# lukors/kanter_core

Hardware: AMD Instinct MI355X
Metric: node-Mpix/s on 4096x4096 f32x4, 32-node graph (higher is better)
Workload: dtype f32

## Files before the change

### bindings/rust/kanter_core_amd_sys.rs

```rust
#![allow(non_camel_case_types, dead_code)]
use std::os::raw::{c_char, c_void};

#[repr(C)] pub struct KcPlane { _private: [u8; 0] }
#[repr(C)] pub struct KcImage { _private: [u8; 0] }
#[repr(C)] pub struct KcNodeGraph { _private: [u8; 0] }
#[repr(C)] pub struct KcLiveGraph { _private: [u8; 0] }
#[repr(C)] pub struct KcTexPro { _private: [u8; 0] }
#[repr(C)] pub struct KcPartition { _private: [u8; 0] }
#[repr(C)] pub struct KcU8Pipe { _private: [u8; 0] }

#[repr(C)] #[derive(Clone, Copy, Debug, PartialEq, Eq)]
pub struct KcPlacement { pub node_id: u32, pub rank: i32, pub component: i32, pub kind: i32 }

#[repr(C)] #[derive(Clone, Copy, Debug, PartialEq, Eq)]
pub struct KcBandRows { pub node_id: u32, pub y0: i32, pub y1: i32, pub width: u32, pub height: u32 }

#[repr(C)] #[derive(Clone, Copy, Debug, PartialEq, Eq)]
pub struct KcBandRange { pub y0: i32, pub y1: i32 }

#[repr(C)] #[derive(Clone, Copy, Debug, PartialEq, Eq)]
pub struct KcTransfer { pub node_id: u32, pub slot_id: u32, pub src_rank: i32, pub dst_rank: i32, pub level: i32 }

#[repr(C)] #[derive(Clone, Copy, Debug)]
pub struct KcDeviceImage {
// ... 75 lines not shown
    pub node_type: i32,
    pub mix_type: i32,
    pub value: f32,
    pub embed_id: u32,
    pub text: *const c_char,
    pub graph: *const KcNodeGraph,
    pub resize_policy: i32,
    pub policy_slot: u32,
    pub policy_size: KcSize,
    pub resize_filter: i32,
}

pub const KC_OK: i32 = 0;
pub const KC_ERR_CANCELED: i32 = 2;
pub const KC_ERR_NO_DEVICE: i32 = 101;

#[link(name = "kanter_core_amd")]
extern "C" {
    pub fn kc_init(device_ordinal: i32) -> i32;
    pub fn kc_shutdown() -> i32;
    pub fn kc_is_initialized() -> i32;
    pub fn kc_set_stream(hip_stream: *mut c_void) -> i32;
    pub fn kc_get_stream() -> *mut c_void;
    pub fn kc_sync() -> i32;
    pub fn kc_last_error() -> *const c_char;
    pub fn kc_status_string(status: i32) -> *const c_char;
    pub fn kc_set_fusion(enabled: i32) -> i32;
    pub fn kc_get_fusion() -> i32;
    pub fn kc_set_resize_mode(mode: i32) -> i32;
    pub fn kc_get_resize_mode() -> i32;
    pub fn kc_set_cache_policy(mode: i32) -> i32;
    pub fn kc_get_cache_policy() -> i32;
    pub fn kc_set_option(name: *const c_char, value: i32) -> i32;
    pub fn kc_get_option(name: *const c_char, value: *mut i32) -> i32;
    pub fn kc_resize_upsample_plan(in_n: u32, out_n: u32, filter: i32, eligible: *mut i32, info: *mut i32, rows: *mut f32, cap: usize) -> i32;
    pub fn kc_resize_down2_plan(in_n: u32, out_n: u32, filter: i32, info: *mut i32, left_count: *mut u32, w: *mut f32, wcap: usize, vrec: *mut u32, vcap: usize, hw: *mut f32, hcap: usize) -> i32;
    pub fn kc_stats(bytes_in_use: *mut u64, bytes_cached: *mut u64, kernel_launches: *mut u64) -> i32;
    pub fn kc_stats_algorithmic_bytes(bytes: *mut u64) -> i32;
    pub fn kc_stats_counter(name: *const c_char, value: *mut u64) -> i32;
    pub fn kc_pool_trim() -> i32;
    pub fn kc_set_specialize(mode: i32, after: i32) -> i32;
    pub fn kc_get_specialize() -> i32;
    pub fn kc_specialize_wait() -> i32;
    pub fn kc_specialize_stats(kernels_compiled: *mut u64, compiles_failed: *mut u64, specialized_launches: *mut u64, compiles_pending: *mut u64) -> i32;
    pub fn kc_specialize_compile_check(words: *const u32, n_ops: u32, n_in: u32, start_src: i32, flat: i32, source: *mut c_char, cap: usize) -> i32;
    pub fn kc_specialize_compile_check_mask(words: *const u32, n_ops: u32, n_in: u32, start_src: i32, flat: i32, nt_mask: u32, source: *mut c_char, cap: usize) -> i32;
    pub fn kc_set_chain_quads(quads: i32) -> i32;
    pub fn kc_get_chain_quads() -> i32;
    pub fn kc_specialize_compile_check_upsample(words: *const u32, n_ops: u32, n_in: u32, start_src: i32, taps: u32, wide: i32, source: *mut c_char, cap: usize) -> i32;
    pub fn kc_kernel_cache_set_dir(dir: *const c_char) -> i32;
    pub fn kc_kernel_cache_stats(files_accepted: *mut u64, files_refused: *mut u64, files_written: *mut u64, kernels_loaded: *mut u64) -> i32;
    pub fn kc_kernel_cache_precompile(words: *const u32, n_ops: u32, n_in: u32, start_src: i32, flat: i32, nt_mask: u32, up_taps: u32, up_wide: i32, dir: *const c_char) -> i32;
    pub fn kc_specialize_reset() -> i32;
    pub fn kc_plane_alloc(width: u32, height: u32, out: *mut *mut KcPlane) -> i32;
    pub fn kc_plane_const(width: u32, height: u32, value: f32, out: *mut *mut KcPlane) -> i32;
    pub fn kc_plane_wrap(device_ptr: *mut c_void, width: u32, height: u32, pitch_bytes: usize, out: *mut *mut KcPlane) -> i32;
    pub fn kc_plane_retain(p: *mut KcPlane) -> i32;
    pub fn kc_plane_release(p: *mut KcPlane) -> i32;
    pub fn kc_plane_size(p: *const KcPlane, width: *mut u32, height: *mut u32) -> i32;
    pub fn kc_plane_is_const(p: *const KcPlane, is_const: *mut i32, value: *mut f32) -> i32;
    pub fn kc_plane_materialize(p: *mut KcPlane) -> i32;
    pub fn kc_plane_device_ptr(p: *mut KcPlane, device_ptr: *mut *mut c_void, pitch_bytes: *mut usize) -> i32;
    pub fn kc_plane_upload_f32(p: *mut KcPlane, host: *const f32, host_pitch_bytes: usize) -> i32;
    pub fn kc_plane_download_f32(p: *mut KcPlane, host: *mut f32, host_pitch_bytes: usize) -> i32;
    pub fn kc_image_gray(p: *mut KcPlane, out: *mut *mut KcImage) -> i32;
    pub fn kc_image_rgba(planes: *const *mut KcPlane, out: *mut *mut KcImage) -> i32;
    pub fn kc_image_retain(img: *mut KcImage) -> i32;
    pub fn kc_image_release(img: *mut KcImage) -> i32;
    pub fn kc_image_is_rgba(img: *const KcImage, is_rgba: *mut i32) -> i32;
    pub fn kc_image_size(img: *const KcImage, size: *mut KcSize) -> i32;
    pub fn kc_image_plane(img: *const KcImage, channel: i32, out: *mut *mut KcPlane) -> i32;
    pub fn kc_image_from_value(size: KcSize, value: f32, rgba: i32, out: *mut *mut KcImage) -> i32;
    pub fn kc_image_as_type(img: *const KcImage, rgba: i32, out: *mut *mut KcImage) -> i32;
    pub fn kc_image_materialize(img: *mut KcImage) -> i32;
    pub fn kc_image_from_u8(host: *const u8, width: u32, height: u32, channels: i32, out: *mut *mut KcImage) -> i32;
    pub fn kc_image_to_u8(img: *mut KcImage, srgb: i32, host_rgba8: *mut u8) -> i32;
    pub fn kc_u8_pipe_create(width: u32, height: u32, channels: i32, depth: i32, out: *mut *mut KcU8Pipe) -> i32;
    pub fn kc_u8_pipe_free(pipe: *mut KcU8Pipe) -> i32;
    pub fn kc_u8_pipe_buffers(pipe: *mut KcU8Pipe, slot: i32, host_in: *mut *mut u8, host_out: *mut *const u8) -> i32;
    pub fn kc_u8_pipe_upload(pipe: *mut KcU8Pipe, slot: i32, out: *mut *mut KcImage) -> i32;
    pub fn kc_u8_pipe_download(pipe: *mut KcU8Pipe, slot: i32, img: *mut KcImage, srgb: i32) -> i32;
    pub fn kc_u8_pipe_wait_download(pipe: *mut KcU8Pipe, slot: i32) -> i32;
    pub fn kc_image_from_f32(host_planes: *const *const f32, n_planes: i32, width: u32, height: u32, out: *mut *mut KcImage) -> i32;
    pub fn kc_image_to_f32(img: *mut KcImage, host_planes: *const *mut f32, n_planes: i32) -> i32;
    pub fn kc_device_image_validate(d: *const KcDeviceImage, extent_bytes: *mut usize) -> i32;
    pub fn kc_image_from_device(src: *const KcDeviceImage, flags: u32, hip_stream: *mut c_void, out: *mut *mut KcImage) -> i32;
    pub fn kc_image_to_device(img: *mut KcImage, dst: *const KcDeviceImage, flags: u32, hip_stream: *mut c_void) -> i32;
    pub fn kc_image_channel_stats(img: *mut KcImage, flags: u32, out: *mut KcChannelStats) -> i32;
    pub fn kc_bc_image_validate(d: *const KcBcImage, extent_bytes: *mut usize) -> i32;
    pub fn kc_image_to_bc(img: *mut KcImage, format: i32, flags: u32, host: *mut u8, host_bytes: usize) -> i32;
    pub fn kc_image_to_bc_device(img: *mut KcImage, dst: *const KcBcImage, flags: u32, hip_stream: *mut c_void) -> i32;
    pub fn kc_mip_level_count(width: u32, height: u32, levels: *mut u32) -> i32;
    pub fn kc_preview_level(width: u32, height: u32, max_extent: u32, level: *mut u32, level_width: *mut u32, level_height: *mut u32) -> i32;
    pub fn kc_image_build_mips(img: *mut KcImage, flags: u32, levels: *mut *mut KcImage, cap: u32, count: *mut u32) -> i32;
    pub fn kc_bc_mip_layout(width: u32, height: u32, format: i32, levels: *mut u32, offsets: *mut usize, cap: u32, total_bytes: *mut usize) -> i32;
    pub fn kc_image_to_bc_mips(img: *mut KcImage, format: i32, flags: u32, host: *mut u8, host_bytes: usize) -> i32;
    pub fn kc_image_to_bc_mips_device(img: *mut KcImage, format: i32, flags: u32, device_ptr: *mut c_void, bytes: usize, hip_stream: *mut c_void) -> i32;
    pub fn kc_dds_header(width: u32, height: u32, format: i32, flags: u32, levels: u32, out: *mut u8, bytes: *mut usize) -> i32;
    pub fn kc_image_write_dds(img: *mut KcImage, path: *const c_char, format: i32, flags: u32, with_mips: i32) -> i32;
    pub fn kc_image_from_bc(host: *const u8, host_bytes: usize, width: u32, height: u32, format: i32, flags: u32, out: *mut *mut KcImage, undecoded_blocks: *mut u64) -> i32;
    pub fn kc_image_from_bc_device(src: *const KcBcImage, flags: u32, hip_stream: *mut c_void, out: *mut *mut KcImage, undecoded_blocks: *mut u64) -> i32;
    pub fn kc_image_bc_compare(img: *mut KcImage, blocks: *const KcBcImage, flags: u32, out: *mut KcBcError) -> i32;
    pub fn kc_image_bc_error(img: *mut KcImage, format: i32, flags: u32, out: *mut KcBcError) -> i32;
    pub fn kc_dds_parse(data: *const u8, bytes: usize, info: *mut KcDdsInfo) -> i32;
    pub fn kc_image_read_dds(path: *const c_char, level: u32, flags: u32, out: *mut *mut KcImage, info: *mut KcDdsInfo) -> i32;
    pub fn kc_image_read_png(path: *const c_char, out: *mut *mut KcImage) -> i32;
// ... 93 lines not shown
```

### include/kanter_core_amd.h

```cpp
#ifndef KANTER_CORE_AMD_H
#define KANTER_CORE_AMD_H

#include <stddef.h>
#include <stdint.h>

#ifdef __cplusplus
extern "C" {
#endif

#define KC_API __attribute__((visibility("default")))

typedef enum kc_status {
    KC_OK = 0,
    KC_ERR_GENERIC = 1,
    KC_ERR_CANCELED = 2,
    KC_ERR_IMAGE = 3,
    KC_ERR_INVALID_BUFFER_COUNT = 4,
    KC_ERR_INVALID_NODE_ID = 5,
    KC_ERR_INVALID_NODE_TYPE = 6,
    KC_ERR_INVALID_SLOT_ID = 7,
    KC_ERR_INVALID_SLOT_TYPE = 8,
    KC_ERR_INVALID_EDGE = 9,
    KC_ERR_NO_SLOT_DATA = 10,
    KC_ERR_SLOT_OCCUPIED = 11,
// ... 40 lines not shown
    int32_t mix_type;
    float value;
    uint32_t embed_id;
    const char *text;
    const kc_node_graph *graph;
    int32_t resize_policy;
    uint32_t policy_slot;
    kc_size policy_size;
    int32_t resize_filter;
} kc_node_desc;

KC_API int kc_init(int device_ordinal);
KC_API int kc_shutdown(void);
KC_API int kc_is_initialized(void);
KC_API int kc_set_stream(void *hip_stream);
KC_API void *kc_get_stream(void);
KC_API int kc_sync(void);
KC_API const char *kc_last_error(void);
KC_API const char *kc_status_string(int status);
KC_API int kc_set_fusion(int enabled);
KC_API int kc_get_fusion(void);
KC_API int kc_set_resize_mode(int mode);
KC_API int kc_get_resize_mode(void);
KC_API int kc_set_cache_policy(int mode);
KC_API int kc_get_cache_policy(void);
KC_API int kc_set_option(const char *name, int value);
KC_API int kc_get_option(const char *name, int *value);
KC_API int kc_resize_upsample_plan(uint32_t in_n, uint32_t out_n, int filter, int *eligible, int32_t info[5], float *rows,
                                   size_t cap);
KC_API int kc_resize_down2_plan(uint32_t in_n, uint32_t out_n, int filter, int32_t info[5], uint32_t *left_count, float *w, size_t wcap,
                                uint32_t *vrec, size_t vcap, float *hw, size_t hcap);
KC_API int kc_stats(uint64_t *bytes_in_use, uint64_t *bytes_cached, uint64_t *kernel_launches);
KC_API int kc_stats_algorithmic_bytes(uint64_t *bytes);
KC_API int kc_stats_counter(const char *name, uint64_t *value);
KC_API int kc_pool_trim(void);
KC_API int kc_set_specialize(int mode, int after);
KC_API int kc_get_specialize(void);
KC_API int kc_specialize_wait(void);
KC_API int kc_specialize_stats(uint64_t *kernels_compiled, uint64_t *compiles_failed, uint64_t *specialized_launches,
                               uint64_t *compiles_pending);
KC_API int kc_specialize_compile_check(const uint32_t *words, uint32_t n_ops, uint32_t n_in, int start_src, int flat,
                                       char *source, size_t cap);
KC_API int kc_specialize_compile_check_mask(const uint32_t *words, uint32_t n_ops, uint32_t n_in, int start_src, int flat,
                                            uint32_t nt_mask, char *source, size_t cap);
KC_API int kc_set_chain_quads(int quads);
KC_API int kc_get_chain_quads(void);
KC_API int kc_specialize_compile_check_upsample(const uint32_t *words, uint32_t n_ops, uint32_t n_in, int start_src, uint32_t taps,
                                                int wide, char *source, size_t cap);
KC_API int kc_kernel_cache_set_dir(const char *dir);
KC_API int kc_kernel_cache_stats(uint64_t *files_accepted, uint64_t *files_refused, uint64_t *files_written, uint64_t *kernels_loaded);
KC_API int kc_kernel_cache_precompile(const uint32_t *words, uint32_t n_ops, uint32_t n_in, int start_src, int flat, uint32_t nt_mask,
                                      uint32_t up_taps, int up_wide, const char *dir);
KC_API int kc_specialize_reset(void);

KC_API int kc_plane_alloc(uint32_t width, uint32_t height, kc_plane **out);
KC_API int kc_plane_const(uint32_t width, uint32_t height, float value, kc_plane **out);
KC_API int kc_plane_wrap(void *device_ptr, uint32_t width, uint32_t height, size_t pitch_bytes, kc_plane **out);
KC_API int kc_plane_retain(kc_plane *p);
KC_API int kc_plane_release(kc_plane *p);
KC_API int kc_plane_size(const kc_plane *p, uint32_t *width, uint32_t *height);
KC_API int kc_plane_is_const(const kc_plane *p, int *is_const, float *value);
KC_API int kc_plane_materialize(kc_plane *p);
KC_API int kc_plane_device_ptr(kc_plane *p, void **device_ptr, size_t *pitch_bytes);
KC_API int kc_plane_upload_f32(kc_plane *p, const float *host, size_t host_pitch_bytes);
KC_API int kc_plane_download_f32(kc_plane *p, float *host, size_t host_pitch_bytes);

KC_API int kc_image_gray(kc_plane *p, kc_image **out);
KC_API int kc_image_rgba(kc_plane *const planes[4], kc_image **out);
KC_API int kc_image_retain(kc_image *img);
KC_API int kc_image_release(kc_image *img);
KC_API int kc_image_is_rgba(const kc_image *img, int *is_rgba);
KC_API int kc_image_size(const kc_image *img, kc_size *size);
KC_API int kc_image_plane(const kc_image *img, int channel, kc_plane **out);
KC_API int kc_image_from_value(kc_size size, float value, int rgba, kc_image **out);
KC_API int kc_image_as_type(const kc_image *img, int rgba, kc_image **out);
KC_API int kc_image_materialize(kc_image *img);
KC_API int kc_image_from_u8(const uint8_t *host, uint32_t width, uint32_t height, int channels, kc_image **out);
KC_API int kc_image_to_u8(kc_image *img, int srgb, uint8_t *host_rgba8);
KC_API int kc_u8_pipe_create(uint32_t width, uint32_t height, int channels, int depth, kc_u8_pipe **out);
KC_API int kc_u8_pipe_free(kc_u8_pipe *pipe);
KC_API int kc_u8_pipe_buffers(kc_u8_pipe *pipe, int slot, uint8_t **host_in, const uint8_t **host_out);
KC_API int kc_u8_pipe_upload(kc_u8_pipe *pipe, int slot, kc_image **out);
KC_API int kc_u8_pipe_download(kc_u8_pipe *pipe, int slot, kc_image *img, int srgb);
KC_API int kc_u8_pipe_wait_download(kc_u8_pipe *pipe, int slot);
KC_API int kc_image_from_f32(const float *const host_planes[], int n_planes, uint32_t width, uint32_t height, kc_image **out);
KC_API int kc_image_to_f32(kc_image *img, float *const host_planes[], int n_planes);
typedef enum kc_dtype { KC_DTYPE_U8 = 0, KC_DTYPE_U16 = 1, KC_DTYPE_F16 = 2, KC_DTYPE_BF16 = 3, KC_DTYPE_F32 = 4 } kc_dtype;
typedef enum kc_layout { KC_LAYOUT_INTERLEAVED = 0 , KC_LAYOUT_PLANAR = 1  } kc_layout;
typedef struct kc_device_image {
    void *ptr;
    uint32_t width, height;
    int32_t channels;
    int32_t dtype, layout;
    size_t row_pitch_bytes;
    size_t channel_pitch_bytes;
} kc_device_image;
#define KC_DEVICE_SRGB 1u
#define KC_DEVICE_GRAY 2u
KC_API int kc_device_image_validate(const kc_device_image *d, size_t *extent_bytes);
KC_API int kc_image_from_device(const kc_device_image *src, uint32_t flags, void *hip_stream, kc_image **out);
KC_API int kc_image_to_device(kc_image *img, const kc_device_image *dst, uint32_t flags, void *hip_stream);
#define KC_STATS_HISTOGRAM 1u
#define KC_STATS_SRGB 2u
typedef struct kc_channel_stats {
    uint32_t channels;
    uint32_t flags;
// ... 185 lines not shown
```

### kanter_core_amd/__init__.py

```python
from .api import (Edge, EmbeddedSlotDataId, LiveGraph, MixType, Node, NodeGraph, NodeId, NodeState, NodeType,
                  ResizeFilter, ResizePolicy, Side, Size, SlotData, SlotId, SlotImage, TexProError,
                  TextureProcessor, calculate_size, combine_rgba_process, get_stream, height_to_normal_process,
                  init, is_initialized, mix_process, resize_image, separate_rgba_process, set_fusion, set_stream,
                  shutdown, stats, sync, value_process, set_specialize, get_specialize, specialize_wait,
                  specialize_stats, specialize_compile_check, Partition, PartitionPolicy, NodeKind, set_resize_mode,
                  get_resize_mode, resize_upsample_plan, resize_down2_plan, stats_counter, specialize_compile_check_upsample, specialize_compile_check_mask, set_chain_quads, get_chain_quads, set_cache_policy, get_cache_policy, set_option, get_option, comm_unique_id, comm_init,
                  comm_destroy, comm_info, comm_stats, comm_transport, comm_gather_bands, PlanKind, pool_trim, kernel_cache_set_dir, kernel_cache_stats,
                  kernel_cache_precompile, specialize_reset, U8Pipe, device_image_desc, DEVICE_SRGB, DEVICE_GRAY,
                  ChannelStats, STATS_HISTOGRAM, STATS_SRGB, BC_SRGB, BC6H, BC7, BC_BLOCK_BYTES,
                  MIP_PER_LEVEL, mip_level_count, bc_mip_layout, dds_header, BC_GRAY, BC_ALL_MODES, BcError, DdsInfo, dds_parse, preview_level)

__all__ = [n for n in dir() if not n.startswith("_")]
```

### kanter_core_amd/_lib.py

```python
import ctypes as C
import os

_HERE = os.path.dirname(os.path.abspath(__file__))
LIB_PATH = os.path.join(_HERE, "libkanter_core_amd.so")

c_u8p = C.POINTER(C.c_uint8)
c_u32p = C.POINTER(C.c_uint32)
c_fp = C.POINTER(C.c_float)
c_vp = C.c_void_p


class kc_size(C.Structure):
    _fields_ = [("width", C.c_uint32), ("height", C.c_uint32)]


class kc_edge(C.Structure):
    _fields_ = [("output_id", C.c_uint32), ("input_id", C.c_uint32), ("output_slot", C.c_uint32),
                ("input_slot", C.c_uint32)]


class kc_node_desc(C.Structure):
    _fields_ = [("node_id", C.c_uint32), ("node_type", C.c_int32), ("mix_type", C.c_int32), ("value", C.c_float),
                ("embed_id", C.c_uint32), ("text", C.c_char_p), ("graph", c_vp), ("resize_policy", C.c_int32),
                ("policy_slot", C.c_uint32), ("policy_size", kc_size), ("resize_filter", C.c_int32)]
# ... 39 lines not shown
    _fields_ = [("width", C.c_uint32), ("height", C.c_uint32), ("format", C.c_int32), ("flags", C.c_uint32), ("levels", C.c_uint32),
                ("data_offset", C.c_size_t), ("data_bytes", C.c_size_t)]


SIGNATURES = {
    "kc_init": (C.c_int, [C.c_int]),
    "kc_shutdown": (C.c_int, []),
    "kc_is_initialized": (C.c_int, []),
    "kc_set_stream": (C.c_int, [c_vp]),
    "kc_get_stream": (c_vp, []),
    "kc_sync": (C.c_int, []),
    "kc_last_error": (C.c_char_p, []),
    "kc_status_string": (C.c_char_p, [C.c_int]),
    "kc_set_fusion": (C.c_int, [C.c_int]),
    "kc_set_resize_mode": (C.c_int, [C.c_int]),
    "kc_get_resize_mode": (C.c_int, []),
    "kc_set_cache_policy": (C.c_int, [C.c_int]),
    "kc_comm_unique_id": (C.c_int, [C.c_void_p]),
    "kc_comm_init": (C.c_int, [C.c_int, C.c_int, C.c_void_p]),
    "kc_comm_destroy": (C.c_int, []),
    "kc_comm_info": (C.c_int, [C.POINTER(C.c_int), C.POINTER(C.c_int)]),
    "kc_comm_stats": (C.c_int, [C.POINTER(C.c_uint64), C.POINTER(C.c_uint64), C.POINTER(C.c_uint64)]),
    "kc_live_graph_exchange": (C.c_int, [C.c_void_p, C.c_void_p, C.c_uint32]),
    "kc_comm_transport": (C.c_int, [C.c_char_p, C.c_size_t]),
    "kc_u8_pipe_create": (C.c_int, [C.c_uint32, C.c_uint32, C.c_int, C.c_int, C.POINTER(C.c_void_p)]),
    "kc_u8_pipe_free": (C.c_int, [C.c_void_p]),
    "kc_u8_pipe_buffers": (C.c_int, [C.c_void_p, C.c_int, C.POINTER(C.c_void_p), C.POINTER(C.c_void_p)]),
    "kc_u8_pipe_upload": (C.c_int, [C.c_void_p, C.c_int, C.POINTER(C.c_void_p)]),
    "kc_u8_pipe_download": (C.c_int, [C.c_void_p, C.c_int, C.c_void_p, C.c_int]),
    "kc_u8_pipe_wait_download": (C.c_int, [C.c_void_p, C.c_int]),
    "kc_kernel_cache_set_dir": (C.c_int, [C.c_char_p]),
    "kc_kernel_cache_stats": (C.c_int, [C.POINTER(C.c_uint64)] * 4),
    "kc_kernel_cache_precompile": (C.c_int, [C.POINTER(C.c_uint32), C.c_uint32, C.c_uint32, C.c_int, C.c_int, C.c_uint32, C.c_uint32, C.c_int, C.c_char_p]),
    "kc_specialize_reset": (C.c_int, []),
    "kc_comm_gather_bands": (C.c_int, [C.c_void_p, C.c_int32, C.c_uint32, C.c_int, C.POINTER(C.c_void_p)]),
    "kc_live_graph_evaluate_partitioned": (C.c_int, [C.c_void_p, C.c_void_p, C.c_uint32, C.POINTER(C.c_void_p)]),
    "kc_set_option": (C.c_int, [C.c_char_p, C.c_int]),
    "kc_get_option": (C.c_int, [C.c_char_p, C.POINTER(C.c_int)]),
    "kc_get_cache_policy": (C.c_int, []),
    "kc_stats_counter": (C.c_int, [C.c_char_p, C.POINTER(C.c_uint64)]),
    "kc_resize_down2_plan": (C.c_int, [C.c_uint32, C.c_uint32, C.c_int, C.POINTER(C.c_int32), C.POINTER(C.c_uint32), C.POINTER(C.c_float),
                                       C.c_size_t, C.POINTER(C.c_uint32), C.c_size_t, C.POINTER(C.c_float), C.c_size_t]),
    "kc_resize_upsample_plan": (C.c_int, [C.c_uint32, C.c_uint32, C.c_int, C.POINTER(C.c_int), C.POINTER(C.c_int32),
                                          C.POINTER(C.c_float), C.c_size_t]),
    "kc_get_fusion": (C.c_int, []),
    "kc_stats": (C.c_int, [C.POINTER(C.c_uint64)] * 3),
    "kc_set_specialize": (C.c_int, [C.c_int, C.c_int]),
    "kc_get_specialize": (C.c_int, []),
    "kc_specialize_wait": (C.c_int, []),
    "kc_specialize_stats": (C.c_int, [C.POINTER(C.c_uint64)] * 4),
    "kc_specialize_compile_check": (C.c_int, [c_u32p, C.c_uint32, C.c_uint32, C.c_int, C.c_int, C.c_char_p, C.c_size_t]),
    "kc_specialize_compile_check_mask": (C.c_int, [c_u32p, C.c_uint32, C.c_uint32, C.c_int, C.c_int, C.c_uint32, C.c_char_p, C.c_size_t]),
    "kc_set_chain_quads": (C.c_int, [C.c_int]),
    "kc_get_chain_quads": (C.c_int, []),
    "kc_specialize_compile_check_upsample": (C.c_int, [c_u32p, C.c_uint32, C.c_uint32, C.c_int, C.c_uint32, C.c_int, C.c_char_p,
                                                       C.c_size_t]),
    "kc_stats_algorithmic_bytes": (C.c_int, [C.POINTER(C.c_uint64)]),
    "kc_pool_trim": (C.c_int, []),
    "kc_live_graph_partition": (C.c_int, [c_vp, C.c_uint32, C.c_int, C.c_int, C.POINTER(c_vp)]),
    "kc_partition_free": (C.c_int, [c_vp]),
    "kc_partition_info": (C.c_int, [c_vp, C.POINTER(C.c_int), C.POINTER(C.c_int), C.POINTER(C.c_int)]),
    "kc_partition_nodes": (C.c_int, [c_vp, C.POINTER(kc_placement), C.c_uint32, c_u32p]),
    "kc_partition_transfers": (C.c_int, [c_vp, C.POINTER(kc_transfer), C.c_uint32, c_u32p]),
    "kc_partition_kind": (C.c_int, [c_vp, C.POINTER(C.c_int), C.POINTER(C.c_double), C.POINTER(C.c_double), C.POINTER(C.c_double)]),
    "kc_partition_bands": (C.c_int, [c_vp, C.POINTER(kc_band_range), C.c_uint32, c_u32p, c_u32p, c_u32p]),
    "kc_partition_set_gather": (C.c_int, [c_vp, C.c_int]),
    "kc_live_graph_import_slot_data": (C.c_int, [c_vp, C.c_uint32, C.c_uint32, c_vp]),
    "kc_live_graph_evaluate_band": (C.c_int, [c_vp, C.c_uint32, C.c_uint32, C.c_int32, C.c_int32, C.POINTER(c_vp)]),
    "kc_live_graph_band_source_rows": (C.c_int, [c_vp, C.c_uint32, C.c_int32, C.c_int32, C.POINTER(kc_band_rows), C.c_uint32, c_u32p]),
    "kc_live_graph_embed_slot_data_band": (C.c_int, [c_vp, c_vp, C.c_uint32, C.c_uint32, C.c_int32, C.c_uint32]),
    "kc_plane_alloc": (C.c_int, [C.c_uint32, C.c_uint32, C.POINTER(c_vp)]),
    "kc_plane_const": (C.c_int, [C.c_uint32, C.c_uint32, C.c_float, C.POINTER(c_vp)]),
    "kc_plane_wrap": (C.c_int, [c_vp, C.c_uint32, C.c_uint32, C.c_size_t, C.POINTER(c_vp)]),
    "kc_plane_retain": (C.c_int, [c_vp]),
    "kc_plane_release": (C.c_int, [c_vp]),
    "kc_plane_size": (C.c_int, [c_vp, c_u32p, c_u32p]),
    "kc_plane_is_const": (C.c_int, [c_vp, C.POINTER(C.c_int), c_fp]),
    "kc_plane_materialize": (C.c_int, [c_vp]),
    "kc_plane_device_ptr": (C.c_int, [c_vp, C.POINTER(c_vp), C.POINTER(C.c_size_t)]),
    "kc_plane_upload_f32": (C.c_int, [c_vp, c_vp, C.c_size_t]),
    "kc_plane_download_f32": (C.c_int, [c_vp, c_vp, C.c_size_t]),
    "kc_image_gray": (C.c_int, [c_vp, C.POINTER(c_vp)]),
    "kc_image_rgba": (C.c_int, [C.POINTER(c_vp), C.POINTER(c_vp)]),
    "kc_image_retain": (C.c_int, [c_vp]),
    "kc_image_release": (C.c_int, [c_vp]),
    "kc_image_is_rgba": (C.c_int, [c_vp, C.POINTER(C.c_int)]),
    "kc_image_size": (C.c_int, [c_vp, C.POINTER(kc_size)]),
    "kc_image_plane": (C.c_int, [c_vp, C.c_int, C.POINTER(c_vp)]),
    "kc_image_from_value": (C.c_int, [kc_size, C.c_float, C.c_int, C.POINTER(c_vp)]),
    "kc_image_as_type": (C.c_int, [c_vp, C.c_int, C.POINTER(c_vp)]),
    "kc_image_materialize": (C.c_int, [c_vp]),
    "kc_image_from_u8": (C.c_int, [c_vp, C.c_uint32, C.c_uint32, C.c_int, C.POINTER(c_vp)]),
    "kc_image_to_u8": (C.c_int, [c_vp, C.c_int, c_vp]),
    "kc_device_image_validate": (C.c_int, [C.POINTER(kc_device_image), C.POINTER(C.c_size_t)]),
    "kc_image_from_device": (C.c_int, [C.POINTER(kc_device_image), C.c_uint32, c_vp, C.POINTER(c_vp)]),
    "kc_image_to_device": (C.c_int, [c_vp, C.POINTER(kc_device_image), C.c_uint32, c_vp]),
    "kc_image_channel_stats": (C.c_int, [c_vp, C.c_uint32, C.POINTER(kc_channel_stats)]),
    "kc_bc_image_validate": (C.c_int, [C.POINTER(kc_bc_image), C.POINTER(C.c_size_t)]),
    "kc_image_to_bc": (C.c_int, [c_vp, C.c_int, C.c_uint32, c_vp, C.c_size_t]),
    "kc_image_to_bc_device": (C.c_int, [c_vp, C.POINTER(kc_bc_image), C.c_uint32, c_vp]),
    "kc_mip_level_count": (C.c_int, [C.c_uint32, C.c_uint32, C.POINTER(C.c_uint32)]),
    "kc_preview_level": (C.c_int, [C.c_uint32, C.c_uint32, C.c_uint32, c_u32p, c_u32p, c_u32p]),
    "kc_image_build_mips": (C.c_int, [c_vp, C.c_uint32, C.POINTER(c_vp), C.c_uint32, C.POINTER(C.c_uint32)]),
    "kc_bc_mip_layout": (C.c_int, [C.c_uint32, C.c_uint32, C.c_int, C.POINTER(C.c_uint32), C.POINTER(C.c_size_t), C.c_uint32,
                                   C.POINTER(C.c_size_t)]),
    "kc_image_to_bc_mips": (C.c_int, [c_vp, C.c_int, C.c_uint32, c_vp, C.c_size_t]),
# ... 126 lines not shown
```

### kanter_core_amd/api.py

```python
import collections
import ctypes as C
import os

import numpy as np

from . import _lib
from ._lib import kc_edge, kc_node_desc, kc_size

_ERROR_NAMES = {
    1: "Generic", 2: "Canceled", 3: "Image", 4: "InvalidBufferCount", 5: "InvalidNodeId", 6: "InvalidNodeType",
    7: "InvalidSlotId", 8: "InvalidSlotType", 9: "InvalidEdge", 10: "NoSlotData", 11: "SlotOccupied",
    12: "SlotNotOccupied", 13: "UnableToLock", 14: "NodeProcessing", 15: "PoisonError", 16: "TryLockError",
    17: "NodeDirty", 18: "Io", 19: "InvalidName", 100: "Hip", 101: "NoDevice", 102: "InvalidArgument",
    103: "OutOfMemory", 104: "Unsupported",
}


class TexProError(Exception):

    def __init__(self, code, detail=""):
        self.code = code
        self.kind = _ERROR_NAMES.get(code, "Unknown")
        L = _lib.load()
        msg = L.kc_status_string(code).decode()
# ... 139 lines not shown
    lc = np.zeros(2 * out_n, np.uint32)
    w = np.zeros((out_n, stride), np.float32)
    vrec = np.zeros((groups, max(nc, 1), 72), np.uint32)
    hw = np.zeros((out_n, max(hstride, 1)), np.float32)
    _check(L.kc_resize_down2_plan(int(in_n), int(out_n), int(f), info, lc.ctypes.data_as(C.POINTER(C.c_uint32)),
                                  w.ctypes.data_as(C.POINTER(C.c_float)), w.size,
                                  vrec.ctypes.data_as(C.POINTER(C.c_uint32)), vrec.size if nc else 0,
                                  hw.ctypes.data_as(C.POINTER(C.c_float)), hw.size if hstride else 0))
    return dict(stride=stride, nc=nc, hstride=hstride, tile_w=tile_w, min_count=min_count, left=lc[:out_n].copy(),
                count=lc[out_n:].copy(), w=w, vrec=vrec if nc else None, hw=hw if hstride else None)


def set_specialize(mode, after=0):
    _check(_lib.load().kc_set_specialize(int(mode), int(after)))


def get_specialize():
    return _lib.load().kc_get_specialize()


def specialize_wait():
    _check(_lib.load().kc_specialize_wait())


def specialize_stats():
    v = [C.c_uint64() for _ in range(4)]
    _check(_lib.load().kc_specialize_stats(*[C.byref(x) for x in v]))
    return dict(zip(("kernels_compiled", "compiles_failed", "specialized_launches", "compiles_pending"), [x.value for x in v]))


def specialize_compile_check(words, n_in, start_src=0, flat=True):
    arr = (C.c_uint32 * len(words))(*words)
    buf = C.create_string_buffer(1 << 16)
    _check(_lib.load().kc_specialize_compile_check(arr, len(words), int(n_in), int(start_src), int(bool(flat)), buf, len(buf)))
    return buf.value.decode()


def specialize_compile_check_mask(words, n_in, nt_mask, start_src=0, flat=True):
    arr = (C.c_uint32 * len(words))(*words)
    buf = C.create_string_buffer(1 << 17)
    _check(_lib.load().kc_specialize_compile_check_mask(arr, len(words), int(n_in), int(start_src), int(bool(flat)), int(nt_mask),
                                                        buf, len(buf)))
    return buf.value.decode()


def set_chain_quads(quads):
    _check(_lib.load().kc_set_chain_quads(int(quads)))


def get_chain_quads():
    return _lib.load().kc_get_chain_quads()


def specialize_compile_check_upsample(words, n_in, start_src=0, taps=3, wide=True):
    arr = (C.c_uint32 * len(words))(*words)
    buf = C.create_string_buffer(1 << 17)
    _check(_lib.load().kc_specialize_compile_check_upsample(arr, len(words), int(n_in), int(start_src), int(taps), int(bool(wide)),
                                                            buf, len(buf)))
    return buf.value.decode()


def stats():
    a, b, c = C.c_uint64(), C.c_uint64(), C.c_uint64()
    _check(_lib.load().kc_stats(C.byref(a), C.byref(b), C.byref(c)))
    d = C.c_uint64()
    _check(_lib.load().kc_stats_algorithmic_bytes(C.byref(d)))
    return {"bytes_in_use": a.value, "bytes_cached": b.value, "kernel_launches": c.value, "algorithmic_bytes": d.value}


def kernel_cache_set_dir(path):
    _check(_lib.load().kc_kernel_cache_set_dir(None if path is None else str(path).encode()))


def kernel_cache_stats():
    v = [C.c_uint64() for _ in range(4)]
    _check(_lib.load().kc_kernel_cache_stats(*[C.byref(x) for x in v]))
    return dict(zip(("files_accepted", "files_refused", "files_written", "kernels_loaded"), (x.value for x in v)))


def kernel_cache_precompile(words, n_in, start_src, flat, nt_mask, directory, up_taps=0, up_wide=False):
    arr = (C.c_uint32 * len(words))(*words)
    _check(_lib.load().kc_kernel_cache_precompile(arr, len(words), int(n_in), int(start_src), int(bool(flat)), int(nt_mask),
                                                  int(up_taps), int(bool(up_wide)), str(directory).encode()))


def specialize_reset():
    _check(_lib.load().kc_specialize_reset())


def pool_trim():
    _check(_lib.load().kc_pool_trim())


def stats_counter(name):
    v = C.c_uint64()
    _check(_lib.load().kc_stats_counter(name.encode(), C.byref(v)))
    return v.value


class NodeId(int):
    """NodeId(u32), src/node_graph.rs:592-607"""


class SlotId(int):
    """SlotId(u32), src/node_graph.rs:609-624"""


class EmbeddedSlotDataId(int):
    """src/node/embed.rs:13-14"""


class Size:

    def __init__(self, width, height):
        self.width, self.height = int(width), int(height)

    def pixel_count(self):
        return (self.width * self.height) & 0xFFFFFFFF

    def __eq__(self, o):
        if isinstance(o, tuple):
            return (self.width, self.height) == o
        return isinstance(o, Size) and (self.width, self.height) == (o.width, o.height)

    def __hash__(self):
        return hash((self.width, self.height))

    def __iter__(self):
        return iter((self.width, self.height))

    def __repr__(self):
        return "%dx%d" % (self.width, self.height)

    def _c(self):
# ... 1143 lines not shown
```

### kanter_core_amd/build.py

```python
import os
import subprocess
import sys
from concurrent.futures import ThreadPoolExecutor

HERE = os.path.dirname(os.path.abspath(__file__))
CSRC = os.path.join(HERE, "csrc")
OBJ = os.path.join(HERE, "csrc", "build")
LIB = os.path.join(HERE, "libkanter_core_amd.so")
SOURCES = ["chain.hip", "upsample.hip", "resize_tile.hip", "resize_down.hip", "h2n.hip", "u8.hip", "chain1.hip", "down2.hip", "runtime.cpp",
           "ops.cpp", "resize.cpp", "graph.cpp", "json.cpp", "png.cpp", "specialize.cpp", "partition.cpp", "bands.cpp", "comm.cpp", "replay.cpp",
           "u8pipe.cpp", "devimage.hip", "devimage.cpp", "stats.hip", "stats.cpp", "bc.hip", "bc7.hip", "bc6h.hip", "bc.cpp", "mip.hip", "mip.cpp", "bc_decode.hip",
           "bc_decode.cpp", "bc_modes.hip",
           "c_api.cpp"]
HEADERS = ["kc_internal.hpp", "kc_runtime.hpp", "chain_program.h", os.path.join("..", "..", "include", "kanter_core_amd.h"), "pow_positive.inc",
           "srgb_thresholds.inc", "streaming.h", "bc_blocks.h", "bc_modes.h", "upsample.h", "upsample_chain.inc", "chain_apply.inc", "chain_interp.inc", "resample.inc"]
JIT_TEXTS = [("kJitChainProgramH", "chain_program.h"), ("kJitPowPositiveInc", "pow_positive.inc"), ("kJitUpsampleH", "upsample.h"),
             ("kJitUpsampleChainInc", "upsample_chain.inc")]

FLAGS = ["--offload-arch=gfx950", "-O3", "-std=c++17", "-fPIC", "-fvisibility=hidden", "-fno-fast-math",
         "-ffp-contract=off", "-fhip-fp32-correctly-rounded-divide-sqrt", "-Wall", "-Wno-unused-result"]
DEVICE_FLAGS = ["-mllvm", "-structurizecfg-skip-uniform-regions=1"]
if os.environ.get("KC_HOST_PROFILE"):
    FLAGS = FLAGS + ["-DKC_HOST_PROFILE"]
if os.environ.get("KC_HOST_SAMPLE"):
    FLAGS = FLAGS + ["-DKC_HOST_SAMPLE", "-fno-omit-frame-pointer"]


def _hipcc():
    for cand in (os.environ.get("HIPCC"), "/opt/rocm/bin/hipcc", "hipcc"):
        if cand and (os.path.isabs(cand) and os.path.exists(cand) or not os.path.isabs(cand)):
            return cand
    return "hipcc"


def _stale(target, deps):
    if not os.path.exists(target):
        return True
    t = os.path.getmtime(target)
    return any(os.path.getmtime(d) > t for d in deps)


def object_name(src):
    stem = os.path.splitext(src)[0]
    if src.endswith(".hip") and stem + ".cpp" in SOURCES:
        stem += "_kernels"
    return stem + ".o"


def _write_jit_texts():
    out = os.path.join(OBJ, "jit_texts.cpp")
    parts = ["// generated by kanter_core_amd/build.py from csrc/chain_program.h and csrc/pow_positive.inc -- do not edit\n",
             "namespace kc {\n"]
    for name, fn in JIT_TEXTS:
        with open(os.path.join(CSRC, fn)) as f:
            text = f.read()
        assert ')KCJIT"' not in text
        parts.append('extern const char %s[];\nconst char %s[] = R"KCJIT(\n%s)KCJIT";\n' % (name, name, text))
    parts.append("}  // namespace kc\n")
    new = "".join(parts)
    old = open(out).read() if os.path.exists(out) else None
    if new != old:
        with open(out, "w") as f:
            f.write(new)
    return out


def build(force=False, verbose=False):
    os.makedirs(OBJ, exist_ok=True)
    hipcc = _hipcc()
    hdrs = [os.path.join(CSRC, h) for h in HEADERS]
# ... 6 lines not shown
        jobs.append([hipcc] + FLAGS + ["-c", jit, "-o", jit_o])
    for src in SOURCES:
        s = os.path.join(CSRC, src)
        o = os.path.join(OBJ, object_name(src))
        objs.append(o)
        if force or _stale(o, [s] + hdrs):
            cmd = [hipcc] + FLAGS + (DEVICE_FLAGS + ["-x", "hip"] if src.endswith(".hip") else []) + ["-c", s, "-o", o]
            jobs.append(cmd)

    def run(cmd):
        if verbose:
            print(" ".join(cmd), flush=True)
        r = subprocess.run(cmd, stdout=subprocess.PIPE, stderr=subprocess.STDOUT, text=True)
        if r.returncode != 0:
            raise RuntimeError("hipcc failed:\n%s\n%s" % (" ".join(cmd), r.stdout))
        return r.stdout

    with ThreadPoolExecutor(max_workers=4) as ex:
        for out in ex.map(run, jobs):
            if verbose and out.strip():
                print(out)
    if force or jobs or _stale(LIB, objs):
        run([hipcc, "--offload-arch=gfx950", "-shared", "-fPIC", "-o", LIB] + objs + ["-lz", "-ldl"])
    populate_kernel_cache(verbose=verbose)
    return LIB


MANIFEST = os.path.join(HERE, "baseline_programs.jsonl")
KERNEL_CACHE = os.path.join(HERE, "kernel_cache")


def populate_kernel_cache(force=False, verbose=False):
    import ctypes as C
    import hashlib
    import json
    if not os.path.exists(MANIFEST) or not os.path.exists(LIB):
        return 0
    with open(MANIFEST) as f:
        text = f.read()
    entries = [json.loads(line) for line in text.splitlines() if line.strip()]
    st = os.stat(LIB)
    stamp = hashlib.sha256(("%s|%d|%d" % (text, st.st_mtime_ns, st.st_size)).encode()).hexdigest()
    stamp_file = os.path.join(KERNEL_CACHE, ".stamp")
    if not force and os.path.exists(stamp_file) and open(stamp_file).read() == stamp:
        return len(entries)
    os.makedirs(KERNEL_CACHE, exist_ok=True)
    for old in os.listdir(KERNEL_CACHE):
        if old.endswith(".kcco"):
            os.remove(os.path.join(KERNEL_CACHE, old))
    L = C.CDLL(LIB)
    L.kc_kernel_cache_precompile.argtypes = [C.POINTER(C.c_uint32), C.c_uint32, C.c_uint32, C.c_int, C.c_int, C.c_uint32, C.c_uint32,
                                             C.c_int, C.c_char_p]
    L.kc_kernel_cache_precompile.restype = C.c_int
    L.kc_last_error.restype = C.c_char_p

    def one(e):
        words = (C.c_uint32 * len(e["words"]))(*e["words"])
        rc = L.kc_kernel_cache_precompile(words, len(e["words"]), e["n_in"], e["start_src"], e["flat"], e["nt_mask"], e["up_taps"],
                                          e["up_wide"], KERNEL_CACHE.encode())
        if rc != 0:
            raise RuntimeError("pre-compiling %s failed (%d): %s" % (e.get("name"), rc, (L.kc_last_error() or b"").decode(errors="replace")))
        if verbose:
            print("pre-compiled", e.get("name"), flush=True)

    with ThreadPoolExecutor(max_workers=4) as ex:
        list(ex.map(one, entries))
    with open(stamp_file, "w") as f:
        f.write(stamp)
    return len(entries)


if __name__ == "__main__":
    print(build(force="--force" in sys.argv, verbose=True))
```

### kanter_core_amd/csrc/c_api.cpp

```cpp
#include <algorithm>
#include <cctype>
#include <climits>
#include <cstdio>
#include <cstdlib>
#include <cstring>
#include <fstream>
#include <sstream>

#include "kc_runtime.hpp"

namespace kc {
const std::string &last_error();
}
using namespace kc;

#define KC_ARG(cond)                                         \
    do {                                                     \
        if (!(cond)) {                                       \
            set_error("invalid argument: " #cond);           \
            return KC_ERR_INVALID_ARG;                       \
        }                                                    \
    } while (0)

typedef std::lock_guard<std::recursive_mutex> Lock;
// ... 359 lines not shown
    P.nt_mask = nt_mask;
    for (uint32_t i = 0; i < n_ops; ++i) {
        const uint32_t from = (words[i] >> 8) & 0xffu, level = words[i] >> 16;
        KC_ARG((words[i] & 0xffu) <= CH_SAVE_LOAD && (from <= n_in || (from == (uint32_t)KC_CHAIN_SRC_SAVED && (words[i] & 0xffu) != CH_SAVE_LOAD)));
        KC_ARG(level < (uint32_t)KC_CHAIN_MAX_SAVED && (level == 0 || from == (uint32_t)KC_CHAIN_SRC_SAVED || (words[i] & 0xffu) == CH_SAVE_LOAD));
        ((i & 1u) ? P.step[0][i / 2].b : P.step[0][i / 2].a).word = words[i];
    }
    if (source && cap) {
        const std::string src = specialize_source(P);
        std::snprintf(source, cap, "%s", src.c_str());
    }
    std::string log;
    int s = specialize_compile_only(P, &log);
    if (s != KC_OK) set_error("specialised chain kernel did not compile: " + log);
    return s;
}
KC_CATCH

int kc_set_chain_quads(int quads)
try {
    const int s = specialize_set_chain_quads(quads);
    if (s != KC_OK) set_error("kc_set_chain_quads accepts 0, 1, 2 or 4");
    return s;
}
KC_CATCH

int kc_get_chain_quads(void)
try {
    return specialize_get_chain_quads();
}
catch (...) {
    return 0;
}

int kc_kernel_cache_set_dir(const char *dir)
try {
    Lock lk(ctx().mu);
    return kernel_cache_set_dir(dir);
}
KC_CATCH

int kc_kernel_cache_stats(uint64_t *hits, uint64_t *rejected, uint64_t *written, uint64_t *kernels_loaded)
try {
    kernel_cache_stats(hits, rejected, written, kernels_loaded);
    return KC_OK;
}
KC_CATCH

int kc_kernel_cache_precompile(const uint32_t *words, uint32_t n_ops, uint32_t n_in, int start_src, int flat, uint32_t nt_mask,
                               uint32_t up_taps, int up_wide, const char *dir)
try {
    KC_ARG(words && dir);
    std::string log;
    const int s = kernel_cache_precompile(words, n_ops, n_in, start_src, flat != 0, nt_mask, up_taps, up_wide != 0, dir, &log);
    if (s != KC_OK) set_error("kernel cache: " + log);
    return s;
}
KC_CATCH

int kc_specialize_reset(void)
try {
    Lock lk(ctx().mu);
    if (ctx().stream) (void)hipStreamSynchronize(ctx().stream);
    const int mode = specialize_get_mode();
    specialize_shutdown();
    (void)mode;
    return KC_OK;
}
KC_CATCH

int kc_specialize_compile_check_upsample(const uint32_t *words, uint32_t n_ops, uint32_t n_in, int start_src, uint32_t taps, int wide,
                                         char *source, size_t cap)
try {
    KC_ARG(words && n_ops >= 1 && n_ops <= (uint32_t)KC_CHAIN_MAX_OPS && n_in >= 1 && n_in <= (uint32_t)KC_CHAIN_INTERP_IN);
    KC_ARG(start_src >= -1 && start_src < (int)n_in && (taps == 1 || taps == 3));
    ChainProgram P;
    std::memset(&P, 0, sizeof P);
    P.n_ops = n_ops;
    P.n_in = n_in;
    P.start_src = start_src;
    for (uint32_t i = 0; i < n_ops; ++i) {
        const uint32_t from = words[i] >> 8, code = words[i] & 0xffu;
        KC_ARG(code <= CH_MUL_INV && from <= n_in && code != CH_DIV_L && code != CH_DIV_R && code != CH_POW_L && code != CH_POW_R);
        ((i & 1u) ? P.step[0][i / 2].b : P.step[0][i / 2].a).word = words[i];
    }
    UpsampleArgs U{};
    U.H.taps = U.V.taps = taps;
    U.tile_w = wide ? 1024u : 256u;
    if (source && cap) {
        const std::string src = specialize_source(P, &U);
        std::snprintf(source, cap, "%s", src.c_str());
    }
    std::string log;
    int s = specialize_compile_only(P, &log, &U);
    if (s != KC_OK) set_error("specialised up-sampling kernel did not compile: " + log);
    return s;
}
KC_CATCH

int kc_stats(uint64_t *in_use, uint64_t *cached, uint64_t *launches)
try {
    Context &c = ctx();
    Lock lk(c.mu);
    if (in_use) *in_use = c.bytes_in_use;
    if (cached) *cached = c.bytes_cached;
    if (launches) *launches = c.launches;
    return KC_OK;
}
KC_CATCH

int kc_stats_counter(const char *name, uint64_t *value)
// ... 60 lines not shown
    *out = p;
    return KC_OK;
}
KC_CATCH

int kc_plane_retain(kc_plane *p)
try {
    Lock api_lock(ctx().mu);
    KC_ARG(p);
    plane_retain(p);
    return KC_OK;
}
KC_CATCH

int kc_plane_release(kc_plane *p)
try {
    if (!p) return KC_OK;
    Lock lk(ctx().mu);
    plane_release(p);
    return KC_OK;
}
KC_CATCH

int kc_plane_size(const kc_plane *p, uint32_t *w, uint32_t *h)
try {
    KC_ARG(p);
    if (w) *w = p->w;
    if (h) *h = p->h;
    return KC_OK;
}
KC_CATCH

int kc_plane_is_const(const kc_plane *p, int *is_const, float *v)
try {
    KC_ARG(p);
    if (is_const) *is_const = p->kind == kc_plane::CONST;
    if (v) *v = p->cval;
    return KC_OK;
}
KC_CATCH

int kc_plane_materialize(kc_plane *p)
try {
    Lock api_lock(ctx().mu);
    KC_ARG(p);
    return plane_materialize(p);
}
KC_CATCH

int kc_plane_device_ptr(kc_plane *p, void **dptr, size_t *pitch)
try {
    KC_ARG(p);
    KC_TRY(plane_materialize(p));
    if (dptr) *dptr = p->dptr;
    if (pitch) *pitch = p->pitch;
    return KC_OK;
}
KC_CATCH

int kc_plane_upload_f32(kc_plane *p, const float *host, size_t host_pitch)
try {
    KC_TRY(need_init());
    KC_ARG(p && host && p->kind == kc_plane::MEM);
    if (host_pitch == 0) host_pitch = (size_t)p->w * 4;
    Lock lk(ctx().mu);
    KC_HIP(hipMemcpy2DAsync(p->dptr, p->pitch, host, host_pitch, (size_t)p->w * 4, p->h, hipMemcpyHostToDevice, ctx().stream));
    KC_HIP(hipStreamSynchronize(ctx().stream));
    return KC_OK;
}
KC_CATCH

int kc_plane_download_f32(kc_plane *p, float *host, size_t host_pitch)
try {
    KC_ARG(p && host);
    if (host_pitch == 0) host_pitch = (size_t)p->w * 4;
    Lock lk(ctx().mu);
    if (p->kind == kc_plane::CONST) {
        for (uint32_t y = 0; y < p->h; ++y) {
            float *row = (float *)((char *)host + y * host_pitch);
            for (uint32_t x = 0; x < p->w; ++x) row[x] = p->cval;
        }
        return KC_OK;
    }
    KC_TRY(need_init());
    KC_TRY(plane_force(p));
    KC_HIP(hipMemcpy2DAsync(host, host_pitch, p->dptr, p->pitch, (size_t)p->w * 4, p->h, hipMemcpyDeviceToHost, ctx().stream));
    KC_HIP(hipStreamSynchronize(ctx().stream));
    return KC_OK;
}
KC_CATCH

int kc_image_gray(kc_plane *p, kc_image **out)
try {
    Lock api_lock(ctx().mu);
    KC_ARG(p && out);
    *out = image_new(1, &p);
    return KC_OK;
}
KC_CATCH

int kc_image_rgba(kc_plane *const planes[4], kc_image **out)
try {
    Lock api_lock(ctx().mu);
    KC_ARG(planes && out && planes[0] && planes[1] && planes[2] && planes[3]);
    for (int i = 1; i < 4; ++i) KC_ARG(planes[i]->w == planes[0]->w && planes[i]->h == planes[0]->h);
    *out = image_new(4, planes);
    return KC_OK;
}
KC_CATCH

int kc_image_retain(kc_image *img)
try {
    Lock api_lock(ctx().mu);
    KC_ARG(img);
    image_retain(img);
    return KC_OK;
}
KC_CATCH
// ... 1195 lines not shown
```

### kanter_core_amd/csrc/chain_program.h

```cpp
enum { KC_CHAIN_MAX_OPS = 80, KC_CHAIN_MAX_IN = 16, KC_CHAIN_INTERP_IN = 4, KC_CHAIN_MAX_BATCH = 4 };
#define KC_CHAIN_NT_BIT(k) ((k) < 8 ? 1u << (k) : 1u << ((k) + 8))

enum ChainCode : unsigned char {
    CH_ADD = 0,
    CH_SUB_L = 1,
    CH_SUB_R = 2,
    CH_MUL = 3,
    CH_DIV_L = 4,
    CH_DIV_R = 5,
    CH_POW_L = 6,
    CH_POW_R = 7,
    CH_ADD_R = 8,
    CH_MUL_R = 9,
    CH_ADD_INV = 10,
    CH_SUBL_INV = 11,
    CH_SUBR_INV = 12,
    CH_MUL_INV = 13,
    CH_SAVE_LOAD = 14
};
enum { KC_CHAIN_SRC_SAVED = 255, KC_CHAIN_MAX_SAVED = 3 };

struct ChainStepRec {
    unsigned int word;
    float c;
};
struct alignas(16) ChainStepPair {
    ChainStepRec a, b;
};

struct ChainProgram {
    unsigned int n_ops;
    unsigned int n_in;
    unsigned int row_units;
    unsigned int rows;
    int start_src;
    unsigned int nt_mask;
    const float *in[KC_CHAIN_MAX_BATCH][KC_CHAIN_MAX_IN];
    unsigned int in_pitch[KC_CHAIN_MAX_BATCH][KC_CHAIN_MAX_IN];
    float *out[KC_CHAIN_MAX_BATCH];
    unsigned int out_pitch[KC_CHAIN_MAX_BATCH];
    float start_c[KC_CHAIN_MAX_BATCH];
    const float *samp_src[KC_CHAIN_MAX_BATCH];
    unsigned int samp_pitch[KC_CHAIN_MAX_BATCH];
    ChainStepPair step[KC_CHAIN_MAX_BATCH][KC_CHAIN_MAX_OPS / 2 + 1];
};
```

### kanter_core_amd/csrc/kc_internal.hpp

```cpp
#pragma once

#include <hip/hip_runtime.h>

#include <atomic>
#include <cstdint>
#include <map>
#include <memory>
#include <mutex>
#include <string>
#include <vector>

#include "../../include/kanter_core_amd.h"

namespace kc {

#include "chain_program.h"
#include "upsample.h"

struct Options {
    int chain1, replay, join, wide, fusion, down2, down2_by_rows, poly2, poly2_min_ratio, resize_mode, resize_tile_w, resize_tile_h;
    int poly_rows, poly2_xcd, down2_xcd, h2n_tiled, cache_policy, cache_budget_mb, nt_force, chain_unroll, max_blocks, tune_cap;
    int upload_ring, link_gbps, hbm_gbps;
};
Options option_defaults();
// ... 118 lines not shown
                                    uint32_t dh, TapsDev h, hipStream_t s);
hipError_t launch_resize_down(const ResizePlan &r, const ResizePlanes &p, TapsDev v, TapsDev h, hipStream_t s);
hipError_t launch_resize_poly(const ResizePlan &r, const ResizePlanes &p, TapsDev v, TapsDev h, hipStream_t s);
hipError_t launch_resize_poly2(const ResizePlan &r, const ResizePlanes &p, TapsDev v, TapsDev h, hipStream_t s);
hipError_t launch_resize_down2(const ResizePlan &r, const ResizePlanes &p, const Down2Args &a, hipStream_t s);
#ifdef KC_UP_RU
constexpr uint32_t KC_UPSAMPLE_ROWS = KC_UP_RU;
#else
constexpr uint32_t KC_UPSAMPLE_ROWS = 4;
#endif
inline uint32_t upsample_tile_rows(const UpsampleArgs &u) { return KC_UPSAMPLE_ROWS * (1024u / u.tile_w); }
inline size_t upsample_lds_bytes(const UpsampleArgs &u)
{
    return ((size_t)upsample_tile_rows(u) * u.ncp + (size_t)(std::max(u.H.ratio >> 2, 1u) + u.H.qb_lo + u.H.qb_hi) * 4u * u.H.taps) * sizeof(float);
}
inline bool upsample_args_ok(const UpsampleArgs &u, int batch)
{
    if (batch < 1 || batch > 4) return false;
    if (u.tile_w % 4 != 0 || u.tile_w == 0 || u.tile_w > 1024 || 256u % (u.tile_w / 4) != 0) return false;
    const uint32_t tile_h = upsample_tile_rows(u);
    if (u.chunk == 0 || tile_h % u.chunk != 0 || u.V.ratio % u.chunk != 0) return false;
    if (u.H.ratio % 4 != 0 && !(u.H.ratio == 2 && u.H.n_out % 4 == 0)) return false;
    if (u.H.taps != u.V.taps || u.ncp % 4 != 0 || !u.H.qcls || !u.V.cls) return false;
    if (u.H.n_out > 65535 || u.V.n_out > 65535) return false;
    if (u.ncp / 4 > 257 || (std::max(u.H.ratio >> 2, 1u) + u.H.qb_lo + u.H.qb_hi) * u.H.taps > 256) return false;
    return upsample_lds_bytes(u) <= 64 * 1024;
}
inline dim3 upsample_grid(const UpsampleArgs &u, int batch)
{
    const uint32_t tile_h = upsample_tile_rows(u);
    return dim3((u.H.n_out + u.tile_w - 1) / u.tile_w, (u.V.n_out + tile_h - 1) / tile_h, batch);
}
struct UpsamplePlanes {
    const float *samp_src[4];
    unsigned int samp_pitch[4];
    float *out[4];
    unsigned int out_pitch[4];
    const float *in[4][1];
    unsigned int in_pitch[4][1];
    unsigned int nt_mask;
};
hipError_t launch_upsample_chain(const ChainProgram &p, int batch, const UpsampleArgs &u, hipStream_t s);
hipError_t launch_upsample(const UpsamplePlanes &p, int batch, const UpsampleArgs &u, hipStream_t s);
struct H2nVariant {
    bool launched = false, band = false, nt = false;
    uint32_t tq = 0;
};
hipError_t launch_height_to_normal(const float *hgt, uint32_t hpitch, uint32_t w, uint32_t h, uint32_t full_h, int band,
                                   float *nx, float *ny, float *nz, uint32_t opitch, uint32_t nt_mask, hipStream_t s, H2nVariant *var);
hipError_t launch_to_u8(Operand r, Operand g, Operand b, Operand a, int gray, int srgb, uint32_t w, uint32_t h,
                        uint8_t *dst, uint32_t nt_mask, hipStream_t s, bool *launched_nt);
hipError_t launch_from_u8(const uint8_t *src, int channels, uint32_t w, uint32_t h, float *const planes[4],
                          uint32_t pitch, uint32_t nt_mask, hipStream_t s, bool *launched_nt);
struct DevImageArgs {
    const char *ptr;
    uint64_t row_pitch, channel_pitch;
    uint32_t w, h;
    int channels, layout;
    int vec;
};
hipError_t launch_image_import(int dtype, const DevImageArgs &a, float *const planes[4], uint32_t ppitch, uint32_t nt_mask, hipStream_t s,
                               bool *launched_nt);
hipError_t launch_image_export(int dtype, int srgb, const Operand op[4], int gray, const DevImageArgs &a, uint32_t nt_mask, hipStream_t s,
                               bool *launched_nt);
struct StatsArgs {
    const float *ptr[4];
    uint32_t pitch[4];
    uint32_t w, h, n, srgb;
    uint32_t *partials;
    uint32_t rec_words;
    unsigned long long *result;
};
hipError_t launch_channel_stats(const StatsArgs &a, bool hist, bool srgb, bool nt, uint32_t groups, hipStream_t s);
uint32_t channel_stats_groups(uint32_t w, uint32_t h, bool hist, bool srgb, uint32_t cus);
hipError_t launch_bc_encode(int fmt, int srgb, const Operand op[4], int gray, char *dst, uint64_t row_pitch, uint32_t w, uint32_t h,
                            uint32_t nt_mask, hipStream_t s);
hipError_t launch_bc7_encode(int srgb, const Operand op[4], int gray, char *dst, uint64_t row_pitch, uint32_t w, uint32_t h, uint32_t nt_mask,
                             hipStream_t s);
struct BcDecodeArgs {
    const char *src;
    uint64_t row_pitch;
    float *dst[4];
    uint32_t dst_pitch;
    uint32_t w, h, bx, by;
    unsigned long long *partials, *result;
};
hipError_t launch_bc_decode(int fmt, const BcDecodeArgs &a, bool count, uint32_t nt_mask, uint32_t groups, hipStream_t s);
uint32_t bc_decode_groups(uint32_t w, uint32_t h, bool count);
constexpr uint32_t KC_BC_REC_WORDS = 17;
hipError_t launch_bc_compare(int fmt, int srgb, const Operand op[4], int gray, const char *blocks, uint64_t row_pitch, uint32_t w, uint32_t h,
                             uint32_t nt_mask, uint32_t groups, unsigned long long *partials, unsigned long long *result, hipStream_t s);
uint32_t bc_compare_groups(uint32_t w, uint32_t h);
hipError_t launch_bc_combine(const unsigned long long *partials, uint32_t groups, uint32_t rec_words, uint32_t max_cols,
                             unsigned long long *result, hipStream_t s);
hipError_t launch_bc6h_encode(const Operand op[4], int gray, char *dst, uint64_t row_pitch, uint32_t w, uint32_t h, uint32_t nt_mask,
                              hipStream_t s);
hipError_t launch_bc6h_decode(const BcDecodeArgs &a, bool count, uint32_t nt_mask, uint32_t groups, hipStream_t s);
hipError_t launch_bc6h_compare(const Operand op[4], int gray, const char *blocks, uint64_t row_pitch, uint32_t w, uint32_t h, uint32_t nt_mask,
                               uint32_t groups, unsigned long long *partials, unsigned long long *result, hipStream_t s);
hipError_t launch_bc_modes_decode(int fmt, const BcDecodeArgs &a, uint32_t nt_mask, uint32_t groups, hipStream_t s);
hipError_t launch_bc_modes_compare(int fmt, int srgb, const Operand op[4], int gray, const char *blocks, uint64_t row_pitch, uint32_t w,
                                   uint32_t h, uint32_t nt_mask, uint32_t groups, unsigned long long *partials, unsigned long long *result,
                                   hipStream_t s);
struct MipPyramidArgs {
    const float *src[4];
    uint32_t src_pitch[4];
// ... 16 lines not shown
```

### kanter_core_amd/csrc/kc_runtime.hpp

```cpp
#pragma once

#include <cstring>
#include <deque>
#include <set>
#include <tuple>
#include <type_traits>
#include <unordered_map>
#include <unordered_set>

#include "kc_internal.hpp"

namespace kc {
struct Chain;
struct ChainLink;
}

namespace kc {
#if defined(__SANITIZE_ADDRESS__) || defined(__SANITIZE_THREAD__)
#define KC_NO_OBJECT_POOL 1
#elif defined(__has_feature)
#if __has_feature(address_sanitizer) || __has_feature(thread_sanitizer)
#define KC_NO_OBJECT_POOL 1
#endif
#endif
// ... 13 lines not shown
                head = b->next;
                ::operator delete(b);
            }
            n = 0;
        }
    };
    static FreeList &list()
    {
        static FreeList fl;
        return fl;
    }
    static void *operator new(size_t bytes)
    {
        FreeList &fl = list();
        if (bytes == sizeof(T) && fl.head) {
            typename FreeList::Block *b = fl.head;
            fl.head = b->next;
            --fl.n;
            return b;
        }
        return ::operator new(bytes < sizeof(typename FreeList::Block) ? sizeof(typename FreeList::Block) : bytes);
    }
    static void operator delete(void *q, size_t bytes)
    {
        FreeList &fl = list();
        if (bytes == sizeof(T) && fl.n < FreeList::kMaxFree && !fl.closed) {
            typename FreeList::Block *b = static_cast<typename FreeList::Block *>(q);
            b->next = fl.head;
            fl.head = b;
            ++fl.n;
            return;
        }
        ::operator delete(q);
    }
#endif
};
}

struct kc_plane : kc::Pooled<kc_plane> {
    enum Kind { MEM = 0, CONST = 1, LAZY = 2, RESIZE = 3 };
    int refs = 1;
    uint32_t w = 0, h = 0;
    Kind kind = MEM;
    float *dptr = nullptr;
    size_t pitch = 0;
    size_t bytes = 0;
    bool owned = false;
    float cval = 0.0f;
    kc::ChainLink *link = nullptr;
    kc::Chain *chain = nullptr;
    kc_plane *view_of = nullptr;
    kc_plane *rz_src = nullptr;
    int rz_filter = 0;
};

struct kc_image : kc::Pooled<kc_image> {
    int refs = 1;
    int n = 0;
    kc_plane *planes[4] = { nullptr, nullptr, nullptr, nullptr };
    bool is_rgba() const { return n == 4; }
    uint32_t w() const { return planes[0]->w; }
    uint32_t h() const { return planes[0]->h; }
};

namespace kc {

struct ChainStep {
    uint8_t code;
    kc_plane *operand;
    uint8_t level = 0;
};
kc_plane *saved_value_marker();

struct Chain : Pooled<Chain> {
    kc_plane *start = nullptr;
    std::vector<ChainStep> steps;
    std::vector<kc_plane *> joined;
    ~Chain();
};

struct ChainLink : Pooled<ChainLink> {
    kc_plane *prev = nullptr;
    kc_plane *start = nullptr;
    ChainStep step{};
    uint32_t length = 1;
    bool fused = false;
    uint8_t saved = 0;
    int n_in = 0;
    struct InKey {
        const void *p = nullptr;
        size_t q = 0;
        bool operator==(const InKey &o) const { return p == o.p && q == o.q; }
    };
    InKey ins[KC_CHAIN_MAX_IN + 1];
    ~ChainLink();
};

struct TapsHost {
    std::vector<uint32_t> left, count;
    std::vector<float> w;
    uint32_t stride = 1;
    uint32_t min_count = 1;
    uint32_t reg_a = 0, reg_b = 0, reg_ages = 0, reg_ratio = 0;
    bool up_ok = false;
    UpAxis up{};
    std::vector<float> up_rows, up_qrows;
    std::vector<uint32_t> d2_vrec, d2_strips;
    std::vector<float> d2_hw;
    bool d2_want = false;
    uint32_t d2_nc = 0, d2_hstride = 0, d2_tile_w = 0;
    uint32_t p2_tile_w = 0;
    const uint32_t *d2_vrec_dev = nullptr, *d2_strips_dev = nullptr;
    const float *d2_hw_dev = nullptr;
};

struct TapsEntry {
    uint64_t last_use = 0;
    TapsHost host;
    void *dev_block = nullptr;
    size_t dev_bytes = 0;
    TapsDev dev{};
};

struct ReplayLaunch {
    ChainProgram prog;
    int batch = 0, mode = 0;
    uint32_t in_refs[KC_CHAIN_MAX_IN] = {};
    uint32_t w = 0, h = 0;
    kc_plane *planes[KC_CHAIN_MAX_BATCH] = { nullptr, nullptr, nullptr, nullptr };
    int in_from[KC_CHAIN_MAX_BATCH][KC_CHAIN_MAX_IN];
    int in_ch[KC_CHAIN_MAX_BATCH][KC_CHAIN_MAX_IN];
};
struct ReplayCapture {
    bool ok = true;
    std::vector<ReplayLaunch> launches;
};

struct Context {
    std::recursive_mutex mu;
    ReplayCapture *capture = nullptr;
    uint64_t band_taps_clock = 0;
    bool inited = false;
    int device = -1;
    hipStream_t own_stream = nullptr;
    hipStream_t stream = nullptr;
    Options opt = option_defaults();
    bool plain_chains = false;
    std::multimap<size_t, void *> free_blocks;
    uint64_t bytes_in_use = 0, bytes_cached = 0, launches = 0;
    std::map<std::string, uint64_t> counters;
    uint64_t alg_bytes = 0;
    std::map<std::tuple<uint32_t, uint32_t, int>, TapsEntry> taps;
    std::map<std::tuple<uint32_t, uint32_t, int, int32_t, int32_t, int32_t>, TapsEntry> band_taps;
    int memo_depth = 0;
    std::map<std::tuple<kc_plane *, uint32_t, uint32_t, int>, kc_plane *> resize_memo;
    struct UploadSlot {
        void *host = nullptr;
        size_t bytes = 0;
        hipEvent_t copied = nullptr;
    };
    static constexpr int kUploadSlots = 4;
    static constexpr size_t kUploadSlotMax = (size_t)4 << 20;
    UploadSlot upload_ring[kUploadSlots];
    int upload_next = 0;
    struct StatsBuffers {
        void *partials = nullptr;
        size_t partials_bytes = 0;
        unsigned long long *result = nullptr, *host = nullptr;
        hipEvent_t done = nullptr;
        uint32_t cus = 0;
    };
    StatsBuffers stats;
};

struct ResizeMemoScope {
    ResizeMemoScope();
    ~ResizeMemoScope();
};

Context &ctx();
void set_error(const std::string &msg);
const std::string &last_error();
int hip_fail(hipError_t e, const char *what);
int need_init();

#ifdef KC_HOST_PROFILE
struct ProfScope {
    const char *name;
    unsigned long long t0;
    explicit ProfScope(const char *n) : name(n), t0(__builtin_ia32_rdtsc()) {}
    ~ProfScope();
};
void prof_report();
#define KC_PROF(name) kc::ProfScope _kc_prof_scope(name)
#else
#define KC_PROF(name) (void)0
#endif

#ifdef KC_HOST_SAMPLE
void sampler_start();
void sampler_report();
#endif

// ... 87 lines not shown
    return (uint32_t)(uint8_t)a | (uint32_t)(uint8_t)b << 8 | (uint32_t)(uint8_t)c << 16 | (uint32_t)(uint8_t)d << 24;
}
const BcFormat *bc_format(int format);
const BcFormat *bc_format_of_dds(uint32_t dxgi, uint32_t cc, uint32_t *flags);
size_t bc_block_bytes(int format);
size_t bc_level_bytes(uint32_t w, uint32_t h, const BcFormat &f);
int bc_block_count(uint32_t w, uint32_t h, const char *who, uint64_t *bx, uint64_t *by);
int bc_check_flags(int format, uint32_t flags, uint32_t allowed, const char *who);
uint32_t bc_source_operands(const kc_image *img, uint32_t mask, Operand (&o)[4]);
int bc_encode(kc_image *img, int format, bool srgb, char *dst, size_t row_pitch, hipStream_t s);
hipError_t bc_launch_encode(int format, bool srgb, const Operand op[4], int gray, char *dst, uint64_t row_pitch, uint32_t w, uint32_t h,
                            uint32_t nt_mask, hipStream_t s);
hipError_t bc_launch_decode(int format, bool all_modes, const BcDecodeArgs &a, bool count, uint32_t nt_mask, uint32_t groups, hipStream_t s);
hipError_t bc_launch_compare(int format, bool srgb, bool all_modes, const Operand op[4], int gray, const char *blocks, uint64_t row_pitch, uint32_t w, uint32_t h,
                             uint32_t nt_mask, uint32_t groups, unsigned long long *partials, unsigned long long *result, hipStream_t s);
int image_from_bc(const uint8_t *host, size_t host_bytes, uint32_t w, uint32_t h, int format, uint32_t flags, kc_image **out,
                  uint64_t *undecoded_blocks);
int image_from_bc_device(const kc_bc_image *src, uint32_t flags, void *hip_stream, kc_image **out, uint64_t *undecoded_blocks);
int image_bc_compare(kc_image *img, const kc_bc_image *blocks, uint32_t flags, kc_bc_error *out);
int image_bc_error(kc_image *img, int format, uint32_t flags, kc_bc_error *out);
int dds_parse(const uint8_t *data, size_t bytes, kc_dds_info *info);
int image_read_dds(const char *path, uint32_t level, uint32_t flags, kc_image **out, kc_dds_info *info);
int mip_level_count(uint32_t w, uint32_t h, uint32_t *levels);
int preview_level(uint32_t w, uint32_t h, uint32_t max_extent, uint32_t *level, uint32_t *pw, uint32_t *ph);
float mip_const_fold(float c);
int image_build_mips(kc_image *img, uint32_t flags, kc_image **levels, uint32_t cap, uint32_t *count);
int bc_mip_layout(uint32_t w, uint32_t h, int format, uint32_t *levels, size_t *offsets, uint32_t cap, size_t *total_bytes);
int image_to_bc_mips(kc_image *img, int format, uint32_t flags, uint8_t *host, size_t host_bytes);
int image_to_bc_mips_device(kc_image *img, int format, uint32_t flags, void *device_ptr, size_t bytes, void *hip_stream);
int dds_header(uint32_t w, uint32_t h, int format, uint32_t flags, uint32_t levels, uint8_t *out, size_t *bytes);
int image_write_dds(kc_image *img, const char *path, int format, uint32_t flags, int with_mips);
int image_channel_stats(kc_image *img, uint32_t flags, kc_channel_stats *out);
int stats_buffers(size_t partials_bytes);
void channel_stats_release();
int calculate_size(int policy, const kc_size *sizes, int n, int slot_index, kc_size specific, kc_size *out);
int mix_process(kc_image *left, kc_image *right, int mix_type, kc_image **out);
int separate_process(kc_image *in, kc_image *out[4]);
int combine_process(kc_image *const in[4], kc_image **out);
int value_process(float v, kc_image **out);
int height_to_normal_process(kc_image *in, kc_image **out);
int height_to_normal_band(kc_image *in_with_halo, uint32_t full_h, kc_image **out);

int build_taps_host(uint32_t in_n, uint32_t out_n, int filter, TapsHost &t);
int resize_image(kc_image *src, kc_size size, int filter, kc_image **out);
int resize_force(kc_plane *p);
int resize_planes_band(kc_plane *const *srcs, int n, int32_t src_y0, uint32_t src_h_full, kc_size dst_full, int32_t a, int32_t b,
                       int filter, kc_plane **outs);
int resize_force_many(kc_plane *const *planes, int n);
int chain_resize_launch(const ChainProgram &P, int batch, int mode, kc_plane *const *sampled, bool *launched);

hipError_t launch_chain_specialized(const ChainProgram &P, int batch, hipStream_t s, bool *launched, uint32_t *nt_mask, uint32_t *quads = nullptr);
uint32_t cache_policy_mask(uint64_t in_bytes, uint64_t out_bytes, uint32_t n_resident, const Options &o = options());
uint32_t chain_cache_policy(const uint32_t *refs, uint32_t n, uint64_t stream_bytes, uint64_t out_bytes);
hipError_t chain_dispatch(ChainProgram &P, int batch, int mode, uint32_t w, uint32_t h, size_t out_pitch_bytes);
hipError_t launch_upsample_chain_specialized(const ChainProgram &P, int batch, const UpsampleArgs &U, hipStream_t s, bool *launched);
int specialize_set_mode(int mode, int after);
int specialize_get_mode();
int specialize_set_chain_quads(int quads);
int specialize_get_chain_quads();
void specialize_wait();
void specialize_stats(uint64_t *compiled, uint64_t *failed, uint64_t *launches, uint64_t *pending);
std::string specialize_last_log();
void specialize_shutdown();
std::string specialize_source(const ChainProgram &P, const UpsampleArgs *U = nullptr);
int specialize_compile_only(const ChainProgram &P, std::string *log, const UpsampleArgs *U = nullptr);
int kernel_cache_set_dir(const char *dir);
void kernel_cache_stats(uint64_t *hits, uint64_t *rejected, uint64_t *written, uint64_t *kernels_loaded);
bool kernel_cache_populated();
int kernel_cache_precompile(const uint32_t *words, uint32_t n_ops, uint32_t n_in, int32_t start_src, bool flat, uint32_t nt_mask,
                            uint32_t up_taps, bool up_wide, const char *dir, std::string *log);

int u8_pipe_create(uint32_t w, uint32_t h, int channels, int depth, kc_u8_pipe **out);
int u8_pipe_free(kc_u8_pipe *p);
int u8_pipe_buffers(kc_u8_pipe *p, int slot, uint8_t **host_in, const uint8_t **host_out);
int u8_pipe_upload(kc_u8_pipe *p, int slot, kc_image **out);
int u8_pipe_download(kc_u8_pipe *p, int slot, kc_image *img, bool srgb);
int u8_pipe_wait_download(kc_u8_pipe *p, int slot);

int png_read(const std::string &path, std::vector<uint8_t> &px, uint32_t &w, uint32_t &h, int &channels);
int png_write_rgba8(const std::string &path, const uint8_t *px, uint32_t w, uint32_t h);

struct NodeGraph;

struct Node {
    uint32_t node_id = 0;
    int type = KC_NODE_VALUE;
    int mix_type = KC_MIX_ADD;
    float value = 0.0f;
    uint32_t embed_id = 0;
    std::string text;
    std::shared_ptr<NodeGraph> graph;
    int policy = KC_POLICY_MOST_PIXELS;
    uint32_t policy_slot = 0;
    kc_size policy_size{ 0, 0 };
    int filter = KC_FILTER_TRIANGLE;

    bool is_input() const { return type == KC_NODE_INPUT_GRAY || type == KC_NODE_INPUT_RGBA; }
    bool is_output() const { return type == KC_NODE_OUTPUT_GRAY || type == KC_NODE_OUTPUT_RGBA; }
    bool is_source() const { return type == KC_NODE_EMBED || type == KC_NODE_IMAGE || is_input(); }
};

enum SlotType { SLOT_GRAY = 0, SLOT_RGBA = 1, SLOT_GRAY_OR_RGBA = 2 };
struct Slot {
    std::string name;
    uint32_t slot_id;
    int slot_type;
};

struct GraphIndex {
    uint64_t version = ~0ull;
    size_t n_nodes = 0, n_edges = 0;
    std::unordered_map<uint32_t, uint32_t> node_pos;
    std::unordered_map<uint32_t, std::vector<kc_edge>> in_edges;
    std::unordered_map<uint32_t, std::vector<kc_edge>> out_edges;
};

struct NodeGraph {
    std::vector<Node> nodes;
    std::vector<kc_edge> edges;
    uint32_t node_id_counter = 0;
    uint64_t version = 0;
    mutable GraphIndex idx;
// ... 213 lines not shown
```

### kanter_core_amd/csrc/replay.cpp

```cpp
#include "kc_runtime.hpp"

using namespace kc;

struct kc_live_graph::ReplayEntry {
    uint32_t root = 0;
    uint64_t ghash = 0;
    std::vector<std::pair<uint32_t, int>> pre_state;
    struct Held {
        uint32_t node, slot;
        kc_image *img;
    };
    std::vector<Held> pre_slots;
    std::vector<EmbeddedSlotData> embedded;
    std::vector<std::pair<uint32_t, int>> post_state;
    std::vector<uint32_t> dropped;
    std::vector<uint32_t> changed_ids;
    std::vector<ReplayLaunch> launches;
    uint32_t w = 0, h = 0;
    uint32_t root_slot = 0;
    int n_planes = 0;
    int out_l[4] = { -1, -1, -1, -1 };
    int out_b[4] = { -1, -1, -1, -1 };
    float cval[4] = { 0, 0, 0, 0 };

// ... 28 lines not shown
    h = mix64(h, g.edges.size());
    for (auto &e : g.edges) {
        h = mix64(h, ((uint64_t)e.output_id << 32) | e.input_id);
        h = mix64(h, ((uint64_t)e.output_slot << 32) | e.input_slot);
    }
    return h;
}

static bool recordable_type(int t)
{
    return t == KC_NODE_MIX || t == KC_NODE_VALUE || t == KC_NODE_COMBINE_RGBA || t == KC_NODE_SEPARATE_RGBA ||
           t == KC_NODE_OUTPUT_GRAY || t == KC_NODE_OUTPUT_RGBA || t == KC_NODE_EMBED;
}

static size_t slot_count_except(const kc_live_graph &lg, uint32_t node)
{
    size_t n = 0;
    for (auto &kv : lg.slot_datas)
        if (kv.first != node) n += kv.second.size();
    return n;
}

int replay_try(kc_live_graph &lg, uint32_t id, bool *hit)
{
    *hit = false;
    const kc_live_graph::ReplayEntry *e = lg.replay;
    if (!e || e->root != id || lg.use_cache || lg.auto_update || !options().fusion || !options().replay) return KC_OK;
    if (e->pre_state.size() != lg.node_state.size()) return KC_OK;
    for (auto &ps : e->pre_state) {
        auto it = lg.node_state.find(ps.first);
        if (it == lg.node_state.end() || it->second != ps.second) return KC_OK;
    }
    if (slot_count_except(lg, id) != e->pre_slots.size()) return KC_OK;
    for (auto &h : e->pre_slots) {
        const SlotData *sd = lg.find_slot(h.node, h.slot);
        if (!sd || sd->image != h.img) return KC_OK;
    }
    if (lg.embedded.size() != e->embedded.size()) return KC_OK;
    for (size_t i = 0; i < e->embedded.size(); ++i) {
        const EmbeddedSlotData &a = lg.embedded[i], &b = e->embedded[i];
        if (a.image != b.image || a.slot_data_id != b.slot_data_id || a.slot_id != b.slot_id || a.full_h != b.full_h || a.band_y0 != b.band_y0)
            return KC_OK;
    }
    if (graph_content_hash(lg.g) != e->ghash) return KC_OK;

    Context &c = ctx();
    std::vector<kc_plane *> outs(e->launches.size() * KC_CHAIN_MAX_BATCH, nullptr);
    auto drop_outs = [&] {
        for (auto *o : outs) plane_release(o);
    };
    for (size_t li = 0; li < e->launches.size(); ++li) {
        const ReplayLaunch &L = e->launches[li];
        ChainProgram P = L.prog;
        for (int b = 0; b < L.batch; ++b) {
            kc_plane *&o = outs[li * KC_CHAIN_MAX_BATCH + b];
            int s = plane_new_mem(L.w, L.h, &o);
            if (s != KC_OK) {
                drop_outs();
                return s;
            }
            P.out[b] = o->dptr;
            P.out_pitch[b] = (uint32_t)(o->pitch / 16);
            for (uint32_t k = 0; k < P.n_in; ++k)
                if (L.in_from[b][k] >= 0) {
                    const kc_plane *src = outs[(size_t)L.in_from[b][k] * KC_CHAIN_MAX_BATCH + L.in_ch[b][k]];
                    P.in[b][k] = src->dptr;
                    P.in_pitch[b][k] = (uint32_t)(src->pitch / 16);
                }
        }
        const uint64_t px4 = 4ull * L.w * L.h;
        P.nt_mask = chain_cache_policy(L.in_refs, P.n_in, px4 * L.batch, px4 * L.batch);
        hipError_t he = chain_dispatch(P, L.batch, L.mode, L.w, L.h, outs[li * KC_CHAIN_MAX_BATCH]->pitch);
        if (he == hipErrorNotReady) {
            drop_outs();
            return KC_OK;
        }
        if (he != hipSuccess) {
            drop_outs();
            return hip_fail(he, "launch_chain (replay)");
        }
        c.launches++;
        c.alg_bytes += (uint64_t)L.batch * px4 * (P.n_in + 1);
    }
    c.counters["replayed_evaluations"]++;

    kc_plane *planes[4] = { nullptr, nullptr, nullptr, nullptr };
    std::vector<kc_plane *> consts;
    for (int p = 0; p < e->n_planes; ++p) {
        if (e->out_l[p] >= 0) planes[p] = outs[(size_t)e->out_l[p] * KC_CHAIN_MAX_BATCH + e->out_b[p]];
        else {
            planes[p] = plane_new_const(e->w, e->h, e->cval[p]);
            consts.push_back(planes[p]);
        }
    }
    kc_image *img = image_new(e->n_planes, planes);
    for (auto *q : consts) plane_release(q);
    drop_outs();

    for (uint32_t d : e->dropped) lg.remove_nodes_data(d);
    lg.slot_datas[id].push_back(SlotData{ id, e->root_slot, img });
    for (auto &ps : e->post_state) lg.node_state[ps.first] = ps.second;
    for (uint32_t ch : e->changed_ids) lg.changed.insert(ch);
    *hit = true;
    return KC_OK;
}

struct ReplayRecorder {
    kc_live_graph::ReplayEntry *entry = nullptr;
    ReplayCapture cap;
    uint64_t launches0 = 0;
    std::unordered_set<uint32_t> changed0;
    std::set<const void *> resident0;
};

static void note_resident(std::set<const void *> &set, const kc_image *img)
{
    for (int p = 0; p < img->n; ++p)
        if (img->planes[p]->kind == kc_plane::MEM) set.insert(img->planes[p]->dptr);
}

ReplayRecorder *replay_begin(kc_live_graph &lg, uint32_t id)
{
    Context &c = ctx();
    if (lg.use_cache || lg.auto_update || !c.opt.fusion || !c.opt.replay || c.capture || lg.depth > 0) return nullptr;
    if (lg.g.nodes.size() > 4096) return nullptr;
    auto *r = new ReplayRecorder();
    auto *e = new kc_live_graph::ReplayEntry();
    r->entry = e;
    e->root = id;
    e->ghash = graph_content_hash(lg.g);
    e->pre_state.assign(lg.node_state.begin(), lg.node_state.end());
    for (auto &kv : lg.slot_datas)
        for (auto &sd : kv.second) {
            if (sd.node_id == id) continue;
            image_retain(sd.image);
            e->pre_slots.push_back({ sd.node_id, sd.slot_id, sd.image });
            note_resident(r->resident0, sd.image);
        }
    for (auto &em : lg.embedded) {
        if (em.full_h != 0) {
            delete e;
            delete r;
            return nullptr;
        }
        image_retain(em.image);
        e->embedded.push_back(em);
        note_resident(r->resident0, em.image);
    }
    r->launches0 = c.launches;
    r->changed0 = lg.changed;
    c.capture = &r->cap;
    return r;
}

void replay_end(kc_live_graph &lg, uint32_t id, ReplayRecorder *r, int s)
{
    if (!r) return;
    Context &c = ctx();
    c.capture = nullptr;
    std::unique_ptr<ReplayRecorder> own(r);
    std::unique_ptr<kc_live_graph::ReplayEntry> e(r->entry);
    lg.replay_clear();
    if (s != KC_OK || !r->cap.ok || r->cap.launches.empty() || c.launches - r->launches0 != r->cap.launches.size()) return;
    std::unordered_map<uint32_t, int> pre(e->pre_state.begin(), e->pre_state.end());
    if (pre.size() != lg.node_state.size()) return;
    {
        std::unordered_set<uint32_t> had;
        for (auto &h : e->pre_slots) had.insert(h.node);
        for (auto &n : lg.g.nodes)
            if (!had.count(n.node_id) && !recordable_type(n.type)) return;
    }
    for (auto &kv : lg.node_state) {
        auto it = pre.find(kv.first);
        if (it == pre.end()) return;
        if (it->second != kv.second) {
            const Node *n = lg.g.find(kv.first);
            if (!n || !recordable_type(n->type)) return;
            e->post_state.push_back({ kv.first, kv.second });
        }
    }
    std::unordered_map<uint64_t, kc_image *> before;
    for (auto &h : e->pre_slots) before[((uint64_t)h.node << 32) | h.slot] = h.img;
    std::unordered_set<uint32_t> has_after;
    const SlotData *root_sd = nullptr;
    size_t root_slots = 0;
    for (auto &kv : lg.slot_datas)
        for (auto &sd : kv.second) {
            has_after.insert(sd.node_id);
            if (sd.node_id == id) {
                root_sd = &sd;
                ++root_slots;
                continue;
            }
            auto it = before.find(((uint64_t)sd.node_id << 32) | sd.slot_id);
            if (it == before.end() || it->second != sd.image) return;
        }
    if (!root_sd || root_slots != 1) return;
    std::unordered_set<uint32_t> dropped;
    for (auto &h : e->pre_slots)
        if (!has_after.count(h.node)) dropped.insert(h.node);
    dropped.insert(id);
    for (auto &h : e->pre_slots)
        if (!dropped.count(h.node) && !lg.find_slot(h.node, h.slot)) return;
    e->dropped.assign(dropped.begin(), dropped.end());
    const kc_image *img = root_sd->image;
    ReplayCapture &cap = r->cap;
    e->w = img->w();
    e->h = img->h();
    e->root_slot = root_sd->slot_id;
    e->n_planes = img->n;
    for (int p = 0; p < img->n; ++p) {
        const kc_plane *pl = img->planes[p];
        e->out_l[p] = e->out_b[p] = -1;
        if (pl->kind == kc_plane::CONST) {
            e->cval[p] = pl->cval;
            continue;
        }
        for (size_t li = 0; li < cap.launches.size(); ++li)
            for (int b = 0; b < cap.launches[li].batch; ++b)
                if (cap.launches[li].planes[b] == pl && cap.launches[li].w == img->w() && cap.launches[li].h == img->h()) {
                    e->out_l[p] = (int)li;
                    e->out_b[p] = b;
                }
        if (e->out_l[p] < 0) return;
    }
    for (size_t li = 0; li < cap.launches.size(); ++li) {
        ReplayLaunch &L = cap.launches[li];
        for (int b = 0; b < L.batch; ++b)
            for (uint32_t k = 0; k < L.prog.n_in; ++k) {
                L.in_from[b][k] = L.in_ch[b][k] = -1;
                for (size_t lj = li; lj-- > 0 && L.in_from[b][k] < 0;)
                    for (int bj = 0; bj < cap.launches[lj].batch; ++bj)
                        if (cap.launches[lj].prog.out[bj] == L.prog.in[b][k]) {
                            if (cap.launches[lj].w != L.w || cap.launches[lj].h != L.h) return;
                            L.in_from[b][k] = (int)lj;
                            L.in_ch[b][k] = bj;
                        }
                if (L.in_from[b][k] < 0 && !r->resident0.count(L.prog.in[b][k])) return;
            }
    }
    for (uint32_t ch : lg.changed)
        if (!r->changed0.count(ch)) e->changed_ids.push_back(ch);
    e->launches = std::move(cap.launches);
    lg.replay = e.release();
}

}

void kc_live_graph::replay_clear()
{
    delete replay;
    replay = nullptr;
}
```

### kanter_core_amd/csrc/runtime.cpp

```cpp
#include <cmath>
#include <cstdlib>
#include <cstdio>
#include <cstring>

#include <algorithm>

#ifdef KC_HOST_SAMPLE
#include <dlfcn.h>
#include <new>
#include <signal.h>
#include <sys/time.h>
#include <ucontext.h>
#endif

#include "kc_runtime.hpp"

namespace kc {

static const int KC_RETRY_CHAIN = -1000;

static thread_local std::string g_last_error;

Context &ctx()
{
// ... 161 lines not shown
    c.bytes_cached = 0;
    return KC_OK;
}

static size_t pitch_for(uint32_t w)
{
    size_t row = (size_t)w * sizeof(float);
    return (row + 255) / 256 * 256;
}

int plane_new_mem(uint32_t w, uint32_t h, kc_plane **out)
{
    KC_TRY(need_init());
    if (w == 0 || h == 0) {
        set_error("plane with zero extent");
        return KC_ERR_INVALID_ARG;
    }
    kc_plane *p = new kc_plane();
    p->w = w;
    p->h = h;
    p->kind = kc_plane::MEM;
    p->pitch = pitch_for(w);
    p->bytes = p->pitch * h;
    p->owned = true;
    void *d = nullptr;
    int s = pool_alloc(p->bytes, &d);
    if (s != KC_OK) {
        delete p;
        return s;
    }
    p->dptr = (float *)d;
    *out = p;
    return KC_OK;
}

kc_plane *plane_new_const(uint32_t w, uint32_t h, float v)
{
    kc_plane *p = new kc_plane();
    p->w = w;
    p->h = h;
    p->kind = kc_plane::CONST;
    p->cval = v;
    return p;
}

void plane_release(kc_plane *p)
{
    if (!p) return;
    if (--p->refs == 0) {
        if (p->chain) delete p->chain;
        if (p->link) delete p->link;
        if (p->rz_src) plane_release(p->rz_src);
        if (p->view_of) plane_release(p->view_of);
        if (p->owned && p->dptr) pool_free(p->dptr, p->bytes);
        delete p;
    }
}

Chain::~Chain()
{
    plane_release(start);
    for (auto &s : steps) plane_release(s.operand);
    for (auto *j : joined) plane_release(j);
}

kc_plane *saved_value_marker()
{
    static kc_plane *m = [] {
        kc_plane *p = new kc_plane();
        p->kind = kc_plane::CONST;
        p->refs = 1 << 30;
        return p;
    }();
    return m;
}

ChainLink::~ChainLink()
{
    plane_release(start);
    plane_release(step.operand);
    kc_plane *q = prev;
    prev = nullptr;
    while (q) {
        if (--q->refs != 0) break;
        kc_plane *next = nullptr;
        if (q->link) {
            next = q->link->prev;
            q->link->prev = nullptr;
        }
        q->refs = 1;
        plane_release(q);
        q = next;
    }
}

static int chain_in_limit()
{
    const Context &c = ctx();
    return (c.opt.wide && c.opt.fusion && !c.plain_chains && specialize_get_mode() != 0) ? KC_CHAIN_MAX_IN : KC_CHAIN_INTERP_IN;
}

static void link_add_input(ChainLink &L, const kc_plane *q)
{
    ChainLink::InKey k;
    if (q->kind == kc_plane::MEM)
        k = { q->dptr, q->pitch };
// ... 49 lines not shown
            uint8_t code = L->step.code;
            switch (code) {
            case CH_SUB_L: code = CH_SUB_R; break;
            case CH_SUB_R: code = CH_SUB_L; break;
            case CH_DIV_L: code = CH_DIV_R; break;
            case CH_DIV_R: code = CH_DIV_L; break;
            case CH_POW_L: code = CH_POW_R; break;
            case CH_POW_R: code = CH_POW_L; break;
            default: break;
            }
            c->steps.push_back({ code, saved_value_marker(), 0 });
            for (size_t i = sub.steps.size(); i-- > 0;) {
                ChainStep st = sub.steps[i];
                if (st.code == CH_SAVE_LOAD || st.operand == saved_value_marker()) st.level++;
                c->steps.push_back(st);
            }
            c->steps.push_back({ (uint8_t)CH_SAVE_LOAD, sub.start, 0 });
            c->joined.push_back(opnd);
            plane_retain(opnd);
        } else {
            c->steps.push_back(L->step);
        }
        if (L->prev && L->prev->kind == kc_plane::LAZY) {
            q = L->prev;
            continue;
        }
        c->start = L->prev ? L->prev : L->start;
        break;
    }
    std::reverse(c->steps.begin(), c->steps.end());
    plane_retain(c->start);
    for (auto &s : c->steps) plane_retain(s.operand);
    p->chain = c;
}

Operand plane_operand(const kc_plane *p)
{
    Operand o;
    if (p->kind == kc_plane::CONST) {
        o.ptr = nullptr;
        o.pitch = 0;
        o.c = p->cval;
    } else {
        o.ptr = p->dptr;
        o.pitch = (uint32_t)(p->pitch / sizeof(float));
        o.c = 0.0f;
    }
    return o;
}

struct BuiltChain {
    ChainProgram prog;
    uint32_t in_refs[KC_CHAIN_MAX_IN] = {};
    int mode = 0;
    kc_plane *sampled[KC_CHAIN_MAX_BATCH] = { nullptr, nullptr, nullptr, nullptr };
    bool joins = false;
};

static int input_index(std::vector<const kc_plane *> &ins, const kc_plane *p)
{
    for (size_t i = 0; i < ins.size(); ++i)
        if (ins[i] == p || (p->kind == kc_plane::MEM && ins[i]->kind == kc_plane::MEM && ins[i]->dptr == p->dptr &&
                            ins[i]->pitch == p->pitch))
            return (int)i;
    ins.push_back(p);
    return (int)ins.size() - 1;
}

static bool chain_fill(BuiltChain &bc, int b, const kc_plane *p)
{
    KC_PROF("chain_fill");
    const Chain &ch = *p->chain;
    ChainProgram &P = bc.prog;
    std::vector<const kc_plane *> ins;
    kc_plane *samp = nullptr;
    if (ch.start->kind == kc_plane::MEM) input_index(ins, ch.start);
    for (auto &st : ch.steps)
        if (st.operand->kind == kc_plane::MEM) input_index(ins, st.operand);
    auto slot = [&](kc_plane *q, float *c) -> int {
        if (q == saved_value_marker()) return KC_CHAIN_SRC_SAVED - 1;
        if (q->kind == kc_plane::MEM) return input_index(ins, q);
        if (q->kind == kc_plane::RESIZE) {
            samp = q;
            return -2;
        }
        *c = q->cval;
        return -1;
    };
    const int km = (int)ins.size();
    if (km > KC_CHAIN_MAX_IN) return false;
    float c0 = 0.0f;
    int start_src = slot(ch.start, &c0);
    if (start_src == -2) start_src = km;
    if (b == 0) {
        std::memset(&P, 0, sizeof(P));
        P.start_src = start_src;
    } else if (P.start_src != start_src) {
        return false;
    }
    P.start_c[b] = c0;
    size_t r = 0;
    for (size_t i = 0; i < ch.steps.size(); ++i, ++r) {
        const ChainStep &st = ch.steps[i];
        float c = 0.0f;
        int src = slot(st.operand, &c);
        if (src == -2) src = km;
        uint8_t code = st.code;
        if (code == CH_ADD_R) code = CH_ADD;
        if (code == CH_MUL_R) code = CH_MUL;
        if (code == CH_SAVE_LOAD) bc.joins = true;
        if (src >= 0 && code <= CH_MUL && i + 1 < ch.steps.size() && ch.steps[i + 1].code == CH_SUB_R &&
            ch.steps[i + 1].operand->kind == kc_plane::CONST && ch.steps[i + 1].operand != saved_value_marker()) {
            static const uint8_t inv[4] = { CH_ADD_INV, CH_SUBL_INV, CH_SUBR_INV, CH_MUL_INV };
            code = inv[code];
            c = ch.steps[i + 1].operand->cval;
            ++i;
        }
        uint32_t word = chain_op_word(code, src);
        if (st.code == CH_SAVE_LOAD || st.operand == saved_value_marker()) word |= (uint32_t)st.level << 16;
        auto rec = [&](int ch_) -> ChainStepRec & { return (r & 1) ? P.step[ch_][r / 2].b : P.step[ch_][r / 2].a; };
        if (b == 0) {
            rec(0).word = word;
            if (code == CH_DIV_L || code == CH_DIV_R) bc.mode = bc.mode < 1 ? 1 : bc.mode;
            if (code == CH_POW_L || code == CH_POW_R) bc.mode = 2;
        } else if (r >= P.n_ops || rec(0).word != word) {
            return false;
        }
        rec(b).word = word;
        rec(b).c = c;
    }
    if (b == 0)
        P.n_ops = (uint32_t)r;
    else if (P.n_ops != r)
        return false;
    const uint32_t n_in = (uint32_t)km + (samp ? 1u : 0u);
    if (b == 0)
        P.n_in = n_in;
    else if (P.n_in != n_in || (samp != nullptr) != (bc.sampled[0] != nullptr))
        return false;
    if (samp && b > 0) {
        const kc_plane *s0 = bc.sampled[0];
        if (samp->rz_filter != s0->rz_filter || samp->rz_src->w != s0->rz_src->w || samp->rz_src->h != s0->rz_src->h)
            return false;
    }
    bc.sampled[b] = samp;
    for (int k = 0; k < km; ++k) {
        P.in[b][k] = ins[k]->dptr;
        P.in_pitch[b][k] = (uint32_t)(ins[k]->pitch / 16);
        if (b == 0) bc.in_refs[k] = (uint32_t)ins[k]->refs;
    }
    if (samp) {
        P.samp_src[b] = samp->rz_src->dptr;
        P.samp_pitch[b] = (uint32_t)(samp->rz_src->pitch / 4);
    }
    return true;
}

static int chain_prepare(kc_plane *p)
{
    Chain &ch = *p->chain;
    kc_plane *first = nullptr;
    auto visit = [&](kc_plane *q) -> int {
        if (q->kind != kc_plane::RESIZE) return KC_OK;
        if (!first) {
            first = q;
            return KC_OK;
        }
        return q == first ? KC_OK : resize_force(q);
    };
    KC_TRY(visit(ch.start));
    for (auto &st : ch.steps) KC_TRY(visit(st.operand));
    return KC_OK;
}

uint32_t chain_cache_policy(const uint32_t *refs, uint32_t n, uint64_t stream_bytes, uint64_t out_bytes)
{
    const Options &o = options();
    if (!o.cache_policy) return 0;
    uint32_t all = 0;
    for (uint32_t k = 0; k < n; ++k) all |= KC_CHAIN_NT_BIT(k);
    if (o.nt_force >= 0) return (uint32_t)o.nt_force & (all | 0x100u);
    const uint64_t budget = (uint64_t)o.cache_budget_mb << 20;
    if (n * stream_bytes + out_bytes <= budget) return 0;
    uint32_t mask = all;
    uint64_t used = 0;
    for (;;) {
        int best = -1;
        for (uint32_t k = 0; k < n; ++k)
            if ((mask & KC_CHAIN_NT_BIT(k)) && refs[k] >= 2 && (best < 0 || refs[k] > refs[best])) best = (int)k;
        if (best < 0 || used + stream_bytes > budget) break;
        used += stream_bytes;
        mask &= ~KC_CHAIN_NT_BIT(best);
    }
    if (used + out_bytes > budget) mask |= 0x100u;
    return mask;
}

uint32_t cache_policy_mask(uint64_t in_bytes, uint64_t out_bytes, uint32_t n_resident, const Options &o)
{
    if (!o.cache_policy) return 0;
    if (o.nt_force >= 0) return (uint32_t)o.nt_force & (((1u << n_resident) - 1u) | 0x100u);
    const uint64_t budget = (uint64_t)o.cache_budget_mb << 20;
    if (in_bytes + out_bytes <= budget) return 0;
    uint32_t mask = (1u << n_resident) - 1u;
    if (out_bytes > budget) mask |= 0x100u;
    return mask;
}

namespace {
struct ChainCounterNames {
    std::string interp[5][9][3][2];
    std::string k0[3];
    std::string chain1[8];
    std::string spec[0x200], spec_q2[0x200], spec_q4[0x200];
    ChainCounterNames()
    {
        char buf[64];
        for (int k = 1; k <= 4; ++k)
            for (int u : { 1, 2, 4, 6, 8 })
                for (int m = 0; m < 3; ++m)
                    for (int nt = 0; nt < 2; ++nt) {
                        std::snprintf(buf, sizeof buf, "chain_interp_k%d_u%d_m%d%s", k, u, m, nt ? "_nt" : "");
                        interp[k][u][m][nt] = buf;
                    }
        for (int m = 0; m < 3; ++m) k0[m] = "chain_k0_m" + std::to_string(m);
        for (int b = 0; b < 8; ++b) chain1[b] = "chain1_nt" + std::to_string(b);
        for (int b = 0; b < 0x200; ++b) {
            std::snprintf(buf, sizeof buf, "specialized_nt_%03x", b);
            spec[b] = buf;
            spec_q2[b] = spec[b] + "_q2";
            spec_q4[b] = spec[b] + "_q4";
        }
    }
};
const ChainCounterNames &chain_counter_names()
{
    static const ChainCounterNames n;
    return n;
}
}

hipError_t chain_dispatch(ChainProgram &P, int batch, int mode, uint32_t w, uint32_t h, size_t out_pitch_bytes)
{
    Context &c = ctx();
    const uint32_t row_units = (w + 3) / 4;
    bool launched = false;
    bool dense = (size_t)row_units * 16 == out_pitch_bytes;
    for (int b = 0; b < batch && dense; ++b)
        for (uint32_t k = 0; k < P.n_in; ++k)
            if (P.in_pitch[b][k] != row_units) dense = false;
    if (dense) {
        P.rows = 1;
        P.row_units = row_units * h;
    } else {
        P.rows = h;
        P.row_units = row_units;
    }
    if (!launched && P.n_ops == 1 && c.opt.chain1) {
        Chain1Args a{};
        const uint32_t w0 = P.step[0][0].a.word, from = w0 >> 8;
        for (int b = 0; b < batch; ++b) {
            if (P.start_src >= 0) {
                a.start[b] = P.in[b][P.start_src];
                a.start_pitch[b] = P.in_pitch[b][P.start_src];
            }
            a.start_c[b] = P.start_c[b];
            if (from) {
                a.operand[b] = P.in[b][from - 1];
                a.operand_pitch[b] = P.in_pitch[b][from - 1];
            }
            a.operand_c[b] = a.c[b] = P.step[b][0].a.c;
            a.out[b] = P.out[b];
            a.out_pitch[b] = P.out_pitch[b];
        }
        a.rows = P.rows;
        a.row_units = P.row_units;
        const unsigned nt = (P.start_src >= 0 && (P.nt_mask >> P.start_src & 1u) ? 1u : 0u) | (from && (P.nt_mask >> (from - 1) & 1u) ? 2u : 0u) |
                            (P.nt_mask & 0x100u ? 4u : 0u);
        unsigned launched_nt = ~0u;
        hipError_t e = launch_chain1(a, batch, (int)(w0 & 0xffu), nt, c.stream, &launched_nt);
        if (e != hipSuccess) return e;
        c.counters["chain1_launches"]++;
        if (launched_nt < 8) c.counters[chain_counter_names().chain1[launched_nt]]++;
        launched = true;
    }
    if (!launched) {
        uint32_t spec_nt = 0, spec_quads = 1;
        hipError_t e = launch_chain_specialized(P, batch, c.stream, &launched, &spec_nt, &spec_quads);
        if (e == hipSuccess && launched) {
            const ChainCounterNames &names = chain_counter_names();
            c.counters[(spec_quads == 2 ? names.spec_q2 : spec_quads == 4 ? names.spec_q4 : names.spec)[spec_nt & 0x1ffu]]++;
        }
        if (e == hipSuccess && !launched) {
            if (P.n_in > (uint32_t)KC_CHAIN_INTERP_IN) return hipErrorNotReady;
            for (uint32_t i = 0; i < P.n_ops; ++i)
                if ((((i & 1u) ? P.step[0][i / 2].b.word : P.step[0][i / 2].a.word) & 0xffu) == CH_SAVE_LOAD) return hipErrorNotReady;
            ChainVariant v;
            e = launch_chain(P, batch, mode, c.opt.max_blocks, c.opt.chain_unroll, c.stream, &v);
            if (e == hipSuccess && v.k == 0) c.counters[chain_counter_names().k0[v.mode]]++;
            else if (e == hipSuccess && v.k > 0) c.counters[chain_counter_names().interp[v.k][v.u][v.mode][v.nt ? 1 : 0]]++;
        }
        if (e != hipSuccess) return e;
    }
    return hipSuccess;
}

static int chain_flatten_to_fit(kc_plane *p, int limit);
static_assert(sizeof(ChainProgram) <= 4096, "a launch passes at most 4 KB of kernel arguments");

static int chain_launch(BuiltChain &bc, kc_plane *const *planes, int batch)
{
    KC_PROF("chain_launch");
    Context &c = ctx();
    ChainProgram &P = bc.prog;
    const kc_plane *p0 = planes[0];
    std::vector<kc_plane *> outs(batch, nullptr);
    for (int b = 0; b < batch; ++b) {
        int s = plane_new_mem(p0->w, p0->h, &outs[b]);
        if (s != KC_OK) {
            for (auto *o : outs) plane_release(o);
            return s;
        }
        P.out[b] = outs[b]->dptr;
        P.out_pitch[b] = (uint32_t)(outs[b]->pitch / 16);
    }
    {
        const uint64_t px4 = 4ull * p0->w * p0->h;
        const uint32_t resident = P.n_in - (bc.sampled[0] ? 1u : 0u);
        P.nt_mask = chain_cache_policy(bc.in_refs, resident, px4 * batch, px4 * batch);
    }
    bool launched = false;
    if (bc.sampled[0]) {
        int s = chain_resize_launch(P, batch, bc.mode, bc.sampled, &launched);
        if (s != KC_OK || !launched) {
            for (auto *o : outs) plane_release(o);
            if (s != KC_OK) return s;
            KC_TRY(resize_force_many(bc.sampled, batch));
            return KC_RETRY_CHAIN;
        }
    }
    if (!launched) {
        hipError_t e = chain_dispatch(P, batch, bc.mode, p0->w, p0->h, outs[0]->pitch);
        if (e == hipErrorNotReady && (bc.joins || P.n_in > (uint32_t)KC_CHAIN_INTERP_IN)) {
            for (auto *o : outs) plane_release(o);
            std::vector<kc_plane *> subs;
            for (size_t j = 0; j < planes[0]->chain->joined.size(); ++j)
                for (int b = 0; b < batch; ++b)
                    if (j < planes[b]->chain->joined.size()) subs.push_back(planes[b]->chain->joined[j]);
            if (!subs.empty()) KC_TRY(planes_force(subs.data(), (int)subs.size()));
            for (int b = 0; b < batch; ++b) {
                if (planes[b]->kind != kc_plane::LAZY) continue;
                delete planes[b]->chain;
                planes[b]->chain = nullptr;
                KC_TRY(chain_flatten_to_fit(planes[b], KC_CHAIN_INTERP_IN));
            }
            c.counters["join_fallbacks"]++;
            if (c.capture) c.capture->ok = false;
            return KC_RETRY_CHAIN;
        }
        if (e != hipSuccess) {
            for (auto *o : outs) plane_release(o);
            return hip_fail(e, "launch_chain");
        }
        if (bc.joins) c.counters["join_launches"]++;
        if (P.n_in > (uint32_t)KC_CHAIN_INTERP_IN) c.counters["wide_launches"]++;
    }
    c.launches++;
    {
        uint64_t px = (uint64_t)p0->w * p0->h, bytes = 0;
        for (int b = 0; b < batch; ++b) {
            const uint32_t resident = P.n_in - (bc.sampled[b] ? 1u : 0u);
            bytes += 4 * px * (resident + 1);
            if (bc.sampled[b]) bytes += 4 * (uint64_t)bc.sampled[b]->rz_src->w * bc.sampled[b]->rz_src->h;
        }
        c.alg_bytes += bytes;
    }
    if (c.capture) {
        ReplayCapture &cap = *c.capture;
        if (bc.sampled[0] || cap.launches.size() >= 32) cap.ok = false;
        else {
            cap.launches.emplace_back();
            ReplayLaunch &L = cap.launches.back();
            L.prog = P;
            L.batch = batch;
            L.mode = bc.mode;
            std::memcpy(L.in_refs, bc.in_refs, sizeof L.in_refs);
            L.w = p0->w;
            L.h = p0->h;
            for (int b = 0; b < batch; ++b) L.planes[b] = planes[b];
        }
    }
    for (int b = 0; b < batch; ++b) {
        kc_plane *p = planes[b];
        Chain *old = p->chain;
        ChainLink *old_link = p->link;
        p->chain = nullptr;
        p->link = nullptr;
        p->kind = kc_plane::MEM;
        p->dptr = outs[b]->dptr;
        p->pitch = outs[b]->pitch;
        p->bytes = outs[b]->bytes;
        p->owned = true;
        outs[b]->owned = false;
        outs[b]->dptr = nullptr;
        plane_release(outs[b]);
        delete old;
        delete old_link;
    }
    return KC_OK;
}

static int chain_flatten_to_fit(kc_plane *p, int limit)
{
    chain_flatten(p);
    while (chain_distinct_inputs(*p->chain) > limit || chain_record_count(*p->chain) > (size_t)KC_CHAIN_MAX_OPS) {
        if (!p->chain->joined.empty()) {
            std::vector<kc_plane *> subs(p->chain->joined);
            for (auto *q : subs) plane_retain(q);
            const int fs = planes_force(subs.data(), (int)subs.size());
            for (auto *q : subs) plane_release(q);
            KC_TRY(fs);
            if (p->kind != kc_plane::LAZY) return KC_OK;
            delete p->chain;
            p->chain = nullptr;
            chain_flatten(p);
            continue;
        }
        kc_plane *prev = p->link->prev;
        if (!prev || prev->kind != kc_plane::LAZY) {
            set_error("chain with more inputs than a program holds cannot be split");
            return KC_ERR_UNSUPPORTED;
        }
        {
            std::vector<kc_plane *> path;
            for (kc_plane *q = prev; q && q->kind == kc_plane::LAZY; q = q->link->prev) path.push_back(q);
            std::reverse(path.begin(), path.end());
            std::vector<ChainLink::InKey> keys;
            auto add = [&](const kc_plane *q) {
                ChainLink::InKey k;
                if (q->kind == kc_plane::MEM) k = { q->dptr, q->pitch };
                else if (q->kind == kc_plane::RESIZE) k = { q, ~(size_t)0 };
                else return;
// ... 328 lines not shown
```

### kanter_core_amd/csrc/specialize.cpp

```cpp
#include <dlfcn.h>
#include <sys/stat.h>
#include <unistd.h>

#include <condition_variable>
#include <cstdio>
#include <cstdlib>
#include <cstring>
#include <thread>

#include "kc_runtime.hpp"

namespace kc {

extern const char kJitChainProgramH[];
extern const char kJitPowPositiveInc[];
extern const char kJitUpsampleH[];
extern const char kJitUpsampleChainInc[];

namespace {

typedef struct _hiprtcProgram *hiprtcProgram;
struct Rtc {
    void *lib = nullptr;
    int (*create)(hiprtcProgram *, const char *, const char *, int, const char **, const char **) = nullptr;
    int (*compile)(hiprtcProgram, int, const char **) = nullptr;
    int (*log_size)(hiprtcProgram, size_t *) = nullptr;
    int (*log)(hiprtcProgram, char *) = nullptr;
    int (*code_size)(hiprtcProgram, size_t *) = nullptr;
    int (*code)(hiprtcProgram, char *) = nullptr;
    int (*destroy)(hiprtcProgram *) = nullptr;
    int (*version)(int *, int *) = nullptr;
    bool ok = false;
    bool tried = false;
};

void specialize_stop_at_exit();

Rtc &rtc()
{
    static Rtc r;
    static std::once_flag once;
    std::call_once(once, [] {
        r.tried = true;
        for (const char *name : { "libhiprtc.so", "libhiprtc.so.7", "/opt/rocm/lib/libhiprtc.so" }) {
            r.lib = dlopen(name, RTLD_NOW | RTLD_LOCAL);
            if (r.lib) break;
        }
        if (!r.lib) return;
#define KC_RTC_SYM(field, sym) *(void **)(&r.field) = dlsym(r.lib, sym)
        KC_RTC_SYM(create, "hiprtcCreateProgram");
        KC_RTC_SYM(compile, "hiprtcCompileProgram");
        KC_RTC_SYM(log_size, "hiprtcGetProgramLogSize");
        KC_RTC_SYM(log, "hiprtcGetProgramLog");
        KC_RTC_SYM(code_size, "hiprtcGetCodeSize");
        KC_RTC_SYM(code, "hiprtcGetCode");
        KC_RTC_SYM(destroy, "hiprtcDestroyProgram");
        KC_RTC_SYM(version, "hiprtcVersion");
#undef KC_RTC_SYM
        r.ok = r.create && r.compile && r.log_size && r.log && r.code_size && r.code && r.destroy;
        if (r.ok) std::atexit(specialize_stop_at_exit);
    });
    return r;
}

struct Signature {
    uint32_t n_in = 0, n_ops = 0;
    int32_t start_src = 0;
    bool flat = false;
    uint32_t up_taps = 0;
    bool up_wide = false;
    uint32_t nt_mask = 0;
    uint32_t quads = 1;
    uint32_t word[KC_CHAIN_MAX_OPS] = {};

    std::string key() const
    {
        std::string k((const char *)&n_in, sizeof n_in);
        k.append((const char *)&n_ops, sizeof n_ops);
        k.append((const char *)&start_src, sizeof start_src);
        k.push_back(flat ? 'f' : 'p');
        k.push_back((char)('0' + up_taps));
        k.push_back(up_wide ? 'w' : 'n');
        k.append((const char *)&nt_mask, sizeof nt_mask);
        k.append((const char *)word, sizeof(uint32_t) * n_ops);
        if (quads > 1) {
            k.push_back('q');
            k.push_back((char)('0' + quads));
        }
        return k;
    }
};

constexpr uint32_t kQuadsWarm = 2, kQuadsMaxOps = 16;
std::atomic<int> g_chain_quads{ 0 };

uint32_t chain_quads_for(const Signature &s, uint64_t total_units)
{
    if (s.up_taps || !s.flat || s.n_in < 1 || s.n_ops > kQuadsMaxOps || total_units > 0xF0000000ull) return 1;
    bool plain = false;
    for (uint32_t k = 0; k < s.n_in; ++k) plain |= !(s.nt_mask & KC_CHAIN_NT_BIT(k));
    if (!plain || !s.nt_mask) return 1;
    for (uint32_t i = 0; i < s.n_ops; ++i) {
        const uint32_t code = s.word[i] & 0xffu;
        if (code == CH_DIV_L || code == CH_DIV_R || code == CH_POW_L || code == CH_POW_R) return 1;
    }
    const int forced = g_chain_quads.load(std::memory_order_relaxed);
    return forced ? (uint32_t)forced : kQuadsWarm;
}

Signature signature_of(const ChainProgram &P, const UpsampleArgs *U = nullptr)
{
    Signature s;
    s.n_in = P.n_in;
    s.n_ops = P.n_ops;
    s.start_src = P.start_src;
    s.flat = U ? false : P.rows == 1;
    {
        uint32_t valid = 0x100u;
        for (uint32_t k = 0; k < (U ? P.n_in - 1u : P.n_in); ++k) valid |= KC_CHAIN_NT_BIT(k);
        s.nt_mask = P.nt_mask & valid;
    }
    if (U) {
        s.up_taps = U->H.taps;
        s.up_wide = U->tile_w == 1024;
    }
    for (uint32_t i = 0; i < P.n_ops; ++i) s.word[i] = (i & 1u) ? P.step[0][i / 2].b.word : P.step[0][i / 2].a.word;
    s.quads = chain_quads_for(s, (uint64_t)P.rows * P.row_units);
    return s;
}

static int spec_wg()
{
    static int wg = [] {
        int v = 256;
        if (const char *e = std::getenv("KC_SPEC_WG")) {
            const int x = std::atoi(e);
            if (x == 64 || x == 128 || x == 256 || x == 512 || x == 1024) v = x;
        }
        return v;
    }();
    return wg;
}

std::string kernel_name(const Signature &s)
{
    uint32_t h = 2166136261u;
    for (unsigned char c : s.key()) h = (h ^ c) * 16777619u;
    char buf[32];
    std::snprintf(buf, sizeof buf, s.up_taps ? "kc_upchain_%08x" : "kc_chain_%08x", h);
    return buf;
}

static const char kPackedF4[] = R"KCF4(typedef float raw4 __attribute__((ext_vector_type(4)));
typedef float f2 __attribute__((ext_vector_type(2)));
typedef unsigned long long __attribute__((may_alias)) rec64;
static __device__ __forceinline__ f2 pk_sub(f2 a, f2 b)
{
    f2 d;
    asm("v_pk_add_f32 %0, %1, %2 neg_lo:[0,1] neg_hi:[0,1]" : "=v"(d) : "v"(a), "v"(b));
    return d;
}
struct kconst {
    rec64 rec;  // { word, c }
    __device__ __forceinline__ operator float() const { return __builtin_bit_cast(float, (unsigned int)(rec >> 32)); }
    __device__ __forceinline__ f2 minus(f2 b) const
    {
        f2 d;
        asm("v_pk_add_f32 %0, %1, %2 op_sel_hi:[0,1] neg_lo:[0,1] neg_hi:[0,1]" : "=v"(d) : "s"(rec >> 32), "v"(b));
        return d;
    }
};
struct f4 {
    f2 lo, hi;
    f4() = default;
    __device__ __forceinline__ f4(float x, float y, float z, float w) : lo{ x, y }, hi{ z, w } {}
    __device__ __forceinline__ f4(f2 l, f2 h) : lo(l), hi(h) {}
    __device__ __forceinline__ f4(raw4 v) : lo(v.xy), hi(v.zw) {}
    __device__ __forceinline__ raw4 raw() const { return raw4{ lo.x, lo.y, hi.x, hi.y }; }
};
// ... 33 lines not shown
    case CH_MUL: return std::string("acc * ") + x;
    case CH_DIV_L: return std::string("acc / ") + x;
    case CH_DIV_R: return std::string(x) + " / acc";
    case CH_POW_L: return std::string("pow4(acc, ") + x + ", pow_tab)";
    case CH_POW_R: return std::string("pow4(") + x + ", acc, pow_tab)";
    case CH_ADD_INV: return std::string(c) + " - (acc + " + x + ")";
    case CH_SUBL_INV: return std::string(c) + " - (acc - " + x + ")";
    case CH_SUBR_INV: return std::string(c) + " - (" + x + " - acc)";
    case CH_MUL_INV: return std::string(c) + " - (acc * " + x + ")";
    default: return std::string();
    }
}

static std::string generate_up(const Signature &s)
{
    std::string src;
    src.reserve(32768);
    src += "namespace kc {\n";
    src += kJitChainProgramH;
    src += kJitUpsampleH;
    src += "typedef float f4 __attribute__((ext_vector_type(4)));\n";
    src += kJitUpsampleChainInc;
    char buf[320];
    std::snprintf(buf, sizeof buf,
                  "struct UpProg {\n    const ChainProgram &P;\n"
                  "    __device__ __forceinline__ void operator()(const f4 (&in)[%u][%u], f4 (&out)[%u]) const\n    {\n"
                  "        const unsigned int b = blockIdx.z;\n        const ChainStepPair *pp = P.step[b];\n"
                  "#pragma unroll\n        for (int u = 0; u < %u; ++u) {\n",
                  s.n_in, KC_UPSAMPLE_ROWS, KC_UPSAMPLE_ROWS, KC_UPSAMPLE_ROWS);
    src += buf;
    if (s.start_src < 0)
        src += "            f4 acc = f4{ P.start_c[b], P.start_c[b], P.start_c[b], P.start_c[b] };\n";
    else {
        std::snprintf(buf, sizeof buf, "            f4 acc = in[%d][u];\n", s.start_src);
        src += buf;
    }
    for (uint32_t i = 0; i < s.n_ops; ++i) {
        const uint32_t code = s.word[i] & 0xffu;
        if (code == CH_DIV_L || code == CH_DIV_R || code == CH_POW_L || code == CH_POW_R || code == CH_SAVE_LOAD) return std::string();
        const std::string e = step_expr(s, i, "in[", "][u]");
        if (e.empty()) return std::string();
        src += "            acc = " + e + ";\n";
    }
    src += "            out[u] = acc;\n        }\n    }\n};\n}  // namespace kc\nusing namespace kc;\n";
    std::snprintf(buf, sizeof buf,
                  "extern \"C\" __global__ __launch_bounds__(256) void %s(const ChainProgram P, const UpsampleArgs U)\n{\n"
                  "    extern __shared__ __attribute__((aligned(16))) float lds[];\n"
                  "    upsample_chain_tile<%u, %u, %u, %s, 0x%xu>(P, U, lds, UpProg{ P });\n}\n",
                  kernel_name(s).c_str(), s.n_in, s.up_taps, KC_UPSAMPLE_ROWS, s.up_wide ? "true" : "false", s.nt_mask);
    src += buf;
    return src;
}

static std::string generate_quads(const Signature &s, int SPEC_WG)
{
    std::string src;
    char buf[320];
    std::snprintf(buf, sizeof buf,
                  "    const unsigned int n = P.rows * P.row_units;\n"
                  "    const unsigned int idx = blockIdx.x * %uu + threadIdx.x;\n    if (idx >= n) return;\n",
                  s.quads * (uint32_t)SPEC_WG);
    src += buf;
    for (uint32_t u = 0; u < s.quads; ++u) {
        if (u == 0)
            src += "    const unsigned int at0 = idx;\n";
        else {
            std::snprintf(buf, sizeof buf, "    const unsigned int at%u = idx + %uu < n ? idx + %uu : n - 1u;\n", u, u * SPEC_WG, u * SPEC_WG);
            src += buf;
        }
        for (uint32_t k = 0; k < s.n_in; ++k) {
            if (s.nt_mask & KC_CHAIN_NT_BIT(k))
                std::snprintf(buf, sizeof buf, "    const f4 in%u_%u = __builtin_nontemporal_load(&reinterpret_cast<const raw4 *>(P.in[b][%u])[at%u]);\n", k, u, k, u);
            else
                std::snprintf(buf, sizeof buf, "    const f4 in%u_%u = reinterpret_cast<const raw4 *>(P.in[b][%u])[at%u];\n", k, u, k, u);
            src += buf;
        }
    }
    src += "    const StepTableView pp{ P.step[b] };\n";
    for (uint32_t u = 0; u < s.quads; ++u) {
        char suffix[8];
        std::snprintf(suffix, sizeof suffix, "_%u", u);
        std::snprintf(buf, sizeof buf, "    f4 out%u;\n    {\n", u);
        src += buf;
        if (s.start_src < 0)
            src += "        f4 acc = f4{ P.start_c[b], P.start_c[b], P.start_c[b], P.start_c[b] };\n";
        else {
            std::snprintf(buf, sizeof buf, "        f4 acc = in%d%s;\n", s.start_src, suffix);
            src += buf;
        }
        src += "        f4 saved0 = acc, saved1 = acc, saved2 = acc;\n";
        for (uint32_t i = 0; i < s.n_ops; ++i) {
            const std::string e = step_expr(s, i, "in", suffix);
            if (e.empty()) return std::string();
            src += "        acc = " + e + ";\n";
        }
        std::snprintf(buf, sizeof buf, "        out%u = acc;\n    }\n", u);
        src += buf;
    }
    for (uint32_t u = 0; u < s.quads; ++u) {
        std::snprintf(buf, sizeof buf, "    if (idx + %uu < n) ", u * SPEC_WG);
        src += u ? buf : "    ";
        std::snprintf(buf, sizeof buf,
                      s.nt_mask & 0x100u ? "__builtin_nontemporal_store(out%u.raw(), &reinterpret_cast<raw4 *>(P.out[b])[idx + %uu]);\n"
                                         : "reinterpret_cast<raw4 *>(P.out[b])[idx + %uu] = out%u.raw();\n",
                      s.nt_mask & 0x100u ? u : u * SPEC_WG, s.nt_mask & 0x100u ? u * SPEC_WG : u);
        src += buf;
    }
    src += "}\n";
    return src;
}

std::string generate(const Signature &s)
{
    if (s.up_taps) return generate_up(s);
    const int SPEC_WG = spec_wg();
    bool pow = false;
    for (uint32_t i = 0; i < s.n_ops; ++i) pow |= (s.word[i] & 0xffu) == CH_POW_L || (s.word[i] & 0xffu) == CH_POW_R;
    std::string src;
    src.reserve(16384);
    src += "namespace kc {\n";
    src += kJitChainProgramH;
    src += kPackedF4;
    if (pow) {
        src += kJitPowPositiveInc;
        src += "static __device__ __noinline__ float pow_general(float a, float b) { return (float)pow((double)a, (double)b); }\n"
               "static __device__ __forceinline__ float kc_powf(float a, float b, const PowCtx &pw)\n"
               "{\n"
               "    if (a > 0.0f && a < __builtin_inff() && __builtin_fabsf(b) < __builtin_inff()) return pow_positive(a, b, pw);\n"
               "    return pow_general(a, b);\n"
               "}\n"
               "static __device__ __forceinline__ f4 pow4(f4 a, f4 b, const PowCtx &t) { return f4{ kc_powf(a.lo.x, b.lo.x, t), kc_powf(a.lo.y, b.lo.y, t), kc_powf(a.hi.x, b.hi.x, t), kc_powf(a.hi.y, b.hi.y, t) }; }\n";
    }
    src += "}  // namespace kc\nusing namespace kc;\n";
    char buf[256];
    std::snprintf(buf, sizeof buf, "extern \"C\" __global__ __launch_bounds__(%d) void %s(const ChainProgram P)\n{\n", SPEC_WG,
                  kernel_name(s).c_str());
    src += buf;
    if (pow) src += "    __shared__ double pow_lds[KC_POW_TABLE_DOUBLES];\n    const PowCtx pow_tab = pow_setup(pow_lds);\n";
    src += "    const unsigned int b = blockIdx.y;\n";
    if (s.quads > 1) {
        const std::string body = generate_quads(s, SPEC_WG);
        return body.empty() ? body : src + body;
    }
    std::snprintf(buf, sizeof buf, "    const unsigned int idx = blockIdx.x * %du + threadIdx.x;\n", SPEC_WG);
    src += buf;
    src += "    if (idx >= P.rows * P.row_units) return;\n";
    if (s.flat)
        src += "    const unsigned int row = 0u, col = idx;\n";
    else
        src += "    const unsigned int row = idx / P.row_units, col = idx - row * P.row_units;\n";
    for (uint32_t k = 0; k < s.n_in; ++k) {
        if (s.nt_mask & KC_CHAIN_NT_BIT(k))
            std::snprintf(buf, sizeof buf, "    const f4 in%u = __builtin_nontemporal_load(&reinterpret_cast<const raw4 *>(P.in[b][%u])[row * P.in_pitch[b][%u] + col]);\n", k, k, k);
        else
            std::snprintf(buf, sizeof buf, "    const f4 in%u = reinterpret_cast<const raw4 *>(P.in[b][%u])[row * P.in_pitch[b][%u] + col];\n", k, k, k);
        src += buf;
    }
    src += "    const StepTableView pp{ P.step[b] };\n";
    if (s.start_src < 0)
        src += "    f4 acc = f4{ P.start_c[b], P.start_c[b], P.start_c[b], P.start_c[b] };\n";
    else {
        std::snprintf(buf, sizeof buf, "    f4 acc = in%d;\n", s.start_src);
        src += buf;
    }
    src += "    f4 saved0 = acc, saved1 = acc, saved2 = acc;\n";
    for (uint32_t i = 0; i < s.n_ops; ++i) {
        const std::string e = step_expr(s, i, "in", "");
        if (e.empty()) return std::string();
        src += "    acc = " + e + ";\n";
    }
    if (s.nt_mask & 0x100u)
        src += "    __builtin_nontemporal_store(acc.raw(), &reinterpret_cast<raw4 *>(P.out[b])[row * P.out_pitch[b] + col]);\n}\n";
    else
        src += "    reinterpret_cast<raw4 *>(P.out[b])[row * P.out_pitch[b] + col] = acc.raw();\n}\n";
    return src;
}

static const char *const kCompileOpts[] = { "--gpu-architecture=gfx950", "-O3", "-ffp-contract=off", "-fno-fast-math",
                                            "-fhip-fp32-correctly-rounded-divide-sqrt" };
constexpr int kNumCompileOpts = (int)(sizeof kCompileOpts / sizeof *kCompileOpts);

uint64_t fnv64(const void *data, size_t n, uint64_t h = 1469598103934665603ull)
{
    const unsigned char *p = (const unsigned char *)data;
    for (size_t i = 0; i < n; ++i) h = (h ^ p[i]) * 1099511628211ull;
    return h;
}

struct CacheHeader {
    char magic[8];
    uint64_t key_len, source_hash, code_len, code_hash;
};

struct DiskCache {
    std::mutex mu;
    bool resolved = false;
    std::string write_dir;
    std::vector<std::string> read_dirs;
    uint64_t hits = 0, rejected = 0, written = 0;
};

DiskCache &disk()
{
    static DiskCache d;
// ... 212 lines not shown
            stopping = true;
            for (auto &key : queue) {
                auto it = cache.find(key);
                if (it != cache.end() && it->second.state == Entry::QUEUED) {
                    it->second.state = Entry::COUNTING;
                    it->second.sightings = 0;
                }
            }
            queue.clear();
        }
        cv.notify_all();
        idle_cv.notify_all();
        if (worker.joinable()) worker.join();
        std::lock_guard<std::mutex> lk(mu);
        worker_running = false;
        stopping = false;
    }
};

Spec &spec()
{
    static Spec *s = new Spec();
    return *s;
}

void specialize_stop_at_exit() { spec().stop(); }

bool compile_entry(const Signature &sig, hipModule_t *module, hipFunction_t *fn, std::string *log, bool disk_only = false)
{
    const std::string src = generate(sig);
    if (src.empty()) {
        *log = "unknown step code";
        return false;
    }
    std::vector<char> code;
    if (disk_load(sig, src, code)) {
        if (load_code(sig, code, module, fn, log)) return true;
        std::lock_guard<std::mutex> lk(disk().mu);
        disk().hits--;
        disk().rejected++;
    }
    if (disk_only) {
        *log = "not in the kernel cache";
        return false;
    }
    if (!rtc_compile(src, code, log)) return false;
    if (!load_code(sig, code, module, fn, log)) return false;
    disk_store(sig, src, code);
    if (const char *m = std::getenv("KC_KERNEL_CACHE_MANIFEST")) {
        if (FILE *f = std::fopen(m, "a")) {
            std::fprintf(f, "{\"name\": \"%s\", \"n_in\": %u, \"start_src\": %d, \"flat\": %d, \"nt_mask\": %u, \"up_taps\": %u, \"up_wide\": %d, \"words\": [",
                         kernel_name(sig).c_str(), sig.n_in, sig.start_src, sig.flat ? 1 : 0, sig.nt_mask, sig.up_taps, sig.up_wide ? 1 : 0);
            for (uint32_t k = 0; k < sig.n_ops; ++k) std::fprintf(f, "%s%u", k ? ", " : "", sig.word[k]);
            std::fprintf(f, "]}\n");
            std::fclose(f);
        }
    }
    return true;
}

void finish(Spec &S, const std::string &key, bool ok, hipModule_t m, hipFunction_t f, const std::string &log, bool from_disk = false)
{
    auto it = S.cache.find(key);
    if (it == S.cache.end()) {
        if (ok) (void)hipModuleUnload(m);
        return;
    }
    if (ok) {
        it->second.module = m;
        it->second.fn = f;
        it->second.state = Entry::READY;
        if (from_disk) S.loaded_from_disk++;
        else S.compiled++;
    } else {
        it->second.state = Entry::FAILED;
        S.failed++;
        S.last_log = log;
    }
}

void worker_main()
{
    Spec &S = spec();
    if (S.device >= 0) (void)hipSetDevice(S.device);
    std::unique_lock<std::mutex> lk(S.mu);
    for (;;) {
        S.cv.wait(lk, [&] { return S.stopping || !S.queue.empty(); });
        if (S.stopping) return;
        const std::string key = S.queue.front();
        S.queue.pop_front();
        auto it = S.cache.find(key);
        if (it == S.cache.end()) continue;
        const Signature sig = it->second.sig;
        S.busy++;
        lk.unlock();
        hipModule_t m = nullptr;
        hipFunction_t f = nullptr;
        std::string log;
        const uint64_t hits0 = disk_hits();
        const bool ok = compile_entry(sig, &m, &f, &log);
        const bool from_disk = ok && disk_hits() != hits0;
        lk.lock();
        S.busy--;
        finish(S, key, ok, m, f, log, from_disk);
        S.idle_cv.notify_all();
    }
}

}

static uint64_t signature_hash(const Signature &s)
{
    uint64_t h = 1469598103934665603ull;
    auto mix = [&](uint64_t v) { h = (h ^ v) * 1099511628211ull; };
    mix(s.n_in);
    mix(s.n_ops);
    mix((uint64_t)(int64_t)s.start_src);
    mix(s.flat ? 1 : 0);
    mix(s.up_taps);
    mix(s.up_wide ? 1 : 0);
    mix(s.nt_mask);
    mix(s.quads);
    for (uint32_t i = 0; i < s.n_ops; ++i) mix(s.word[i]);
    return h;
}

static bool same_signature(const Signature &a, const Signature &b)
{
    return a.n_in == b.n_in && a.n_ops == b.n_ops && a.start_src == b.start_src && a.flat == b.flat && a.up_taps == b.up_taps &&
           a.up_wide == b.up_wide && a.nt_mask == b.nt_mask && a.quads == b.quads &&
           std::memcmp(a.word, b.word, sizeof(uint32_t) * a.n_ops) == 0;
}

static hipFunction_t spec_lookup(const Signature &sig)
{
    Spec &S = spec();
    if (S.mode.load(std::memory_order_relaxed) == 0) return nullptr;
    const uint64_t h = signature_hash(sig);
    {
        std::lock_guard<std::mutex> fast(S.mu);
        auto it = S.by_hash.find(h);
        if (it != S.by_hash.end() && it->second.second->state == Entry::READY && same_signature(it->second.second->sig, sig))
            return it->second.second->fn;
    }
    const std::string key = sig.key();
    std::unique_lock<std::mutex> lk(S.mu);
    if (S.mode == 2) {
        auto it = S.cache.find(key);
        if (it != S.cache.end() && it->second.state == Entry::QUEUED)
            S.idle_cv.wait(lk, [&] { return S.cache[key].state != Entry::QUEUED || !S.worker_running; });
    }
    Entry &e = S.cache[key];
    if (e.state == Entry::READY) {
        e.sig = sig;
        S.by_hash[h] = { key, &e };
        return e.fn;
    }
    if (e.state != Entry::COUNTING) return nullptr;
    e.sightings++;
    if (e.sightings == 1 && S.mode == 1) {
        hipModule_t m = nullptr;
        hipFunction_t f = nullptr;
        std::string log;
        e.sig = sig;
        if (compile_entry(sig, &m, &f, &log, true)) {
            e.module = m;
            e.fn = f;
            e.state = Entry::READY;
            S.loaded_from_disk++;
            S.by_hash[h] = { key, &e };
            return f;
        }
    }
    if (S.mode == 1 && e.sightings < S.after) return nullptr;
    e.sig = sig;
    if (S.mode == 2) {
        e.state = Entry::QUEUED;
        lk.unlock();
        hipModule_t m = nullptr;
        hipFunction_t f = nullptr;
        std::string log;
        const uint64_t hits0 = disk_hits();
        const bool ok = compile_entry(sig, &m, &f, &log);
        const bool from_disk = ok && disk_hits() != hits0;
        lk.lock();
        finish(S, key, ok, m, f, log, from_disk);
        return ok ? f : nullptr;
    }
    e.state = Entry::QUEUED;
    S.queue.push_back(key);
    if (!S.worker_running) {
        S.device = ctx().device;
        S.stopping = false;
        S.worker = std::thread(worker_main);
        S.worker_running = true;
    }
    lk.unlock();
    S.cv.notify_one();
    return nullptr;
}

hipError_t launch_chain_specialized(const ChainProgram &P, int batch, hipStream_t s, bool *launched, uint32_t *nt_mask, uint32_t *quads)
{
    *launched = false;
    if (P.n_ops < 1 || P.n_ops > (uint32_t)KC_CHAIN_MAX_OPS || P.n_in > (uint32_t)KC_CHAIN_MAX_IN) return hipSuccess;
    const uint64_t total = (uint64_t)P.rows * P.row_units;
    if (total == 0 || total > 0xFFFFFFFFull) return hipSuccess;
    const Signature sig = signature_of(P);
    hipFunction_t fn = spec_lookup(sig);
    if (!fn) return hipSuccess;
    size_t size = sizeof(ChainProgram);
    const int SPEC_WG = spec_wg();
    void *extra[] = { HIP_LAUNCH_PARAM_BUFFER_POINTER, (void *)&P, HIP_LAUNCH_PARAM_BUFFER_SIZE, &size, HIP_LAUNCH_PARAM_END };
    const uint64_t per_block = (uint64_t)SPEC_WG * sig.quads;
    const unsigned gx = (unsigned)((total + per_block - 1) / per_block);
    hipError_t e = hipModuleLaunchKernel(fn, gx, (unsigned)batch, 1, SPEC_WG, 1, 1, 0, s, nullptr, extra);
    if (e == hipSuccess) {
        *launched = true;
        if (nt_mask) *nt_mask = sig.nt_mask;
        if (quads) *quads = sig.quads;
        std::lock_guard<std::mutex> lk(spec().mu);
        spec().launches++;
    }
    return e;
}

hipError_t launch_upsample_chain_specialized(const ChainProgram &P, int batch, const UpsampleArgs &U, hipStream_t s, bool *launched)
{
    *launched = false;
    if (P.n_ops < 1 || P.n_ops > (uint32_t)KC_CHAIN_MAX_OPS || P.n_in < 1 || P.n_in > (uint32_t)KC_CHAIN_INTERP_IN) return hipSuccess;
    if (!upsample_args_ok(U, batch) || (U.H.taps != 1 && U.H.taps != 3)) return hipSuccess;
    if (U.H.ratio == 2) return hipSuccess;
    hipFunction_t fn = spec_lookup(signature_of(P, &U));
    if (!fn) return hipSuccess;
    struct alignas(16) Params {
        ChainProgram P;
        UpsampleArgs U;
    };
    static_assert(sizeof(ChainProgram) % alignof(UpsampleArgs) == 0, "the second kernel argument follows the first without padding");
    static thread_local Params params;
    params.P = P;
    params.U = U;
    size_t size = sizeof(Params);
    void *extra[] = { HIP_LAUNCH_PARAM_BUFFER_POINTER, (void *)&params, HIP_LAUNCH_PARAM_BUFFER_SIZE, &size, HIP_LAUNCH_PARAM_END };
    const dim3 grid = upsample_grid(U, batch);
    hipError_t e = hipModuleLaunchKernel(fn, grid.x, grid.y, grid.z, 256, 1, 1, (unsigned)upsample_lds_bytes(U), s, nullptr, extra);
    if (e == hipSuccess) {
        *launched = true;
        std::lock_guard<std::mutex> lk(spec().mu);
        spec().launches++;
    }
    return e;
}

int specialize_set_mode(int mode, int after)
{
    Spec &S = spec();
    if (mode < 0 || mode > 2) return KC_ERR_INVALID_ARG;
    {
        std::lock_guard<std::mutex> lk(S.mu);
        S.mode.store(mode);
        if (after >= 1) S.after = (uint32_t)after;
    }
    if (mode == 0) S.stop();
    return KC_OK;
}

int specialize_get_mode()
{
    Spec &S = spec();
    return S.mode.load();
}

void specialize_wait()
{
    Spec &S = spec();
    std::unique_lock<std::mutex> lk(S.mu);
    S.idle_cv.wait(lk, [&] { return S.stopping || (S.queue.empty() && S.busy == 0); });
// ... 47 lines not shown
    const std::string src = generate(signature_of(P, U));
    if (src.empty()) return KC_ERR_GENERIC;
    std::vector<char> code;
    return rtc_compile(src, code, log) ? KC_OK : KC_ERR_GENERIC;
}

int kernel_cache_set_dir(const char *dir)
{
    DiskCache &d = disk();
    std::lock_guard<std::mutex> lk(d.mu);
    resolve_dirs_locked(d, dir && *dir ? dir : nullptr);
    return KC_OK;
}

void kernel_cache_stats(uint64_t *hits, uint64_t *rejected, uint64_t *written, uint64_t *kernels_loaded)
{
    {
        DiskCache &d = disk();
        std::lock_guard<std::mutex> lk(d.mu);
        if (hits) *hits = d.hits;
        if (rejected) *rejected = d.rejected;
        if (written) *written = d.written;
    }
    Spec &S = spec();
    std::lock_guard<std::mutex> lk(S.mu);
    if (kernels_loaded) *kernels_loaded = S.loaded_from_disk;
}

bool kernel_cache_populated()
{
    DiskCache &d = disk();
    std::vector<std::string> dirs;
    {
        std::lock_guard<std::mutex> lk(d.mu);
        if (!d.resolved) resolve_dirs_locked(d, nullptr);
        dirs = d.read_dirs;
        if (dirs.empty()) return false;
        if (d.hits) return true;
    }
    static std::map<std::string, bool> seen;
    for (auto &dir : dirs) {
        auto it = seen.find(dir);
        if (it == seen.end()) {
            bool any = false;
            std::string probe = dir + "/.populated";
            any = access(probe.c_str(), R_OK) == 0;
            it = seen.emplace(dir, any).first;
        }
        if (it->second) return true;
    }
    return false;
}

int kernel_cache_precompile(const uint32_t *words, uint32_t n_ops, uint32_t n_in, int32_t start_src, bool flat, uint32_t nt_mask,
                            uint32_t up_taps, bool up_wide, const char *dir, std::string *log)
{
    if (!words || n_ops < 1 || n_ops > (uint32_t)KC_CHAIN_MAX_OPS || n_in > (uint32_t)KC_CHAIN_MAX_IN || !dir || !*dir) return KC_ERR_INVALID_ARG;
    Signature sig;
    sig.n_in = n_in;
    sig.n_ops = n_ops;
    sig.start_src = start_src;
    sig.flat = flat;
    sig.nt_mask = nt_mask;
    sig.up_taps = up_taps;
    sig.up_wide = up_wide;
    for (uint32_t i = 0; i < n_ops; ++i) sig.word[i] = words[i];
    sig.quads = chain_quads_for(sig, 0);
    const std::string src = generate(sig);
    if (src.empty()) {
        *log = "unknown step code";
        return KC_ERR_INVALID_ARG;
    }
    std::vector<char> code;
    if (!rtc_compile(src, code, log)) return rtc().ok ? KC_ERR_GENERIC : KC_ERR_UNSUPPORTED;
    if (!make_dirs(dir) || !disk_store_in(dir, sig, src, code)) {
        *log = std::string("cannot write into ") + dir;
        return KC_ERR_IO;
    }
    if (FILE *f = std::fopen((std::string(dir) + "/.populated").c_str(), "w")) std::fclose(f);
    return KC_OK;
}

}
```

Baseline: 6.370 million.

## Pack reused chain input planes into lossless u8/fixed24 shadows to cut read bandwidth

Adds an optional source-packing path. Input planes read by two or more chain programs get packed once into a compact shadow copy, u8 at 4 bytes per quad or fixed24 at 12 bytes per quad, but only when the packing kernel reports the conversion is exact. Specialized JIT chain kernels then load and decode the packed shadow instead of the full f32x4 data, which lowers memory traffic in bandwidth-bound chains. This costs extra packing passes with a host sync, shadow memory up to a budget, and more kernel signatures to compile. Shadows are dropped when the plane is uploaded to or its device pointer is exposed.

```diff
diff --git a/bindings/rust/kanter_core_amd_sys.rs b/bindings/rust/kanter_core_amd_sys.rs
--- a/bindings/rust/kanter_core_amd_sys.rs
+++ b/bindings/rust/kanter_core_amd_sys.rs
@@ -151,6 +151,11 @@
     pub fn kc_kernel_cache_stats(files_accepted: *mut u64, files_refused: *mut u64, files_written: *mut u64, kernels_loaded: *mut u64) -> i32;
     pub fn kc_kernel_cache_precompile(words: *const u32, n_ops: u32, n_in: u32, start_src: i32, flat: i32, nt_mask: u32, up_taps: u32, up_wide: i32, dir: *const c_char) -> i32;
     pub fn kc_specialize_reset() -> i32;
+    pub fn kc_kernel_cache_precompile_packed(words: *const u32, n_ops: u32, n_in: u32, start_src: i32, flat: i32, nt_mask: u32, in_tiers: u32, dir: *const c_char) -> i32;
+    pub fn kc_set_pack_sources(mode: i32) -> i32;
+    pub fn kc_get_pack_sources() -> i32;
+    pub fn kc_set_pack_budget_mb(mb: i32) -> i32;
+    pub fn kc_get_pack_budget_mb() -> i32;
     pub fn kc_plane_alloc(width: u32, height: u32, out: *mut *mut KcPlane) -> i32;
     pub fn kc_plane_const(width: u32, height: u32, value: f32, out: *mut *mut KcPlane) -> i32;
     pub fn kc_plane_wrap(device_ptr: *mut c_void, width: u32, height: u32, pitch_bytes: usize, out: *mut *mut KcPlane) -> i32;
diff --git a/include/kanter_core_amd.h b/include/kanter_core_amd.h
--- a/include/kanter_core_amd.h
+++ b/include/kanter_core_amd.h
@@ -116,6 +116,12 @@
 KC_API int kc_kernel_cache_precompile(const uint32_t *words, uint32_t n_ops, uint32_t n_in, int start_src, int flat, uint32_t nt_mask,
                                       uint32_t up_taps, int up_wide, const char *dir);
 KC_API int kc_specialize_reset(void);
+KC_API int kc_kernel_cache_precompile_packed(const uint32_t *words, uint32_t n_ops, uint32_t n_in, int start_src, int flat,
+                                             uint32_t nt_mask, uint32_t in_tiers, const char *dir);
+KC_API int kc_set_pack_sources(int mode);
+KC_API int kc_get_pack_sources(void);
+KC_API int kc_set_pack_budget_mb(int mb);
+KC_API int kc_get_pack_budget_mb(void);
 
 KC_API int kc_plane_alloc(uint32_t width, uint32_t height, kc_plane **out);
 KC_API int kc_plane_const(uint32_t width, uint32_t height, float value, kc_plane **out);
diff --git a/kanter_core_amd/__init__.py b/kanter_core_amd/__init__.py
--- a/kanter_core_amd/__init__.py
+++ b/kanter_core_amd/__init__.py
@@ -4,7 +4,7 @@
                   init, is_initialized, mix_process, resize_image, separate_rgba_process, set_fusion, set_stream,
                   shutdown, stats, sync, value_process, set_specialize, get_specialize, specialize_wait,
                   specialize_stats, specialize_compile_check, Partition, PartitionPolicy, NodeKind, set_resize_mode,
-                  get_resize_mode, resize_upsample_plan, resize_down2_plan, stats_counter, specialize_compile_check_upsample, specialize_compile_check_mask, set_chain_quads, get_chain_quads, set_cache_policy, get_cache_policy, set_option, get_option, comm_unique_id, comm_init,
+                  get_resize_mode, resize_upsample_plan, resize_down2_plan, stats_counter, specialize_compile_check_upsample, specialize_compile_check_mask, set_chain_quads, get_chain_quads, set_pack_sources, get_pack_sources, set_pack_budget_mb, get_pack_budget_mb, set_cache_policy, get_cache_policy, set_option, get_option, comm_unique_id, comm_init,
                   comm_destroy, comm_info, comm_stats, comm_transport, comm_gather_bands, PlanKind, pool_trim, kernel_cache_set_dir, kernel_cache_stats,
                   kernel_cache_precompile, specialize_reset, U8Pipe, device_image_desc, DEVICE_SRGB, DEVICE_GRAY,
                   ChannelStats, STATS_HISTOGRAM, STATS_SRGB, BC_SRGB, BC6H, BC7, BC_BLOCK_BYTES,
diff --git a/kanter_core_amd/_lib.py b/kanter_core_amd/_lib.py
--- a/kanter_core_amd/_lib.py
+++ b/kanter_core_amd/_lib.py
@@ -115,6 +115,11 @@
     "kc_specialize_compile_check": (C.c_int, [c_u32p, C.c_uint32, C.c_uint32, C.c_int, C.c_int, C.c_char_p, C.c_size_t]),
     "kc_specialize_compile_check_mask": (C.c_int, [c_u32p, C.c_uint32, C.c_uint32, C.c_int, C.c_int, C.c_uint32, C.c_char_p, C.c_size_t]),
     "kc_set_chain_quads": (C.c_int, [C.c_int]),
+    "kc_set_pack_sources": (C.c_int, [C.c_int]),
+    "kc_get_pack_sources": (C.c_int, []),
+    "kc_set_pack_budget_mb": (C.c_int, [C.c_int]),
+    "kc_get_pack_budget_mb": (C.c_int, []),
+    "kc_kernel_cache_precompile_packed": (C.c_int, [C.POINTER(C.c_uint32), C.c_uint32, C.c_uint32, C.c_int, C.c_int, C.c_uint32, C.c_uint32, C.c_char_p]),
     "kc_get_chain_quads": (C.c_int, []),
     "kc_specialize_compile_check_upsample": (C.c_int, [c_u32p, C.c_uint32, C.c_uint32, C.c_int, C.c_uint32, C.c_int, C.c_char_p,
                                                        C.c_size_t]),
diff --git a/kanter_core_amd/api.py b/kanter_core_amd/api.py
--- a/kanter_core_amd/api.py
+++ b/kanter_core_amd/api.py
@@ -215,6 +215,22 @@
     return _lib.load().kc_get_chain_quads()
 
 
+def set_pack_sources(mode):
+    _check(_lib.load().kc_set_pack_sources(int(mode)))
+
+
+def get_pack_sources():
+    return _lib.load().kc_get_pack_sources()
+
+
+def set_pack_budget_mb(mb):
+    _check(_lib.load().kc_set_pack_budget_mb(int(mb)))
+
+
+def get_pack_budget_mb():
+    return _lib.load().kc_get_pack_budget_mb()
+
+
 def specialize_compile_check_upsample(words, n_in, start_src=0, taps=3, wide=True):
     arr = (C.c_uint32 * len(words))(*words)
     buf = C.create_string_buffer(1 << 17)
@@ -241,8 +257,14 @@
     return dict(zip(("files_accepted", "files_refused", "files_written", "kernels_loaded"), (x.value for x in v)))
 
 
-def kernel_cache_precompile(words, n_in, start_src, flat, nt_mask, directory, up_taps=0, up_wide=False):
+def kernel_cache_precompile(words, n_in, start_src, flat, nt_mask, directory, up_taps=0, up_wide=False, in_tiers=0):
     arr = (C.c_uint32 * len(words))(*words)
+    if in_tiers:
+        if up_taps:
+            raise ValueError("packed inputs: plain chain programs only")
+        _check(_lib.load().kc_kernel_cache_precompile_packed(arr, len(words), int(n_in), int(start_src), int(bool(flat)), int(nt_mask),
+                                                             int(in_tiers), str(directory).encode()))
+        return
     _check(_lib.load().kc_kernel_cache_precompile(arr, len(words), int(n_in), int(start_src), int(bool(flat)), int(nt_mask),
                                                   int(up_taps), int(bool(up_wide)), str(directory).encode()))
 
diff --git a/kanter_core_amd/build.py b/kanter_core_amd/build.py
--- a/kanter_core_amd/build.py
+++ b/kanter_core_amd/build.py
@@ -10,12 +10,12 @@
 SOURCES = ["chain.hip", "upsample.hip", "resize_tile.hip", "resize_down.hip", "h2n.hip", "u8.hip", "chain1.hip", "down2.hip", "runtime.cpp",
            "ops.cpp", "resize.cpp", "graph.cpp", "json.cpp", "png.cpp", "specialize.cpp", "partition.cpp", "bands.cpp", "comm.cpp", "replay.cpp",
            "u8pipe.cpp", "devimage.hip", "devimage.cpp", "stats.hip", "stats.cpp", "bc.hip", "bc7.hip", "bc6h.hip", "bc.cpp", "mip.hip", "mip.cpp", "bc_decode.hip",
-           "bc_decode.cpp", "bc_modes.hip",
+           "bc_decode.cpp", "bc_modes.hip", "chain_pack.hip", "chain_pack.cpp",
            "c_api.cpp"]
-HEADERS = ["kc_internal.hpp", "kc_runtime.hpp", "chain_program.h", os.path.join("..", "..", "include", "kanter_core_amd.h"), "pow_positive.inc",
+HEADERS = ["kc_internal.hpp", "kc_runtime.hpp", "chain_program.h", "chain_pack.h", os.path.join("..", "..", "include", "kanter_core_amd.h"), "pow_positive.inc",
            "srgb_thresholds.inc", "streaming.h", "bc_blocks.h", "bc_modes.h", "upsample.h", "upsample_chain.inc", "chain_apply.inc", "chain_interp.inc", "resample.inc"]
 JIT_TEXTS = [("kJitChainProgramH", "chain_program.h"), ("kJitPowPositiveInc", "pow_positive.inc"), ("kJitUpsampleH", "upsample.h"),
-             ("kJitUpsampleChainInc", "upsample_chain.inc")]
+             ("kJitUpsampleChainInc", "upsample_chain.inc"), ("kJitChainPackH", "chain_pack.h")]
 
 FLAGS = ["--offload-arch=gfx950", "-O3", "-std=c++17", "-fPIC", "-fvisibility=hidden", "-fno-fast-math",
          "-ffp-contract=off", "-fhip-fp32-correctly-rounded-divide-sqrt", "-Wall", "-Wno-unused-result"]
@@ -128,12 +128,19 @@
     L.kc_kernel_cache_precompile.argtypes = [C.POINTER(C.c_uint32), C.c_uint32, C.c_uint32, C.c_int, C.c_int, C.c_uint32, C.c_uint32,
                                              C.c_int, C.c_char_p]
     L.kc_kernel_cache_precompile.restype = C.c_int
+    L.kc_kernel_cache_precompile_packed.argtypes = [C.POINTER(C.c_uint32), C.c_uint32, C.c_uint32, C.c_int, C.c_int, C.c_uint32, C.c_uint32,
+                                                    C.c_char_p]
+    L.kc_kernel_cache_precompile_packed.restype = C.c_int
     L.kc_last_error.restype = C.c_char_p
 
     def one(e):
         words = (C.c_uint32 * len(e["words"]))(*e["words"])
-        rc = L.kc_kernel_cache_precompile(words, len(e["words"]), e["n_in"], e["start_src"], e["flat"], e["nt_mask"], e["up_taps"],
-                                          e["up_wide"], KERNEL_CACHE.encode())
+        if e.get("in_tiers"):
+            rc = L.kc_kernel_cache_precompile_packed(words, len(e["words"]), e["n_in"], e["start_src"], e["flat"], e["nt_mask"],
+                                                     e["in_tiers"], KERNEL_CACHE.encode())
+        else:
+            rc = L.kc_kernel_cache_precompile(words, len(e["words"]), e["n_in"], e["start_src"], e["flat"], e["nt_mask"], e["up_taps"],
+                                              e["up_wide"], KERNEL_CACHE.encode())
         if rc != 0:
             raise RuntimeError("pre-compiling %s failed (%d): %s" % (e.get("name"), rc, (L.kc_last_error() or b"").decode(errors="replace")))
         if verbose:
diff --git a/kanter_core_amd/csrc/c_api.cpp b/kanter_core_amd/csrc/c_api.cpp
--- a/kanter_core_amd/csrc/c_api.cpp
+++ b/kanter_core_amd/csrc/c_api.cpp
@@ -435,11 +435,62 @@
 try {
     KC_ARG(words && dir);
     std::string log;
-    const int s = kernel_cache_precompile(words, n_ops, n_in, start_src, flat != 0, nt_mask, up_taps, up_wide != 0, dir, &log);
+    const int s = kernel_cache_precompile(words, n_ops, n_in, start_src, flat != 0, nt_mask, 0, up_taps, up_wide != 0, dir, &log);
     if (s != KC_OK) set_error("kernel cache: " + log);
     return s;
 }
 KC_CATCH
+
+int kc_kernel_cache_precompile_packed(const uint32_t *words, uint32_t n_ops, uint32_t n_in, int start_src, int flat, uint32_t nt_mask,
+                                      uint32_t in_tiers, const char *dir)
+try {
+    KC_ARG(words && dir);
+    std::string log = "in_tiers: two bits per input plane, 0 to 2, flat programs only";
+    const int s = kernel_cache_precompile(words, n_ops, n_in, start_src, flat != 0, nt_mask, in_tiers, 0, false, dir, &log);
+    if (s != KC_OK) set_error("kernel cache: " + log);
+    return s;
+}
+KC_CATCH
+
+int kc_set_pack_sources(int mode)
+try {
+    Lock lk(ctx().mu);
+    if (mode < 0 || mode > 2) {
+        set_error("kc_set_pack_sources accepts 0, 1 or 2");
+        return KC_ERR_INVALID_ARG;
+    }
+    ctx().pack_sources = mode;
+    return KC_OK;
+}
+KC_CATCH
+
+int kc_get_pack_sources(void)
+try {
+    return ctx().pack_sources;
+}
+catch (...) {
+    return 0;
+}
+
+int kc_set_pack_budget_mb(int mb)
+try {
+    Lock lk(ctx().mu);
+    if (mb < 0) {
+        set_error("kc_set_pack_budget_mb accepts 0 and up");
+        return KC_ERR_INVALID_ARG;
+    }
+    ctx().pack_budget_mb = mb;
+    return KC_OK;
+}
+KC_CATCH
+
+int kc_get_pack_budget_mb(void)
+try {
+    return ctx().pack_budget_mb;
+}
+catch (...) {
+    return 0;
+}
 
 int kc_specialize_reset(void)
 try {
@@ -606,6 +657,10 @@
 try {
     KC_ARG(p);
     KC_TRY(plane_materialize(p));
+    {
+        Lock lk(ctx().mu);
+        plane_shadow_drop(p, true);
+    }
     if (dptr) *dptr = p->dptr;
     if (pitch) *pitch = p->pitch;
     return KC_OK;
@@ -618,6 +673,7 @@
     KC_ARG(p && host && p->kind == kc_plane::MEM);
     if (host_pitch == 0) host_pitch = (size_t)p->w * 4;
     Lock lk(ctx().mu);
+    plane_shadow_drop(p, false);
     KC_HIP(hipMemcpy2DAsync(p->dptr, p->pitch, host, host_pitch, (size_t)p->w * 4, p->h, hipMemcpyHostToDevice, ctx().stream));
     KC_HIP(hipStreamSynchronize(ctx().stream));
     return KC_OK;
diff --git a/kanter_core_amd/csrc/chain_pack.cpp b/kanter_core_amd/csrc/chain_pack.cpp
--- /dev/null
+++ b/kanter_core_amd/csrc/chain_pack.cpp
@@ -0,0 +1,120 @@
+#include "kc_runtime.hpp"
+
+namespace kc {
+
+uint32_t pack_bytes_per_quad(uint32_t tier) { return tier == (uint32_t)KC_PACK_FIX24 ? 12u : tier == (uint32_t)KC_PACK_U8 ? 4u : 16u; }
+
+void plane_shadow_drop(kc_plane *p, bool never_again)
+{
+    if (p->shadow) {
+        Context &c = ctx();
+        pool_free(p->shadow, p->shadow_bytes);
+        c.shadow_bytes -= p->shadow_bytes;
+        c.counters["packed_bytes"] = c.shadow_bytes;
+        p->shadow = nullptr;
+        p->shadow_bytes = 0;
+    }
+    p->pack_tier = KC_PACK_NONE;
+    p->pack_seen = 0;
+    p->pack_state = never_again ? kc_plane::PACK_NEVER : kc_plane::PACK_UNTRIED;
+}
+
+static bool plane_packable(const kc_plane *p, uint32_t w, uint32_t h)
+{
+    return p && p->kind == kc_plane::MEM && p->owned && !p->view_of && p->dptr && p->w == w && p->h == h && w % 4 == 0 &&
+           (p->pitch == (size_t)w * 4 || h == 1) && p->pack_state != kc_plane::PACK_NEVER;
+}
+
+static size_t shadow_block(uint64_t quads, uint32_t tier) { return (size_t)((quads * pack_bytes_per_quad(tier) + 255) / 256 * 256); }
+
+static void pack_slot(kc_plane *const *planes, int n)
+{
+    Context &c = ctx();
+    const uint64_t quads = (uint64_t)planes[0]->w * planes[0]->h / 4;
+    const uint64_t budget = (uint64_t)c.pack_budget_mb << 20;
+    if (c.shadow_bytes + (uint64_t)n * shadow_block(quads, KC_PACK_U8) > budget) return;
+    static const uint32_t kTiers[2] = { KC_PACK_U8, KC_PACK_FIX24 };
+    void *blk[KC_CHAIN_MAX_BATCH][2] = {};
+    PoolStaging flags;
+    uint32_t host[KC_CHAIN_MAX_BATCH][2];
+    bool ok = flags.alloc(sizeof host) == KC_OK && hipMemsetAsync(flags.ptr, 0, sizeof host, c.stream) == hipSuccess;
+    for (int i = 0; i < n && ok; ++i)
+        for (int t = 0; t < 2 && ok; ++t) {
+            ok = pool_alloc(shadow_block(quads, kTiers[t]), &blk[i][t]) == KC_OK &&
+                 launch_pack_plane(kTiers[t], planes[i]->dptr, blk[i][t], quads, (uint32_t *)flags.ptr + 2 * i + t, c.stream) == hipSuccess;
+        }
+    ok = ok && hipMemcpyAsync(host, flags.ptr, sizeof host, hipMemcpyDeviceToHost, c.stream) == hipSuccess;
+    ok = hipStreamSynchronize(c.stream) == hipSuccess && ok;
+    c.counters["pack_passes"] += 2 * (uint64_t)n;
+    c.alg_bytes += (uint64_t)n * quads * (16 + 4 + 16 + 12);
+    int keep = -1;
+    for (int t = 0; t < 2 && ok && keep < 0; ++t) {
+        bool all = true;
+        for (int i = 0; i < n; ++i) all = all && host[i][t] == 0;
+        if (all) keep = t;
+    }
+    if (!ok) (void)hipGetLastError();
+    if (ok && keep < 0) c.counters["pack_rejected"] += (uint64_t)n;
+    if (keep >= 0 && c.shadow_bytes + (uint64_t)n * shadow_block(quads, kTiers[keep]) > budget) keep = -1;
+    for (int i = 0; i < n; ++i) {
+        for (int t = 0; t < 2; ++t)
+            if (blk[i][t] && t != keep) pool_free(blk[i][t], shadow_block(quads, kTiers[t]));
+        kc_plane *p = planes[i];
+        if (keep < 0) {
+            p->pack_state = kc_plane::PACK_NEVER;
+            continue;
+        }
+        p->shadow = blk[i][keep];
+        p->shadow_bytes = shadow_block(quads, kTiers[keep]);
+        p->pack_tier = (uint8_t)kTiers[keep];
+        p->pack_state = kc_plane::PACKED;
+        c.shadow_bytes += p->shadow_bytes;
+        c.counters["packed_planes"]++;
+    }
+    c.counters["packed_bytes"] = c.shadow_bytes;
+}
+
+uint32_t pack_chain_inputs(const ChainProgram &P, int batch, kc_plane *const (*src)[KC_CHAIN_MAX_IN], const uint32_t *refs, uint32_t w, uint32_t h)
+{
+    Context &c = ctx();
+    const int mode = c.pack_sources;
+    if (!mode || !src || !refs || batch < 1 || batch > (int)KC_CHAIN_MAX_BATCH) return 0;
+    const uint64_t px4 = 4ull * w * h * (uint64_t)batch;
+    if (mode == 1 && (uint64_t)P.n_in * px4 + px4 <= ((uint64_t)c.opt.cache_budget_mb << 20)) return 0;
+    struct Slot {
+        kc_plane *todo[KC_CHAIN_MAX_BATCH];
+        int n_todo = 0;
+        bool ok = false;
+    } slots[KC_CHAIN_MAX_IN];
+    bool due = true;
+    for (uint32_t k = 0; k < P.n_in; ++k) {
+        Slot &sl = slots[k];
+        if (refs[k] < 2) continue;
+        sl.ok = true;
+        for (int b = 0; b < batch && sl.ok; ++b) {
+            kc_plane *p = src[b][k];
+            sl.ok = plane_packable(p, w, h) && (const float *)p->dptr == P.in[b][k];
+            if (!sl.ok || p->pack_state == kc_plane::PACKED) continue;
+            bool seen = false;
+            for (int i = 0; i < sl.n_todo; ++i) seen = seen || sl.todo[i] == p;
+            if (seen) continue;
+            sl.todo[sl.n_todo++] = p;
+            if (p->pack_seen < 255) ++p->pack_seen;
+            if (mode == 1 && p->pack_seen < 2) due = false;
+        }
+    }
+    if (!due) return 0;
+    uint32_t tiers = 0;
+    for (uint32_t k = 0; k < P.n_in; ++k) {
+        Slot &sl = slots[k];
+        if (!sl.ok) continue;
+        if (sl.n_todo) pack_slot(sl.todo, sl.n_todo);
+        uint32_t tier = src[0][k]->pack_state == kc_plane::PACKED ? src[0][k]->pack_tier : 0u;
+        for (int b = 1; b < batch; ++b)
+            if (src[b][k]->pack_state != kc_plane::PACKED || src[b][k]->pack_tier != tier) tier = 0;
+        tiers |= tier << (2 * k);
+    }
+    return tiers;
+}
+
+}
diff --git a/kanter_core_amd/csrc/chain_pack.h b/kanter_core_amd/csrc/chain_pack.h
--- /dev/null
+++ b/kanter_core_amd/csrc/chain_pack.h
@@ -0,0 +1,40 @@
+typedef float pack_f4 __attribute__((ext_vector_type(4)));
+typedef unsigned int pack_u3 __attribute__((ext_vector_type(3)));
+typedef pack_u3 __attribute__((aligned(4))) pack_u3a;
+
+static __device__ __forceinline__ pack_u3 pack_encode_fix24(pack_f4 x)
+{
+    unsigned int k[4];
+#pragma unroll
+    for (int i = 0; i < 4; ++i)
+        k[i] = (unsigned int)__builtin_fminf(__builtin_fmaxf(x[i] * 16777216.0f, 0.0f), 16777215.0f);
+    return pack_u3{ k[0] | k[1] << 24, k[1] >> 8 | k[2] << 16, k[2] >> 16 | k[3] << 8 };
+}
+
+static __device__ __forceinline__ pack_f4 pack_decode_fix24(pack_u3 v)
+{
+    const unsigned int k0 = v.x & 0xffffffu, k1 = __builtin_amdgcn_alignbit(v.y, v.x, 24) & 0xffffffu,
+                       k2 = __builtin_amdgcn_alignbit(v.z, v.y, 16) & 0xffffffu, k3 = v.z >> 8;
+    return pack_f4{ (float)k0, (float)k1, (float)k2, (float)k3 } * 0x1p-24f;
+}
+
+static __device__ __forceinline__ unsigned int pack_encode_u8(pack_f4 x)
+{
+    unsigned int k[4];
+#pragma unroll
+    for (int i = 0; i < 4; ++i) k[i] = (unsigned int)__builtin_fminf(__builtin_fmaxf(__builtin_rintf(x[i] * 255.0f), 0.0f), 255.0f);
+    return k[0] | k[1] << 8 | k[2] << 16 | k[3] << 24;
+}
+
+static __device__ __forceinline__ pack_f4 pack_decode_u8(unsigned int v)
+{
+    const float r = 1.0f / 255.0f;
+    const pack_f4 x = pack_f4{ (float)(v & 0xffu), (float)(v >> 8 & 0xffu), (float)(v >> 16 & 0xffu), (float)(v >> 24) };
+    const pack_f4 q = x * r;
+    pack_f4 e, out;
+#pragma unroll
+    for (int i = 0; i < 4; ++i) e[i] = __builtin_fmaf(-255.0f, q[i], x[i]);
+#pragma unroll
+    for (int i = 0; i < 4; ++i) out[i] = __builtin_fmaf(e[i], r, q[i]);
+    return out;
+}
diff --git a/kanter_core_amd/csrc/chain_pack.hip b/kanter_core_amd/csrc/chain_pack.hip
--- /dev/null
+++ b/kanter_core_amd/csrc/chain_pack.hip
@@ -0,0 +1,41 @@
+#include <hip/hip_runtime.h>
+
+#include "kc_internal.hpp"
+
+namespace kc {
+
+#include "chain_pack.h"
+
+template <int TIER>
+__global__ __launch_bounds__(256) void pack_plane_kernel(const float *__restrict__ src, void *__restrict__ dst, uint64_t quads, uint32_t *flag)
+{
+    const uint64_t q = (uint64_t)blockIdx.x * 256u + threadIdx.x;
+    if (q >= quads) return;
+    typedef unsigned int u4 __attribute__((ext_vector_type(4)));
+    const pack_f4 x = reinterpret_cast<const pack_f4 *>(src)[q];
+    pack_f4 back;
+    if (TIER == KC_PACK_FIX24) {
+        const pack_u3 v = pack_encode_fix24(x);
+        *reinterpret_cast<pack_u3a *>(static_cast<char *>(dst) + q * 12u) = v;
+        back = pack_decode_fix24(v);
+    } else {
+        const unsigned int v = pack_encode_u8(x);
+        static_cast<unsigned int *>(dst)[q] = v;
+        back = pack_decode_u8(v);
+    }
+    const u4 a = __builtin_bit_cast(u4, x), b = __builtin_bit_cast(u4, back);
+    if (a.x != b.x || a.y != b.y || a.z != b.z || a.w != b.w) *flag = 1u;
+}
+
+hipError_t launch_pack_plane(uint32_t tier, const float *src, void *dst, uint64_t quads, uint32_t *flag, hipStream_t s)
+{
+    if (quads == 0 || quads > 0x7fffffffull * 256u || (tier != (uint32_t)KC_PACK_FIX24 && tier != (uint32_t)KC_PACK_U8)) return hipErrorInvalidValue;
+    const dim3 grid((unsigned)((quads + 255u) / 256u));
+    if (tier == (uint32_t)KC_PACK_FIX24)
+        hipLaunchKernelGGL(pack_plane_kernel<KC_PACK_FIX24>, grid, dim3(256), 0, s, src, dst, quads, flag);
+    else
+        hipLaunchKernelGGL(pack_plane_kernel<KC_PACK_U8>, grid, dim3(256), 0, s, src, dst, quads, flag);
+    return hipGetLastError();
+}
+
+}
diff --git a/kanter_core_amd/csrc/chain_program.h b/kanter_core_amd/csrc/chain_program.h
--- a/kanter_core_amd/csrc/chain_program.h
+++ b/kanter_core_amd/csrc/chain_program.h
@@ -1,5 +1,7 @@
 enum { KC_CHAIN_MAX_OPS = 80, KC_CHAIN_MAX_IN = 16, KC_CHAIN_INTERP_IN = 4, KC_CHAIN_MAX_BATCH = 4 };
 #define KC_CHAIN_NT_BIT(k) ((k) < 8 ? 1u << (k) : 1u << ((k) + 8))
+enum { KC_PACK_NONE = 0, KC_PACK_FIX24 = 1, KC_PACK_U8 = 2 };
+#define KC_CHAIN_TIER(tiers, k) (((tiers) >> (2 * (k))) & 3u)
 
 enum ChainCode : unsigned char {
     CH_ADD = 0,
@@ -35,6 +37,7 @@
     unsigned int rows;
     int start_src;
     unsigned int nt_mask;
+    unsigned int in_tiers;
     const float *in[KC_CHAIN_MAX_BATCH][KC_CHAIN_MAX_IN];
     unsigned int in_pitch[KC_CHAIN_MAX_BATCH][KC_CHAIN_MAX_IN];
     float *out[KC_CHAIN_MAX_BATCH];
diff --git a/kanter_core_amd/csrc/kc_internal.hpp b/kanter_core_amd/csrc/kc_internal.hpp
--- a/kanter_core_amd/csrc/kc_internal.hpp
+++ b/kanter_core_amd/csrc/kc_internal.hpp
@@ -194,6 +194,7 @@
                         uint8_t *dst, uint32_t nt_mask, hipStream_t s, bool *launched_nt);
 hipError_t launch_from_u8(const uint8_t *src, int channels, uint32_t w, uint32_t h, float *const planes[4],
                           uint32_t pitch, uint32_t nt_mask, hipStream_t s, bool *launched_nt);
+hipError_t launch_pack_plane(uint32_t tier, const float *src, void *dst, uint64_t quads, uint32_t *flag, hipStream_t s);
 struct DevImageArgs {
     const char *ptr;
     uint64_t row_pitch, channel_pitch;
diff --git a/kanter_core_amd/csrc/kc_runtime.hpp b/kanter_core_amd/csrc/kc_runtime.hpp
--- a/kanter_core_amd/csrc/kc_runtime.hpp
+++ b/kanter_core_amd/csrc/kc_runtime.hpp
@@ -89,6 +89,10 @@
     kc_plane *view_of = nullptr;
     kc_plane *rz_src = nullptr;
     int rz_filter = 0;
+    enum PackState : uint8_t { PACK_UNTRIED = 0, PACKED = 1, PACK_NEVER = 2 };
+    void *shadow = nullptr;
+    size_t shadow_bytes = 0;
+    uint8_t pack_tier = 0, pack_state = PACK_UNTRIED, pack_seen = 0;
 };
 
 struct kc_image : kc::Pooled<kc_image> {
@@ -165,6 +169,7 @@
     uint32_t in_refs[KC_CHAIN_MAX_IN] = {};
     uint32_t w = 0, h = 0;
     kc_plane *planes[KC_CHAIN_MAX_BATCH] = { nullptr, nullptr, nullptr, nullptr };
+    kc_plane *in_plane[KC_CHAIN_MAX_BATCH][KC_CHAIN_MAX_IN] = {};
     int in_from[KC_CHAIN_MAX_BATCH][KC_CHAIN_MAX_IN];
     int in_ch[KC_CHAIN_MAX_BATCH][KC_CHAIN_MAX_IN];
 };
@@ -186,6 +191,8 @@
     std::multimap<size_t, void *> free_blocks;
     uint64_t bytes_in_use = 0, bytes_cached = 0, launches = 0;
     std::map<std::string, uint64_t> counters;
+    int pack_sources = 1, pack_budget_mb = 4096;
+    uint64_t shadow_bytes = 0;
     uint64_t alg_bytes = 0;
     std::map<std::tuple<uint32_t, uint32_t, int>, TapsEntry> taps;
     std::map<std::tuple<uint32_t, uint32_t, int, int32_t, int32_t, int32_t>, TapsEntry> band_taps;
@@ -379,7 +386,12 @@
 hipError_t launch_chain_specialized(const ChainProgram &P, int batch, hipStream_t s, bool *launched, uint32_t *nt_mask, uint32_t *quads = nullptr);
 uint32_t cache_policy_mask(uint64_t in_bytes, uint64_t out_bytes, uint32_t n_resident, const Options &o = options());
 uint32_t chain_cache_policy(const uint32_t *refs, uint32_t n, uint64_t stream_bytes, uint64_t out_bytes);
-hipError_t chain_dispatch(ChainProgram &P, int batch, int mode, uint32_t w, uint32_t h, size_t out_pitch_bytes);
+hipError_t chain_dispatch(ChainProgram &P, int batch, int mode, uint32_t w, uint32_t h, size_t out_pitch_bytes,
+                          kc_plane *const (*src)[KC_CHAIN_MAX_IN] = nullptr, const uint32_t *refs = nullptr, uint64_t *packed_saved = nullptr);
+uint32_t pack_chain_inputs(const ChainProgram &P, int batch, kc_plane *const (*src)[KC_CHAIN_MAX_IN], const uint32_t *refs, uint32_t w, uint32_t h);
+void plane_shadow_drop(kc_plane *p, bool never_again);
+uint32_t pack_bytes_per_quad(uint32_t tier);
+bool chain_pack_program_ok(const ChainProgram &P);
 hipError_t launch_upsample_chain_specialized(const ChainProgram &P, int batch, const UpsampleArgs &U, hipStream_t s, bool *launched);
 int specialize_set_mode(int mode, int after);
 int specialize_get_mode();
@@ -394,7 +406,7 @@
 int kernel_cache_set_dir(const char *dir);
 void kernel_cache_stats(uint64_t *hits, uint64_t *rejected, uint64_t *written, uint64_t *kernels_loaded);
 bool kernel_cache_populated();
-int kernel_cache_precompile(const uint32_t *words, uint32_t n_ops, uint32_t n_in, int32_t start_src, bool flat, uint32_t nt_mask,
+int kernel_cache_precompile(const uint32_t *words, uint32_t n_ops, uint32_t n_in, int32_t start_src, bool flat, uint32_t nt_mask, uint32_t in_tiers,
                             uint32_t up_taps, bool up_wide, const char *dir, std::string *log);
 
 int u8_pipe_create(uint32_t w, uint32_t h, int channels, int depth, kc_u8_pipe **out);
diff --git a/kanter_core_amd/csrc/replay.cpp b/kanter_core_amd/csrc/replay.cpp
--- a/kanter_core_amd/csrc/replay.cpp
+++ b/kanter_core_amd/csrc/replay.cpp
@@ -104,6 +104,7 @@
     for (size_t li = 0; li < e->launches.size(); ++li) {
         const ReplayLaunch &L = e->launches[li];
         ChainProgram P = L.prog;
+        kc_plane *src[KC_CHAIN_MAX_BATCH][KC_CHAIN_MAX_IN] = {};
         for (int b = 0; b < L.batch; ++b) {
             kc_plane *&o = outs[li * KC_CHAIN_MAX_BATCH + b];
             int s = plane_new_mem(L.w, L.h, &o);
@@ -115,14 +116,17 @@
             P.out_pitch[b] = (uint32_t)(o->pitch / 16);
             for (uint32_t k = 0; k < P.n_in; ++k)
                 if (L.in_from[b][k] >= 0) {
-                    const kc_plane *src = outs[(size_t)L.in_from[b][k] * KC_CHAIN_MAX_BATCH + L.in_ch[b][k]];
-                    P.in[b][k] = src->dptr;
-                    P.in_pitch[b][k] = (uint32_t)(src->pitch / 16);
+                    const kc_plane *res = outs[(size_t)L.in_from[b][k] * KC_CHAIN_MAX_BATCH + L.in_ch[b][k]];
+                    P.in[b][k] = res->dptr;
+                    P.in_pitch[b][k] = (uint32_t)(res->pitch / 16);
+                } else {
+                    src[b][k] = L.in_plane[b][k];
                 }
         }
         const uint64_t px4 = 4ull * L.w * L.h;
         P.nt_mask = chain_cache_policy(L.in_refs, P.n_in, px4 * L.batch, px4 * L.batch);
-        hipError_t he = chain_dispatch(P, L.batch, L.mode, L.w, L.h, outs[li * KC_CHAIN_MAX_BATCH]->pitch);
+        uint64_t packed_saved = 0;
+        hipError_t he = chain_dispatch(P, L.batch, L.mode, L.w, L.h, outs[li * KC_CHAIN_MAX_BATCH]->pitch, src, L.in_refs, &packed_saved);
         if (he == hipErrorNotReady) {
             drop_outs();
             return KC_OK;
@@ -132,7 +136,7 @@
             return hip_fail(he, "launch_chain (replay)");
         }
         c.launches++;
-        c.alg_bytes += (uint64_t)L.batch * px4 * (P.n_in + 1);
+        c.alg_bytes += (uint64_t)L.batch * px4 * (P.n_in + 1) - packed_saved;
     }
     c.counters["replayed_evaluations"]++;
 
@@ -163,12 +167,16 @@
     uint64_t launches0 = 0;
     std::unordered_set<uint32_t> changed0;
     std::set<const void *> resident0;
+    std::set<const kc_plane *> resident_planes;
 };
 
-static void note_resident(std::set<const void *> &set, const kc_image *img)
+static void note_resident(ReplayRecorder &r, const kc_image *img)
 {
     for (int p = 0; p < img->n; ++p)
-        if (img->planes[p]->kind == kc_plane::MEM) set.insert(img->planes[p]->dptr);
+        if (img->planes[p]->kind == kc_plane::MEM) {
+            r.resident0.insert(img->planes[p]->dptr);
+            r.resident_planes.insert(img->planes[p]);
+        }
 }
 
 ReplayRecorder *replay_begin(kc_live_graph &lg, uint32_t id)
@@ -187,7 +195,7 @@
             if (sd.node_id == id) continue;
             image_retain(sd.image);
             e->pre_slots.push_back({ sd.node_id, sd.slot_id, sd.image });
-            note_resident(r->resident0, sd.image);
+            note_resident(*r, sd.image);
         }
     for (auto &em : lg.embedded) {
         if (em.full_h != 0) {
@@ -197,7 +205,7 @@
         }
         image_retain(em.image);
         e->embedded.push_back(em);
-        note_resident(r->resident0, em.image);
+        note_resident(*r, em.image);
     }
     r->launches0 = c.launches;
     r->changed0 = lg.changed;
@@ -289,6 +297,7 @@
                             L.in_ch[b][k] = bj;
                         }
                 if (L.in_from[b][k] < 0 && !r->resident0.count(L.prog.in[b][k])) return;
+                if (L.in_from[b][k] >= 0 || !r->resident_planes.count(L.in_plane[b][k])) L.in_plane[b][k] = nullptr;
             }
     }
     for (uint32_t ch : lg.changed)
diff --git a/kanter_core_amd/csrc/runtime.cpp b/kanter_core_amd/csrc/runtime.cpp
--- a/kanter_core_amd/csrc/runtime.cpp
+++ b/kanter_core_amd/csrc/runtime.cpp
@@ -237,6 +237,7 @@
         if (p->link) delete p->link;
         if (p->rz_src) plane_release(p->rz_src);
         if (p->view_of) plane_release(p->view_of);
+        if (p->shadow) plane_shadow_drop(p, false);
         if (p->owned && p->dptr) pool_free(p->dptr, p->bytes);
         delete p;
     }
@@ -392,6 +393,7 @@
 struct BuiltChain {
     ChainProgram prog;
     uint32_t in_refs[KC_CHAIN_MAX_IN] = {};
+    kc_plane *in_plane[KC_CHAIN_MAX_BATCH][KC_CHAIN_MAX_IN] = {};
     int mode = 0;
     kc_plane *sampled[KC_CHAIN_MAX_BATCH] = { nullptr, nullptr, nullptr, nullptr };
     bool joins = false;
@@ -489,6 +491,7 @@
         P.in_pitch[b][k] = (uint32_t)(ins[k]->pitch / 16);
         if (b == 0) bc.in_refs[k] = (uint32_t)ins[k]->refs;
     }
+    for (int k = 0; k < KC_CHAIN_MAX_IN; ++k) bc.in_plane[b][k] = k < km ? const_cast<kc_plane *>(ins[k]) : nullptr;
     if (samp) {
         P.samp_src[b] = samp->rz_src->dptr;
         P.samp_pitch[b] = (uint32_t)(samp->rz_src->pitch / 4);
@@ -553,6 +556,7 @@
     std::string k0[3];
     std::string chain1[8];
     std::string spec[0x200], spec_q2[0x200], spec_q4[0x200];
+    std::string spec_pk[0x200], spec_q2_pk[0x200], spec_q4_pk[0x200];
     ChainCounterNames()
     {
         char buf[64];
@@ -570,6 +574,9 @@
             spec[b] = buf;
             spec_q2[b] = spec[b] + "_q2";
             spec_q4[b] = spec[b] + "_q4";
+            spec_pk[b] = spec[b] + "_pk";
+            spec_q2_pk[b] = spec_q2[b] + "_pk";
+            spec_q4_pk[b] = spec_q4[b] + "_pk";
         }
     }
 };
@@ -580,8 +587,10 @@
 }
 }
 
-hipError_t chain_dispatch(ChainProgram &P, int batch, int mode, uint32_t w, uint32_t h, size_t out_pitch_bytes)
-{
+hipError_t chain_dispatch(ChainProgram &P, int batch, int mode, uint32_t w, uint32_t h, size_t out_pitch_bytes,
+                          kc_plane *const (*src)[KC_CHAIN_MAX_IN], const uint32_t *refs, uint64_t *packed_saved)
+{
+    if (packed_saved) *packed_saved = 0;
     Context &c = ctx();
     const uint32_t row_units = (w + 3) / 4;
     bool launched = false;
@@ -626,10 +635,32 @@
     }
     if (!launched) {
         uint32_t spec_nt = 0, spec_quads = 1;
-        hipError_t e = launch_chain_specialized(P, batch, c.stream, &launched, &spec_nt, &spec_quads);
-        if (e == hipSuccess && launched) {
-            const ChainCounterNames &names = chain_counter_names();
-            c.counters[(spec_quads == 2 ? names.spec_q2 : spec_quads == 4 ? names.spec_q4 : names.spec)[spec_nt & 0x1ffu]]++;
+        hipError_t e = hipSuccess;
+        const uint32_t tiers = src && c.pack_sources && chain_pack_program_ok(P) ? pack_chain_inputs(P, batch, src, refs, w, h) : 0u;
+        if (tiers) {
+            ChainProgram Q = P;
+            Q.in_tiers = tiers;
+            uint64_t saved = 0;
+            for (uint32_t k = 0; k < P.n_in; ++k)
+                if (const uint32_t t = KC_CHAIN_TIER(tiers, k))
+                    for (int b = 0; b < batch; ++b) {
+                        Q.in[b][k] = (const float *)src[b][k]->shadow;
+                        saved += (uint64_t)w * h / 4 * (16 - pack_bytes_per_quad(t));
+                    }
+            e = launch_chain_specialized(Q, batch, c.stream, &launched, &spec_nt, &spec_quads);
+            if (e == hipSuccess && launched) {
+                const ChainCounterNames &names = chain_counter_names();
+                c.counters[(spec_quads == 2 ? names.spec_q2_pk : spec_quads == 4 ? names.spec_q4_pk : names.spec_pk)[spec_nt & 0x1ffu]]++;
+                c.counters["packed_launches"]++;
+                if (packed_saved) *packed_saved = saved;
+            }
+        }
+        if (e == hipSuccess && !launched) {
+            e = launch_chain_specialized(P, batch, c.stream, &launched, &spec_nt, &spec_quads);
+            if (e == hipSuccess && launched) {
+                const ChainCounterNames &names = chain_counter_names();
+                c.counters[(spec_quads == 2 ? names.spec_q2 : spec_quads == 4 ? names.spec_q4 : names.spec)[spec_nt & 0x1ffu]]++;
+            }
         }
         if (e == hipSuccess && !launched) {
             if (P.n_in > (uint32_t)KC_CHAIN_INTERP_IN) return hipErrorNotReady;
@@ -670,6 +701,7 @@
         P.nt_mask = chain_cache_policy(bc.in_refs, resident, px4 * batch, px4 * batch);
     }
     bool launched = false;
+    uint64_t packed_saved = 0;
     if (bc.sampled[0]) {
         int s = chain_resize_launch(P, batch, bc.mode, bc.sampled, &launched);
         if (s != KC_OK || !launched) {
@@ -680,7 +712,7 @@
         }
     }
     if (!launched) {
-        hipError_t e = chain_dispatch(P, batch, bc.mode, p0->w, p0->h, outs[0]->pitch);
+        hipError_t e = chain_dispatch(P, batch, bc.mode, p0->w, p0->h, outs[0]->pitch, bc.in_plane, bc.in_refs, &packed_saved);
         if (e == hipErrorNotReady && (bc.joins || P.n_in > (uint32_t)KC_CHAIN_INTERP_IN)) {
             for (auto *o : outs) plane_release(o);
             std::vector<kc_plane *> subs;
@@ -713,7 +745,7 @@
             bytes += 4 * px * (resident + 1);
             if (bc.sampled[b]) bytes += 4 * (uint64_t)bc.sampled[b]->rz_src->w * bc.sampled[b]->rz_src->h;
         }
-        c.alg_bytes += bytes;
+        c.alg_bytes += bytes - packed_saved;
     }
     if (c.capture) {
         ReplayCapture &cap = *c.capture;
@@ -728,6 +760,7 @@
             L.w = p0->w;
             L.h = p0->h;
             for (int b = 0; b < batch; ++b) L.planes[b] = planes[b];
+            std::memcpy(L.in_plane, bc.in_plane, sizeof L.in_plane);
         }
     }
     for (int b = 0; b < batch; ++b) {
diff --git a/kanter_core_amd/csrc/specialize.cpp b/kanter_core_amd/csrc/specialize.cpp
--- a/kanter_core_amd/csrc/specialize.cpp
+++ b/kanter_core_amd/csrc/specialize.cpp
@@ -16,6 +16,7 @@
 extern const char kJitPowPositiveInc[];
 extern const char kJitUpsampleH[];
 extern const char kJitUpsampleChainInc[];
+extern const char kJitChainPackH[] __attribute__((weak));
 
 namespace {
 
@@ -71,6 +72,7 @@
     bool up_wide = false;
     uint32_t nt_mask = 0;
     uint32_t quads = 1;
+    uint32_t in_tiers = 0;
     uint32_t word[KC_CHAIN_MAX_OPS] = {};
 
     std::string key() const
@@ -87,6 +89,10 @@
             k.push_back('q');
             k.push_back((char)('0' + quads));
         }
+        if (in_tiers) {
+            k.push_back('t');
+            k.append((const char *)&in_tiers, sizeof in_tiers);
+        }
         return k;
     }
 };
@@ -106,6 +112,16 @@
     }
     const int forced = g_chain_quads.load(std::memory_order_relaxed);
     return forced ? (uint32_t)forced : kQuadsWarm;
+}
+
+bool pack_program_ok(const ChainProgram &P)
+{
+    if (P.n_ops < 1 || P.n_ops > kQuadsMaxOps || P.n_in < 1 || P.rows != 1) return false;
+    for (uint32_t i = 0; i < P.n_ops; ++i) {
+        const uint32_t code = ((i & 1u) ? P.step[0][i / 2].b.word : P.step[0][i / 2].a.word) & 0xffu;
+        if (code == CH_DIV_L || code == CH_DIV_R || code == CH_POW_L || code == CH_POW_R) return false;
+    }
+    return true;
 }
 
 Signature signature_of(const ChainProgram &P, const UpsampleArgs *U = nullptr)
@@ -125,6 +141,7 @@
         s.up_wide = U->tile_w == 1024;
     }
     for (uint32_t i = 0; i < P.n_ops; ++i) s.word[i] = (i & 1u) ? P.step[0][i / 2].b.word : P.step[0][i / 2].a.word;
+    if (!U && s.flat) s.in_tiers = P.n_in >= 16 ? P.in_tiers : P.in_tiers & ((1u << (2 * P.n_in)) - 1u);
     s.quads = chain_quads_for(s, (uint64_t)P.rows * P.row_units);
     return s;
 }
@@ -264,6 +281,22 @@
     return src;
 }
 
+static std::string load_expr(const Signature &s, uint32_t k, const std::string &at)
+{
+    const uint32_t tier = KC_CHAIN_TIER(s.in_tiers, k);
+    const bool nt = (s.nt_mask & KC_CHAIN_NT_BIT(k)) != 0;
+    const std::string in = "P.in[b][" + std::to_string(k) + "]";
+    std::string ptr;
+    if (tier == (uint32_t)KC_PACK_FIX24)
+        ptr = "reinterpret_cast<const pack_u3a *>(reinterpret_cast<const char *>(" + in + ") + (unsigned long long)(" + at + ") * 12u)";
+    else if (tier == (uint32_t)KC_PACK_U8)
+        ptr = "&reinterpret_cast<const unsigned int *>(" + in + ")[" + at + "]";
+    else
+        ptr = "&reinterpret_cast<const raw4 *>(" + in + ")[" + at + "]";
+    const std::string v = nt ? "__builtin_nontemporal_load(" + ptr + ")" : "*(" + ptr + ")";
+    return tier == (uint32_t)KC_PACK_FIX24 ? "pack_decode_fix24(" + v + ")" : tier == (uint32_t)KC_PACK_U8 ? "pack_decode_u8(" + v + ")" : v;
+}
+
 static std::string generate_quads(const Signature &s, int SPEC_WG)
 {
     std::string src;
@@ -281,6 +314,10 @@
             src += buf;
         }
         for (uint32_t k = 0; k < s.n_in; ++k) {
+            if (KC_CHAIN_TIER(s.in_tiers, k)) {
+                src += "    const f4 in" + std::to_string(k) + "_" + std::to_string(u) + " = " + load_expr(s, k, "at" + std::to_string(u)) + ";\n";
+                continue;
+            }
             if (s.nt_mask & KC_CHAIN_NT_BIT(k))
                 std::snprintf(buf, sizeof buf, "    const f4 in%u_%u = __builtin_nontemporal_load(&reinterpret_cast<const raw4 *>(P.in[b][%u])[at%u]);\n", k, u, k, u);
             else
@@ -333,6 +370,11 @@
     src += "namespace kc {\n";
     src += kJitChainProgramH;
     src += kPackedF4;
+    if (s.in_tiers) {
+        const char *pack_text = kJitChainPackH;
+        if (!pack_text) return std::string();
+        src += pack_text;
+    }
     if (pow) {
         src += kJitPowPositiveInc;
         src += "static __device__ __noinline__ float pow_general(float a, float b) { return (float)pow((double)a, (double)b); }\n"
@@ -362,6 +404,10 @@
     else
         src += "    const unsigned int row = idx / P.row_units, col = idx - row * P.row_units;\n";
     for (uint32_t k = 0; k < s.n_in; ++k) {
+        if (KC_CHAIN_TIER(s.in_tiers, k)) {
+            src += "    const f4 in" + std::to_string(k) + " = " + load_expr(s, k, "col") + ";\n";
+            continue;
+        }
         if (s.nt_mask & KC_CHAIN_NT_BIT(k))
             std::snprintf(buf, sizeof buf, "    const f4 in%u = __builtin_nontemporal_load(&reinterpret_cast<const raw4 *>(P.in[b][%u])[row * P.in_pitch[b][%u] + col]);\n", k, k, k);
         else
@@ -680,7 +726,8 @@
             std::fprintf(f, "{\"name\": \"%s\", \"n_in\": %u, \"start_src\": %d, \"flat\": %d, \"nt_mask\": %u, \"up_taps\": %u, \"up_wide\": %d, \"words\": [",
                          kernel_name(sig).c_str(), sig.n_in, sig.start_src, sig.flat ? 1 : 0, sig.nt_mask, sig.up_taps, sig.up_wide ? 1 : 0);
             for (uint32_t k = 0; k < sig.n_ops; ++k) std::fprintf(f, "%s%u", k ? ", " : "", sig.word[k]);
-            std::fprintf(f, "]}\n");
+            if (sig.in_tiers) std::fprintf(f, "], \"in_tiers\": %u}\n", sig.in_tiers);
+            else std::fprintf(f, "]}\n");
             std::fclose(f);
         }
     }
@@ -749,6 +796,7 @@
     mix(s.up_wide ? 1 : 0);
     mix(s.nt_mask);
     mix(s.quads);
+    mix(s.in_tiers);
     for (uint32_t i = 0; i < s.n_ops; ++i) mix(s.word[i]);
     return h;
 }
@@ -756,7 +804,7 @@
 static bool same_signature(const Signature &a, const Signature &b)
 {
     return a.n_in == b.n_in && a.n_ops == b.n_ops && a.start_src == b.start_src && a.flat == b.flat && a.up_taps == b.up_taps &&
-           a.up_wide == b.up_wide && a.nt_mask == b.nt_mask && a.quads == b.quads &&
+           a.up_wide == b.up_wide && a.nt_mask == b.nt_mask && a.quads == b.quads && a.in_tiers == b.in_tiers &&
            std::memcmp(a.word, b.word, sizeof(uint32_t) * a.n_ops) == 0;
 }
 
@@ -852,6 +900,8 @@
     }
     return e;
 }
+
+bool chain_pack_program_ok(const ChainProgram &P) { return pack_program_ok(P); }
 
 hipError_t launch_upsample_chain_specialized(const ChainProgram &P, int batch, const UpsampleArgs &U, hipStream_t s, bool *launched)
 {
@@ -1005,9 +1055,12 @@
     return false;
 }
 
-int kernel_cache_precompile(const uint32_t *words, uint32_t n_ops, uint32_t n_in, int32_t start_src, bool flat, uint32_t nt_mask,
+int kernel_cache_precompile(const uint32_t *words, uint32_t n_ops, uint32_t n_in, int32_t start_src, bool flat, uint32_t nt_mask, uint32_t in_tiers,
                             uint32_t up_taps, bool up_wide, const char *dir, std::string *log)
 {
+    if (in_tiers && (!flat || up_taps || (n_in < 16 && in_tiers >> (2 * n_in)))) return KC_ERR_INVALID_ARG;
+    for (uint32_t k = 0; k < n_in; ++k)
+        if (KC_CHAIN_TIER(in_tiers, k) == 3u) return KC_ERR_INVALID_ARG;
     if (!words || n_ops < 1 || n_ops > (uint32_t)KC_CHAIN_MAX_OPS || n_in > (uint32_t)KC_CHAIN_MAX_IN || !dir || !*dir) return KC_ERR_INVALID_ARG;
     Signature sig;
     sig.n_in = n_in;
@@ -1017,6 +1070,7 @@
     sig.nt_mask = nt_mask;
     sig.up_taps = up_taps;
     sig.up_wide = up_wide;
+    sig.in_tiers = in_tiers;
     for (uint32_t i = 0; i < n_ops; ++i) sig.word[i] = words[i];
     sig.quads = chain_quads_for(sig, 0);
     const std::string src = generate(sig);
```

Result: faster. 7.089 million, median of 6 (+11.3%).
